# Edenzzzz/Stable-Diffusion-for-book-cover-generation

Hardware: NVIDIA B200
Metric: unet_denoise_it_per_s (higher is better)
Workload: dtype bf16

## Files before the change

### include/b200sd.h

```cpp
#ifndef B200SD_H_
#define B200SD_H_

#include <stddef.h>
#include <stdint.h>

#ifdef __cplusplus
extern "C" {
#endif

#define B200SD_OK 0
#define B200SD_ERR_INVALID 1
#define B200SD_ERR_CUDA 2
#define B200SD_ERR_UNSUPPORTED 3

#define B200SD_F32 0
#define B200SD_BF16 1

typedef void* b200sd_stream_t;

const char* b200sd_last_error(void);
int b200sd_version(void);
int64_t b200sd_launch_count(void);

void b200sd_debug_gemm_trace(void* buf);
void b200sd_debug_set(int key, int value);
int b200sd_timer_reserve(int n);
int b200sd_timer_record(int i, b200sd_stream_t stream);
int b200sd_timer_elapsed_ms(int i, int j, float* ms);


int b200sd_cfg_ddim_step(const void* eps_u, const void* eps_c, const void* x, void* out, void* eps_out,
                         int64_t n, float guidance, float sa_t, float sb_t, float sa_p, float sb_p,
                         int eps_dtype, int x_dtype, b200sd_stream_t stream);

int b200sd_sampler_advance(const float* timesteps, int n_steps, int* cursor, float* in_t, int n_t, b200sd_stream_t stream);
int b200sd_cfg_ddim_step_table(const void* eps_u, const void* eps_c, const void* x, void* out, void* eps_out,
                               int64_t n, float guidance, const float* coef_table, const int* cursor,
                               int eps_dtype, int x_dtype, b200sd_stream_t stream);

int b200sd_cfg_plms_step_table(const float* eps_u, const float* eps_c, float* x, float* saved, float* ring, int64_t n,
                               float guidance, const float* table, const int* cursor, b200sd_stream_t stream);

int b200sd_cfg_plms_step(const void* eps_u, const void* eps_c, const void* x, void* out, void* eps_out,
                         const void* hist0, const void* hist1, const void* hist2, const void* hist3,
                         int nhist, const float* w_host5, int64_t n, float guidance, float cx, float ce,
                         int eps_dtype, int x_dtype, b200sd_stream_t stream);

int b200sd_add_noise(const void* x0, const void* noise, const int64_t* timesteps, const float* sa_table,
                     const float* sb_table, void* out, int batch, int64_t per_sample, int num_train_timesteps,
                     int dtype, b200sd_stream_t stream);

int b200sd_mse_workspace_floats(void);
int b200sd_mse_loss_fwd(const void* pred, const void* target, float* loss_out, float* workspace, int64_t n,
                        int pred_dtype, int target_dtype, b200sd_stream_t stream);
int b200sd_mse_loss_bwd(const void* pred, const void* target, const float* grad_loss, void* grad_pred, int64_t n,
                        int pred_dtype, int target_dtype, b200sd_stream_t stream);


int b200sd_timestep_embedding(const float* timesteps, float* out, int batch, int dim, b200sd_stream_t stream);

int b200sd_small_linear(const float* in, const void* w_bf16, const float* bias, float* out, int batch, int N, int K,
                        int silu_in, int silu_out, b200sd_stream_t stream);

#define B200SD_EPI_LINEAR 0
#define B200SD_EPI_GEGLU 1
#define B200SD_W_ROW_MAJOR 0
#define B200SD_W_KBLOCK_MAJOR 1

typedef struct b200sd_gemm_args {
    const void* a0;
    const void* a1;
    const void* w;
    const float* bias;
    const float* rowbias;
    const void* residual;
    void* out;
    int M, N, K;
    int C0, C1;
    int lda0, lda1;
    int ldc, ldr;
    int ldrb;
    int conv_taps;
    int batch, H, W;
    int rows_per_image;
    int epilogue;
    int out_dtype;
    int residual_dtype;
    int block_n;
    int split_k;
    void* workspace;
    size_t workspace_bytes;
    int pair;
    float* gn_part;
    const void* prefetch;
    size_t prefetch_bytes;
    int w_layout;
} b200sd_gemm_args;

size_t b200sd_gemm_workspace_bytes(void);
int b200sd_geglu_tile(int N);
int b200sd_gemm(const b200sd_gemm_args* args, b200sd_stream_t stream);
int b200sd_gemm_gn_layout(const b200sd_gemm_args* args, int hw, int* parts_per_image, int* total_parts);

typedef struct b200sd_dgrad_args {
    const void* dy;
    const void* w;
    const void* residual;
    void* out;
    int M, Cout, Cin;
    int conv_taps;
    int batch, H, W;
    int ldy, ldc, ldr;
    int out_dtype, residual_dtype;
    int block_n;
    int pair;
} b200sd_dgrad_args;
int b200sd_gemm_dgrad(const b200sd_dgrad_args* args, b200sd_stream_t stream);

typedef struct b200sd_wgrad_args {
    const void* dy;
    const void* x;
    float* dw;
    int rows, Cout, Cin;
    int conv_taps;
    int batch, H, W;
    int ldy, ldx, lddw;
    int block_n, split_k;
} b200sd_wgrad_args;
int b200sd_gemm_wgrad(const b200sd_wgrad_args* args, b200sd_stream_t stream);

int b200sd_conv_in(const float* x_nchw, const float* w, const float* bias, void* out_nhwc, int batch, int Cin,
                   int Cout, int H, int W, int out_dtype, b200sd_stream_t stream);
int b200sd_conv_out(const void* x_nhwc, const float* w, const float* bias, float* out_nchw, int batch, int Cin,
                    int Cout, int H, int W, b200sd_stream_t stream);
int b200sd_nhwc_bias_to_nchw(const float* x, const float* bias, float* out_nchw, int batch, int C, int hw, int ld,
                             b200sd_stream_t stream);

int b200sd_groupnorm_silu(const void* x0, const void* x1, int C0, int C1, const float* gamma, const float* beta,
                          void* out, void* raw_out, float* stats_ws, int batch, int hw, int groups, float eps,
                          int silu, int in_dtype, b200sd_stream_t stream);

int b200sd_groupnorm_silu_stats(const void* x0, const void* x1, int C0, int C1, const float* gamma, const float* beta,
                                void* out, void* raw_out, float* stats_ws, float* stats_out, int batch, int hw, int groups,
                                float eps, int silu, int in_dtype, b200sd_stream_t stream);

int b200sd_groupnorm_silu_parts(const void* x0, const void* x1, int C0, int C1, const float* part0, int ppi0, int ld0,
                                const float* part1, int ppi1, int ld1, const float* gamma, const float* beta, void* out,
                                void* raw_out, float* stats_out, int batch, int hw, int groups, float eps, int silu,
                                int in_dtype, b200sd_stream_t stream);

int b200sd_groupnorm_workspace_floats(int batch);
int b200sd_layernorm(const void* x, const float* gamma, const float* beta, void* out, int rows, int C, float eps,
                     int in_dtype, b200sd_stream_t stream);

size_t b200sd_attention_workspace_bytes(int batch, int heads, int Skv, int d);
int b200sd_attention(const void* q, const void* k, const void* v, void* out, int batch, int heads, int Sq, int Skv,
                     int d, int ldq, int ldk, int ldv, int ldo, float scale, void* workspace, size_t workspace_bytes,
                     b200sd_stream_t stream);

int b200sd_attention_lse(const void* q, const void* k, const void* v, void* out, float* lse, int batch, int heads, int Sq,
                         int Skv, int d, int ldq, int ldk, int ldv, int ldo, float scale, void* workspace,
                         size_t workspace_bytes, b200sd_stream_t stream);

size_t b200sd_attention_bwd_workspace_bytes(int batch, int heads, int Sq);
int b200sd_attention_bwd(const void* q, const void* k, const void* v, const void* out, const void* dout,
                         const float* lse, void* dq, void* dk, void* dv, int batch, int heads, int Sq, int Skv, int d,
                         int ldq, int ldk, int ldv, int ldo, int lddo, int lddq, int lddk, int lddv, float scale,
                         void* workspace, size_t workspace_bytes, b200sd_stream_t stream);


int b200sd_clip_embed(const int64_t* ids, const float* tok, const float* pos, float* out, int batch, int S, int C, int vocab,
                      b200sd_stream_t stream);
int b200sd_clip_embed_bwd(const int64_t* ids, const float* dx, float* dtok, float* dpos, int batch, int S, int C, int vocab,
                          b200sd_stream_t stream);
int b200sd_quick_gelu_fwd(const void* u, void* out, int64_t n, b200sd_stream_t stream);
int b200sd_quick_gelu_bwd(const void* u, const void* dg, void* du, int64_t n, b200sd_stream_t stream);
int b200sd_layernorm_f32out(const float* x, const float* gamma, const float* beta, float* out, int rows, int C, float eps,
                            b200sd_stream_t stream);
int b200sd_causal_attention(const void* qkv, void* out, int batch, int heads, int S, int d, int ld, int ldo, int q_off,
                            int k_off, int v_off, float scale, b200sd_stream_t stream);
int b200sd_causal_attention_bwd(const void* qkv, const void* dout, void* dqkv, int batch, int heads, int S, int d, int ld,
                                int lddo, int ldd, int q_off, int k_off, int v_off, float scale, b200sd_stream_t stream);


int b200sd_im2col_s2_pad(const void* x, void* out, int batch, int H, int W, int C, int in_dtype, int pad,
                         b200sd_stream_t stream);
int b200sd_softmax_rows(const float* x, void* out_bf16, int rows, int L, int ldx, int ldo, float scale, b200sd_stream_t stream);
int b200sd_conv1x1_small(const float* x_nchw, const float* w, const float* bias, float* out_nchw, int batch, int Cin, int Cout,
                         int hw, b200sd_stream_t stream);
int b200sd_gaussian_sample(const float* moments, const float* noise, float* out, int batch, int C, int hw, float out_scale,
                           b200sd_stream_t stream);


int b200sd_grad_prep(const void* in, int in_dtype, void* out_bf16, float* colsum, int rows, int N, int ld,
                     int rows_per_image, int ldcs, b200sd_stream_t stream);

int b200sd_groupnorm_bwd_workspace_floats(int batch);
int b200sd_groupnorm_silu_bwd(const void* x0, const void* x1, int C0, int C1, int in_dtype, const float* gamma,
                              const float* beta, const void* dy, const float* add_src, void* out0, void* out1,
                              int out_dtype, int accumulate0, int accumulate1, float* dgamma, float* dbeta,
                              const float* mean_rstd, float* workspace, int batch, int hw, int groups, float eps, int silu,
                              b200sd_stream_t stream);

int b200sd_layernorm_bwd(const void* x, int in_dtype, const float* gamma, const void* dy, float* dres, float* dgamma,
                         float* dbeta, int rows, int C, float eps, b200sd_stream_t stream);

int b200sd_geglu_fwd(const void* u, void* out, int64_t rows, int C_half, b200sd_stream_t stream);
int b200sd_geglu_bwd(const void* u, const void* dff, void* du, int64_t rows, int C_half, b200sd_stream_t stream);

int b200sd_upsample2x_bwd(const void* dy, float* dx, int batch, int H, int W, int C, int accumulate, b200sd_stream_t stream);
int b200sd_col2im_s2(const void* dcol, float* dx, int batch, int H, int W, int C, int accumulate, b200sd_stream_t stream);

int b200sd_conv_out_bwd(const float* dout_nchw, const void* x_nhwc, const float* w, void* dx_nhwc, float* dw,
                        float* dbias, int batch, int Cin, int Cout, int H, int W, b200sd_stream_t stream);
int b200sd_conv_in_wgrad(const void* dy_nhwc, int dy_dtype, const float* x_nchw, float* dw, int batch, int Cin, int Cout,
                         int H, int W, b200sd_stream_t stream);

int b200sd_cast_act(const float* in, void* out_bf16, int64_t n, int silu, b200sd_stream_t stream);
int b200sd_silu_bwd_mul(const float* pre, float* grad, int64_t n, b200sd_stream_t stream);

int b200sd_split_hi_lo(const float* x, void* hi_bf16, void* lo_bf16, int64_t n, b200sd_stream_t stream);
int b200sd_groupnorm_silu_split(const void* x0, const void* x1, int C0, int C1, const float* gamma, const float* beta,
                                void* out, void* out_lo, void* raw_out, void* raw_lo, float* stats_ws, float* stats_out,
                                int batch, int hw, int groups, float eps, int silu, int in_dtype, b200sd_stream_t stream);
int b200sd_layernorm_split(const void* x, const float* gamma, const float* beta, void* out, void* out_lo, int rows, int C,
                           float eps, int in_dtype, b200sd_stream_t stream);
int b200sd_geglu_f32(const float* u, void* hi_bf16, void* lo_bf16, int64_t rows, int C_half, b200sd_stream_t stream);
int b200sd_attention_f32(const float* q, const float* k, const float* v, float* out, int batch, int heads, int Sq, int Skv,
                         int d, int ldq, int ldk, int ldv, int ldo, float scale, b200sd_stream_t stream);
int b200sd_small_linear_f32(const float* in, const float* w, const float* bias, float* out, int batch, int N, int K,
                            int silu_in, int silu_out, b200sd_stream_t stream);

int b200sd_cast_flat(const float* in, void* out_bf16, int64_t n, b200sd_stream_t stream);
int b200sd_adamw_step(float* param, float* grad, float* exp_avg, float* exp_avg_sq, void* weights_bf16, int64_t n,
                      float lr, float beta1, float beta2, float eps, float weight_decay, int step, float grad_scale,
                      int zero_grad, b200sd_stream_t stream);

int b200sd_adamw8bit_step(float* param, float* grad, uint8_t* state1, uint8_t* state2, float* absmax1, float* absmax2,
                          const float* qmap1, const float* qmap2, const int32_t* chunk_mode, float* small_exp_avg,
                          float* small_exp_avg_sq, void* weights_bf16, int64_t n, float lr, float beta1, float beta2, float eps,
                          float weight_decay, int step, float grad_scale, int zero_grad, b200sd_stream_t stream);

int b200sd_upsample2x(const void* x, void* out, int batch, int H, int W, int C, int in_dtype, b200sd_stream_t stream);
int b200sd_im2col_s2(const void* x, void* out, int batch, int H, int W, int C, int in_dtype, b200sd_stream_t stream);

#ifdef __cplusplus
}
#endif
#endif
```

### stable-diffusion-for-book-cover-generation_b200/_lib.py

```python
from __future__ import annotations

import ctypes as C
import os

_HERE = os.path.dirname(os.path.abspath(__file__))
LIB_PATH = os.path.join(_HERE, "libb200sd.so")

_lib = None


class B200SDError(RuntimeError):
    pass


class GemmArgs(C.Structure):
    _fields_ = [
        ("a0", C.c_void_p), ("a1", C.c_void_p), ("w", C.c_void_p), ("bias", C.c_void_p), ("rowbias", C.c_void_p),
        ("residual", C.c_void_p), ("out", C.c_void_p),
        ("M", C.c_int), ("N", C.c_int), ("K", C.c_int), ("C0", C.c_int), ("C1", C.c_int),
        ("lda0", C.c_int), ("lda1", C.c_int), ("ldc", C.c_int), ("ldr", C.c_int), ("ldrb", C.c_int), ("conv_taps", C.c_int),
        ("batch", C.c_int), ("H", C.c_int), ("W", C.c_int), ("rows_per_image", C.c_int), ("epilogue", C.c_int),
        ("out_dtype", C.c_int), ("residual_dtype", C.c_int), ("block_n", C.c_int), ("split_k", C.c_int),
        ("workspace", C.c_void_p), ("workspace_bytes", C.c_size_t), ("pair", C.c_int), ("gn_part", C.c_void_p), ("prefetch", C.c_void_p), ("prefetch_bytes", C.c_size_t), ("w_layout", C.c_int),
    ]


class DgradArgs(C.Structure):
    _fields_ = [
        ("dy", C.c_void_p), ("w", C.c_void_p), ("residual", C.c_void_p), ("out", C.c_void_p),
        ("M", C.c_int), ("Cout", C.c_int), ("Cin", C.c_int), ("conv_taps", C.c_int),
        ("batch", C.c_int), ("H", C.c_int), ("W", C.c_int), ("ldy", C.c_int), ("ldc", C.c_int), ("ldr", C.c_int),
        ("out_dtype", C.c_int), ("residual_dtype", C.c_int), ("block_n", C.c_int), ("pair", C.c_int),
    ]


class WgradArgs(C.Structure):
    _fields_ = [
        ("dy", C.c_void_p), ("x", C.c_void_p), ("dw", C.c_void_p),
        ("rows", C.c_int), ("Cout", C.c_int), ("Cin", C.c_int), ("conv_taps", C.c_int),
        ("batch", C.c_int), ("H", C.c_int), ("W", C.c_int), ("ldy", C.c_int), ("ldx", C.c_int), ("lddw", C.c_int),
        ("block_n", C.c_int), ("split_k", C.c_int),
    ]


_vp, _i, _i64, _f, _sz = C.c_void_p, C.c_int, C.c_int64, C.c_float, C.c_size_t

SIGNATURES = {
    "b200sd_last_error": (C.c_char_p, []),
    "b200sd_version": (_i, []),
    "b200sd_launch_count": (_i64, []),
    "b200sd_debug_gemm_trace": (None, [_vp]),
    "b200sd_debug_set": (None, [_i, _i]),
    "b200sd_timer_reserve": (_i, [_i]),
    "b200sd_timer_record": (_i, [_i, _vp]),
    "b200sd_timer_elapsed_ms": (_i, [_i, _i, C.POINTER(C.c_float)]),
    "b200sd_cfg_ddim_step": (_i, [_vp, _vp, _vp, _vp, _vp, _i64, _f, _f, _f, _f, _f, _i, _i, _vp]),
    "b200sd_clip_embed": (_i, [_vp, _vp, _vp, _vp, _i, _i, _i, _i, _vp]),
    "b200sd_clip_embed_bwd": (_i, [_vp, _vp, _vp, _vp, _i, _i, _i, _i, _vp]),
    "b200sd_quick_gelu_fwd": (_i, [_vp, _vp, _i64, _vp]),
    "b200sd_quick_gelu_bwd": (_i, [_vp, _vp, _vp, _i64, _vp]),
    "b200sd_layernorm_f32out": (_i, [_vp, _vp, _vp, _vp, _i, _i, _f, _vp]),
    "b200sd_causal_attention": (_i, [_vp, _vp, _i, _i, _i, _i, _i, _i, _i, _i, _i, _f, _vp]),
    "b200sd_causal_attention_bwd": (_i, [_vp, _vp, _vp, _i, _i, _i, _i, _i, _i, _i, _i, _i, _i, _f, _vp]),
    "b200sd_im2col_s2_pad": (_i, [_vp, _vp, _i, _i, _i, _i, _i, _i, _vp]),
    "b200sd_softmax_rows": (_i, [_vp, _vp, _i, _i, _i, _i, _f, _vp]),
    "b200sd_conv1x1_small": (_i, [_vp, _vp, _vp, _vp, _i, _i, _i, _i, _vp]),
    "b200sd_gaussian_sample": (_i, [_vp, _vp, _vp, _i, _i, _i, _f, _vp]),
    "b200sd_sampler_advance": (_i, [_vp, _i, _vp, _vp, _i, _vp]),
    "b200sd_cfg_plms_step_table": (_i, [_vp, _vp, _vp, _vp, _vp, _i64, _f, _vp, _vp, _vp]),
    "b200sd_cfg_ddim_step_table": (_i, [_vp, _vp, _vp, _vp, _vp, _i64, _f, _vp, _vp, _i, _i, _vp]),
    "b200sd_cfg_plms_step": (_i, [_vp, _vp, _vp, _vp, _vp, _vp, _vp, _vp, _vp, _i, C.POINTER(C.c_float), _i64, _f, _f,
                                  _f, _i, _i, _vp]),
    "b200sd_add_noise": (_i, [_vp, _vp, _vp, _vp, _vp, _vp, _i, _i64, _i, _i, _vp]),
    "b200sd_mse_workspace_floats": (_i, []),
    "b200sd_mse_loss_fwd": (_i, [_vp, _vp, _vp, _vp, _i64, _i, _i, _vp]),
    "b200sd_mse_loss_bwd": (_i, [_vp, _vp, _vp, _vp, _i64, _i, _i, _vp]),
    "b200sd_timestep_embedding": (_i, [_vp, _vp, _i, _i, _vp]),
    "b200sd_small_linear": (_i, [_vp, _vp, _vp, _vp, _i, _i, _i, _i, _i, _vp]),
    "b200sd_gemm_workspace_bytes": (_sz, []),
    "b200sd_geglu_tile": (_i, [_i]),
    "b200sd_gemm": (_i, [C.POINTER(GemmArgs), _vp]),
    "b200sd_gemm_gn_layout": (_i, [C.POINTER(GemmArgs), _i, C.POINTER(C.c_int), C.POINTER(C.c_int)]),
    "b200sd_groupnorm_silu_parts": (_i, [_vp, _vp, _i, _i, _vp, _i, _i, _vp, _i, _i, _vp, _vp, _vp, _vp, _vp, _i, _i, _i, _f, _i,
                                         _i, _vp]),
    "b200sd_gemm_dgrad": (_i, [C.POINTER(DgradArgs), _vp]),
    "b200sd_gemm_wgrad": (_i, [C.POINTER(WgradArgs), _vp]),
    "b200sd_conv_in": (_i, [_vp, _vp, _vp, _vp, _i, _i, _i, _i, _i, _i, _vp]),
    "b200sd_conv_out": (_i, [_vp, _vp, _vp, _vp, _i, _i, _i, _i, _i, _vp]),
    "b200sd_nhwc_bias_to_nchw": (_i, [_vp, _vp, _vp, _i, _i, _i, _i, _vp]),
    "b200sd_groupnorm_silu": (_i, [_vp, _vp, _i, _i, _vp, _vp, _vp, _vp, _vp, _i, _i, _i, _f, _i, _i, _vp]),
    "b200sd_groupnorm_silu_stats": (_i, [_vp, _vp, _i, _i, _vp, _vp, _vp, _vp, _vp, _vp, _i, _i, _i, _f, _i, _i, _vp]),
    "b200sd_groupnorm_workspace_floats": (_i, [_i]),
    "b200sd_layernorm": (_i, [_vp, _vp, _vp, _vp, _i, _i, _f, _i, _vp]),
    "b200sd_attention_workspace_bytes": (_sz, [_i, _i, _i, _i]),
    "b200sd_attention": (_i, [_vp, _vp, _vp, _vp, _i, _i, _i, _i, _i, _i, _i, _i, _i, _f, _vp, _sz, _vp]),
    "b200sd_attention_lse": (_i, [_vp, _vp, _vp, _vp, _vp, _i, _i, _i, _i, _i, _i, _i, _i, _i, _f, _vp, _sz, _vp]),
    "b200sd_attention_bwd_workspace_bytes": (_sz, [_i, _i, _i]),
    "b200sd_attention_bwd": (_i, [_vp] * 9 + [_i] * 13 + [_f, _vp, _sz, _vp]),
    "b200sd_grad_prep": (_i, [_vp, _i, _vp, _vp, _i, _i, _i, _i, _i, _vp]),
    "b200sd_groupnorm_bwd_workspace_floats": (_i, [_i]),
    "b200sd_groupnorm_silu_bwd": (_i, [_vp, _vp, _i, _i, _i, _vp, _vp, _vp, _vp, _vp, _vp, _i, _i, _i, _vp, _vp, _vp, _vp, _i,
                                       _i, _i, _f, _i, _vp]),
    "b200sd_layernorm_bwd": (_i, [_vp, _i, _vp, _vp, _vp, _vp, _vp, _i, _i, _f, _vp]),
    "b200sd_geglu_fwd": (_i, [_vp, _vp, _i64, _i, _vp]),
    "b200sd_geglu_bwd": (_i, [_vp, _vp, _vp, _i64, _i, _vp]),
    "b200sd_upsample2x_bwd": (_i, [_vp, _vp, _i, _i, _i, _i, _i, _vp]),
    "b200sd_col2im_s2": (_i, [_vp, _vp, _i, _i, _i, _i, _i, _vp]),
    "b200sd_conv_out_bwd": (_i, [_vp, _vp, _vp, _vp, _vp, _vp, _i, _i, _i, _i, _i, _vp]),
    "b200sd_conv_in_wgrad": (_i, [_vp, _i, _vp, _vp, _i, _i, _i, _i, _i, _vp]),
    "b200sd_cast_act": (_i, [_vp, _vp, _i64, _i, _vp]),
    "b200sd_silu_bwd_mul": (_i, [_vp, _vp, _i64, _vp]),
    "b200sd_split_hi_lo": (_i, [_vp, _vp, _vp, _i64, _vp]),
    "b200sd_groupnorm_silu_split": (_i, [_vp, _vp, _i, _i, _vp, _vp, _vp, _vp, _vp, _vp, _vp, _vp, _i, _i, _i, _f, _i, _i, _vp]),
    "b200sd_layernorm_split": (_i, [_vp, _vp, _vp, _vp, _vp, _i, _i, _f, _i, _vp]),
    "b200sd_geglu_f32": (_i, [_vp, _vp, _vp, _i64, _i, _vp]),
    "b200sd_attention_f32": (_i, [_vp, _vp, _vp, _vp, _i, _i, _i, _i, _i, _i, _i, _i, _i, _f, _vp]),
    "b200sd_small_linear_f32": (_i, [_vp, _vp, _vp, _vp, _i, _i, _i, _i, _i, _vp]),
    "b200sd_cast_flat": (_i, [_vp, _vp, _i64, _vp]),
    "b200sd_adamw_step": (_i, [_vp, _vp, _vp, _vp, _vp, _i64, _f, _f, _f, _f, _f, _i, _f, _i, _vp]),
    "b200sd_adamw8bit_step": (_i, [_vp] * 12 + [_i64, _f, _f, _f, _f, _f, _i, _f, _i, _vp]),
    "b200sd_upsample2x": (_i, [_vp, _vp, _i, _i, _i, _i, _i, _vp]),
    "b200sd_im2col_s2": (_i, [_vp, _vp, _i, _i, _i, _i, _i, _vp]),
}


def lib() -> C.CDLL:
    global _lib
    if _lib is None:
        if not os.path.exists(LIB_PATH):
            raise B200SDError(
                f"{LIB_PATH} is missing: build it with `python -c 'import __graft_entry__ as g; g.build()'` "
                "(b200sd has no CPU / eager fallback)")
        L = C.CDLL(LIB_PATH)
        for name, (res, args) in SIGNATURES.items():
            fn = getattr(L, name)
            fn.restype = res
            fn.argtypes = args
        _lib = L
    return _lib


def check(rc: int, what: str = "") -> None:
    if rc != 0:
        msg = lib().b200sd_last_error().decode("utf-8", "replace")
        raise B200SDError(f"{what or 'b200sd call'} failed (code {rc}): {msg}")
```

### stable-diffusion-for-book-cover-generation_b200/csrc/gemm_tcgen05.cu

```cuda
#include <atomic>
#include <cstring>
#include <mutex>
#include <cstdio>
#include <cstdlib>

#include "common.cuh"

extern std::atomic<long long> g_b200sd_launches;

static unsigned long long* g_gemm_trace = nullptr;
static int g_dbg[4] = {-1, 0, 0, 0};
static const int g_dbg_env = [] {
    const char* e = getenv("B200SD_EPI_DEPTH");
    if (e) g_dbg[3] = atoi(e);
    return 0;
}();
extern "C" void b200sd_debug_set(int key, int value) { if (key >= 0 && key < 4) g_dbg[key] = value; }
extern "C" void b200sd_debug_gemm_trace(void* buf) { g_gemm_trace = static_cast<unsigned long long*>(buf); }

namespace {

__device__ __forceinline__ unsigned long long gtimer() {
    unsigned long long t;
    asm volatile("mov.u64 %0, %globaltimer;" : "=l"(t));
    return t;
}
#define TRACE(slot)                                                                                   \
    do {                                                                                              \
        if (p.trace) p.trace[((size_t)(blockIdx.z * gridDim.y + blockIdx.y) * gridDim.x + blockIdx.x) * 16 + (slot)] = gtimer(); \
    } while (0)

constexpr int BLOCK_M = 128;
constexpr size_t kWsPartialBytes = (size_t)160 * 128 * 256 * sizeof(float);
constexpr size_t kWsCounterBytes = 4096;
constexpr int BLOCK_K = 64;
constexpr int UMMA_K = 16;
constexpr int kNumThreads = 192;
constexpr int kMaxStages = 8;
constexpr int kABytes = BLOCK_M * BLOCK_K * 2;


struct KParams {
    CUtensorMap tmA0, tmA1, tmB;
    const float* bias;
    const float* rowbias;
    const void* residual;
    void* out;
    int M, N;
    int num_k_blocks;
    int kb_per_split;
    int split_k;
    int block_n;
    int stages;
    int conv;
    int cblocks0;
    int cblocks;
    int tile_w, tile_h, tile_n;
    int tiles_y;
    int tiles_x;
    int rows_valid;
    int a_bytes;
    int ldc, ldr, ldrb;
    int rows_per_image;
    int epilogue;
    int out_f32;
    int res_f32;
    uint32_t tmem_cols;
    int a_mn;
    int b_mode;
    int conv_sign;
    int n_valid;
    int tiles_per_tap;
    int atomic_out;
    int pair;
    int persist;
    int psplit;
    int w_kmajor;
    const void* prefetch;
    size_t prefetch_bytes;
    float* gn_part;
    unsigned long long* trace;
};

__device__ __forceinline__ void cluster_sync_all() {
    asm volatile("barrier.cluster.arrive.release.aligned;\n\tbarrier.cluster.wait.acquire.aligned;" ::: "memory");
}
__device__ __forceinline__ uint32_t cluster_ctarank() {
    uint32_t r;
    asm volatile("mov.u32 %0, %%cluster_ctarank;" : "=r"(r));
    return r;
}
__device__ __forceinline__ float4 ld_dsmem_v4(uint32_t local_smem_addr, uint32_t cta_rank) {
    uint32_t raddr;
    asm volatile("mapa.shared::cluster.u32 %0, %1, %2;" : "=r"(raddr) : "r"(local_smem_addr), "r"(cta_rank));
    float4 v;
    asm volatile("ld.shared::cluster.v4.f32 {%0, %1, %2, %3}, [%4];" : "=f"(v.x), "=f"(v.y), "=f"(v.z), "=f"(v.w) : "r"(raddr) : "memory");
    return v;
}

__device__ __forceinline__ void red_add_v4(float* dst, float a, float b, float c, float d) {
    asm volatile("red.global.add.v4.f32 [%0], {%1, %2, %3, %4};" ::"l"(dst), "f"(a), "f"(b), "f"(c), "f"(d) : "memory");
}

struct EpiCtx {
    uint32_t stage_u32;
    int pitch_f, row_end, R, cb, half, m0, col_out, img0, n0cb;
    const float* s_rb;
    bool multi_img, rb_smem;
};
__device__ __forceinline__ void lds8(uint32_t addr, float (&v)[8]) {
    asm volatile("ld.shared.v4.f32 {%0, %1, %2, %3}, [%4];" : "=f"(v[0]), "=f"(v[1]), "=f"(v[2]), "=f"(v[3]) : "r"(addr));
    asm volatile("ld.shared.v4.f32 {%0, %1, %2, %3}, [%4];" : "=f"(v[4]), "=f"(v[5]), "=f"(v[6]), "=f"(v[7]) : "r"(addr + 16));
}
template <int OUT, int RES, bool SPLIT, bool GEGLU, bool STATS = false>
__device__ __forceinline__ void epilogue_rows(const KParams& p, const EpiCtx& e, int row0, const float (&b)[8], const float (&bg)[8],
                                              float* cs = nullptr, float* cq = nullptr) {
    constexpr int U = 4;
    for (int row = row0; row < e.row_end; row += e.R * U) {
        float v[U][8], r[U][8];
#pragma unroll
        for (int u = 0; u < U; ++u) {
            const int rl = min(row + u * e.R, e.row_end - 1);
            const uint32_t addr = e.stage_u32 + (uint32_t)(rl * e.pitch_f + e.cb) * 4u;
            if constexpr (SPLIT) {
#pragma unroll
                for (int i = 0; i < 8; ++i) v[u][i] = 0.f;
                for (int sp = 0; sp < p.split_k; ++sp) {
                    const float4 a0 = ld_dsmem_v4(addr, sp), a1 = ld_dsmem_v4(addr + 16, sp);
                    v[u][0] += a0.x; v[u][1] += a0.y; v[u][2] += a0.z; v[u][3] += a0.w;
                    v[u][4] += a1.x; v[u][5] += a1.y; v[u][6] += a1.z; v[u][7] += a1.w;
                }
            } else {
                lds8(addr, v[u]);
            }
            if constexpr (GEGLU) lds8(addr + (uint32_t)e.half * 4u, r[u]);
            else if constexpr (RES == 2) ld8<B200SD_F32>(p.residual, (size_t)(e.m0 + rl) * p.ldr + e.col_out, r[u]);
            else if constexpr (RES == 1) ld8<B200SD_BF16>(p.residual, (size_t)(e.m0 + rl) * p.ldr + e.col_out, r[u]);
        }
#pragma unroll
        for (int u = 0; u < U; ++u) {
            const int rl = row + u * e.R;
            if (rl >= e.row_end) break;
            const int grow = e.m0 + rl;
            float o[8];
            if constexpr (GEGLU) {
#pragma unroll
                for (int i = 0; i < 8; ++i) o[i] = (v[u][i] + b[i]) * gelu_erf_f(r[u][i] + bg[i]);
                st8<B200SD_BF16>(p.out, (size_t)grow * p.ldc + e.col_out, o);
            } else {
#pragma unroll
                for (int i = 0; i < 8; ++i) o[i] = v[u][i] + b[i];
                if constexpr (RES != 0) {
#pragma unroll
                    for (int i = 0; i < 8; ++i) o[i] += r[u][i];
                }
                if (e.multi_img) {
                    const int img = grow / p.rows_per_image;
                    if (e.rb_smem) {
                        const float* rb = e.s_rb + (img == e.img0 ? 0 : 256) + e.cb;
#pragma unroll
                        for (int i = 0; i < 8; ++i) o[i] += rb[i];
                    } else {
                        float t[8];
                        ld8<B200SD_F32>(p.rowbias, (size_t)img * p.ldrb + e.n0cb, t);
#pragma unroll
                        for (int i = 0; i < 8; ++i) o[i] += t[i];
                    }
                }
                if constexpr (STATS) {
#pragma unroll
                    for (int i = 0; i < 8; ++i) { cs[i] += o[i]; cq[i] = fmaf(o[i], o[i], cq[i]); }
                }
                if constexpr (OUT == 2) {
                    float* dst = static_cast<float*>(p.out) + (size_t)grow * p.ldc + e.col_out;
                    red_add_v4(dst, o[0], o[1], o[2], o[3]);
                    red_add_v4(dst + 4, o[4], o[5], o[6], o[7]);
                } else if constexpr (OUT == 1) st8<B200SD_F32>(p.out, (size_t)grow * p.ldc + e.col_out, o);
                else st8<B200SD_BF16>(p.out, (size_t)grow * p.ldc + e.col_out, o);
            }
        }
    }
}

template <bool PAIR, int OP>
__global__ void __launch_bounds__(kNumThreads, 1) gemm_tcgen05_kernel(const __grid_constant__ KParams p) {
    constexpr bool a_mn = OP >= 2;
    constexpr int b_mode = OP;
    extern __shared__ uint8_t smem_raw[];
    uint8_t* smem = reinterpret_cast<uint8_t*>((reinterpret_cast<uintptr_t>(smem_raw) + 1023) & ~uintptr_t(1023));
    constexpr bool pair = PAIR;
    const uint32_t crank = pair ? cluster_ctarank() : 0;
    const int b_bytes = (p.block_n * BLOCK_K * 2) >> (pair ? 1 : 0);
    uint8_t* smem_a = smem;
    uint8_t* smem_b = smem + (size_t)p.stages * kABytes;
    uint64_t* bars = reinterpret_cast<uint64_t*>(smem_b + (size_t)p.stages * b_bytes);
    uint64_t* full_bar = bars;
    uint64_t* empty_bar = bars + kMaxStages;
    uint64_t* tmem_full_bar = bars + 2 * kMaxStages;
    uint32_t* tmem_slot = reinterpret_cast<uint32_t*>(bars + 2 * kMaxStages + 1);

    const int warp = threadIdx.x >> 5;
    const int lane = threadIdx.x & 31;
    const int m_tile = blockIdx.x;
    const int n_tile = blockIdx.y;
    const int split = blockIdx.z;
    const int kb_begin = split * p.kb_per_split;
    const int kb_end = min(kb_begin + p.kb_per_split, p.num_k_blocks);
    const int w_tap = b_mode == 3 ? n_tile / p.tiles_per_tap : 0;
    const int n0 = (b_mode == 3 ? n_tile - w_tap * p.tiles_per_tap : n_tile) * p.block_n;
    const int col_base = w_tap * p.n_valid + n0;
    const int col_valid = min(p.block_n, p.n_valid - n0);
    const int m0 = m_tile * p.rows_valid;

    ptx::pdl_trigger();
    if (threadIdx.x == 0) TRACE(0);
    if (warp == 0 && lane == 0) {
        ptx::prefetch_tmap(&p.tmA0);
        ptx::prefetch_tmap(&p.tmB);
        if (p.cblocks0 != p.cblocks) ptx::prefetch_tmap(&p.tmA1);
        for (int s = 0; s < p.stages; ++s) {
            ptx::mbar_init(&full_bar[s], 1);
            ptx::mbar_init(&empty_bar[s], 1);
        }
        ptx::mbar_init(tmem_full_bar, 1);
        ptx::fence_barrier_init();
    }
    if (warp == 1) {
        if constexpr (pair) { ptx::tmem_alloc_cg2(tmem_slot, p.tmem_cols); ptx::tmem_relinquish_cg2(); }
        else { ptx::tmem_alloc(tmem_slot, p.tmem_cols); ptx::tmem_relinquish(); }
    }
    ptx::tc_fence_before();
    __syncthreads();
    if constexpr (pair) cluster_sync_all();
    ptx::tc_fence_after();
    const uint32_t tmem_base = *tmem_slot;
    ptx::pdl_wait();
    if (threadIdx.x == 0) TRACE(1);

    const int epi_tid = threadIdx.x - 64;
    const int pitch_f = p.block_n + 4;
    float* stage = reinterpret_cast<float*>(smem);
    float* s_bias = reinterpret_cast<float*>(bars + 32);
    float* s_rb = s_bias + 256;
    int img0 = 0, img1 = 0;
    bool rb_smem = false;
    if (p.rowbias && m0 < p.M) {
        img0 = m0 / p.rows_per_image;
        img1 = (min(m0 + p.rows_valid, p.M) - 1) / p.rows_per_image;
        rb_smem = (img1 - img0) <= 1;
    }

    if (warp == 0) {
        if (ptx::elect_one()) {
            int stage = 0;
            uint32_t phase = 0;
            int img = 0, y0 = 0, x0 = 0;
            if (p.conv) {
                if (p.tile_n > 1) { img = m_tile * p.tile_n; y0 = 0; }
                else {
                    int mt = m_tile;
                    if (p.tiles_x > 1) { x0 = (mt % p.tiles_x) * p.tile_w; mt /= p.tiles_x; }
                    img = mt / p.tiles_y; y0 = (mt % p.tiles_y) * p.tile_h;
                }
            }
            const int nbox_live = (b_mode != 0 && !pair) ? (col_valid + 63) >> 6 : (p.block_n >> 6);
            const int nboxb = nbox_live >> (pair ? 1 : 0);
            const int nb0 = n0 + (pair ? (int)crank * (p.block_n >> 1) : 0);
            const uint32_t stage_tx = (b_mode != 0 && !pair) ? (uint32_t)(p.a_bytes + nbox_live * 8192)
                                                             : ((uint32_t)(p.a_bytes + b_bytes) << (pair ? 1 : 0));
            for (int kb = kb_begin; kb < kb_end; ++kb) {
                ptx::mbar_wait(&empty_bar[stage], phase ^ 1);
                if (!pair || crank == 0) ptx::mbar_expect_tx(&full_bar[stage], stage_tx);
                uint8_t* dst_a = smem_a + (size_t)stage * kABytes;
                uint8_t* dst_b = smem_b + (size_t)stage * b_bytes;
                uint64_t* fb = &full_bar[stage];
                const uint32_t fbc = pair ? ptx::mapa_u32(ptx::smem_u32(fb), 0) : 0;
#define LD2(dst, tm, c0, c1) do { if constexpr (pair) ptx::tma_load_2d_cg2(dst, tm, fbc, c0, c1); else ptx::tma_load_2d(dst, tm, fb, c0, c1); } while (0)
#define LD3(dst, tm, c0, c1, c2) do { if constexpr (pair) ptx::tma_load_3d_cg2(dst, tm, fbc, c0, c1, c2); else ptx::tma_load_3d(dst, tm, fb, c0, c1, c2); } while (0)
#define LD4(dst, tm, c0, c1, c2, c3) do { if constexpr (pair) ptx::tma_load_4d_cg2(dst, tm, fbc, c0, c1, c2, c3); else ptx::tma_load_4d(dst, tm, fb, c0, c1, c2, c3); } while (0)
                if (a_mn) {
                    LD2(dst_a, &p.tmA0, m0, kb * BLOCK_K);
                    LD2(dst_a + kABytes / 2, &p.tmA0, m0 + 64, kb * BLOCK_K);
                } else if (!p.conv) {
                    if (kb < p.cblocks0) LD2(dst_a, &p.tmA0, kb * BLOCK_K, m0);
                    else LD2(dst_a, &p.tmA1, (kb - p.cblocks0) * BLOCK_K, m0);
                } else {
                    const int tap = kb / p.cblocks;
                    const int cb = kb - tap * p.cblocks;
                    const int dy = (tap / 3 - 1) * p.conv_sign, dx = (tap % 3 - 1) * p.conv_sign;
                    if (cb < p.cblocks0) LD4(dst_a, &p.tmA0, cb * BLOCK_K, x0 + dx, y0 + dy, img);
                    else LD4(dst_a, &p.tmA1, (cb - p.cblocks0) * BLOCK_K, x0 + dx, y0 + dy, img);
                }
                if (b_mode == 0) {
                    if (p.w_kmajor) LD3(dst_b, &p.tmB, 0, nb0, kb);
                    else LD2(dst_b, &p.tmB, kb * BLOCK_K, nb0);
                } else if (b_mode == 1) {
                    if (!p.conv) {
                        for (int j = 0; j < nboxb; ++j) LD2(dst_b + j * 8192, &p.tmB, nb0 + j * 64, kb * BLOCK_K);
                    } else {
                        const int tap = kb / p.cblocks;
                        const int cb = kb - tap * p.cblocks;
                        for (int j = 0; j < nboxb; ++j) LD3(dst_b + j * 8192, &p.tmB, nb0 + j * 64, tap, cb * BLOCK_K);
                    }
                } else if (b_mode == 2) {
                    for (int j = 0; j < nboxb; ++j) LD2(dst_b + j * 8192, &p.tmB, nb0 + j * 64, kb * BLOCK_K);
                } else {
                    int bimg, by0;
                    if (p.tile_n > 1) { bimg = kb * p.tile_n; by0 = 0; }
                    else { bimg = kb / p.tiles_y; by0 = (kb - bimg * p.tiles_y) * p.tile_h; }
                    const int dy = w_tap / 3 - 1, dx = w_tap % 3 - 1;
                    for (int j = 0; j < nboxb; ++j) LD4(dst_b + j * 8192, &p.tmB, nb0 + j * 64, dx, by0 + dy, bimg);
                }
#undef LD2
#undef LD3
#undef LD4
                if (++stage == p.stages) { stage = 0; phase ^= 1; }
            }
        }
    } else if (warp == 1) {
        if ((!pair || crank == 0) && ptx::elect_one()) {
            const uint32_t b_mn = b_mode != 0;
            const uint32_t mma_n = (b_mode != 0 && !pair) ? (uint32_t)(((col_valid + 63) >> 6) << 6) : (uint32_t)p.block_n;
            const uint32_t idesc = ptx::umma_idesc_bf16(pair ? 2 * BLOCK_M : BLOCK_M, mma_n) | ((uint32_t)a_mn << 15) | (b_mn << 16);
            const uint32_t a_step = a_mn ? (2048 >> 4) : 2, b_step = b_mn ? (2048 >> 4) : 2;
            int stage = 0;
            uint32_t phase = 0;
            for (int kb = kb_begin; kb < kb_end; ++kb) {
                ptx::mbar_wait(&full_bar[stage], phase);
                ptx::tc_fence_after();
                if (kb == kb_begin) TRACE(2);
                const uint32_t sa = ptx::smem_u32(smem_a + (size_t)stage * kABytes), sb = ptx::smem_u32(smem_b + (size_t)stage * b_bytes);
                const uint64_t da = a_mn ? ptx::umma_desc_mn_sw128(sa, 8192) : ptx::umma_desc_k_sw128(sa);
                const uint64_t db = b_mn ? ptx::umma_desc_mn_sw128(sb, 8192) : ptx::umma_desc_k_sw128(sb);
#pragma unroll
                for (int k = 0; k < BLOCK_K / UMMA_K; ++k) {
                    const uint32_t accum = (kb > kb_begin || k > 0) ? 1u : 0u;
                    if constexpr (pair) ptx::umma_bf16_ss_cg2(tmem_base, da + a_step * k, db + b_step * k, idesc, accum);
                    else ptx::umma_bf16_ss(tmem_base, da + a_step * k, db + b_step * k, idesc, accum);
                }
                if constexpr (pair) ptx::umma_commit_cg2(&empty_bar[stage], 3); else ptx::umma_commit(&empty_bar[stage]);
                if (++stage == p.stages) { stage = 0; phase ^= 1; }
            }
            if constexpr (pair) ptx::umma_commit_cg2(tmem_full_bar, 3); else ptx::umma_commit(tmem_full_bar);
            TRACE(3);
        }
    } else {
        const int q = warp & 3;
        const int r_in_tile = q * 32 + lane;
        const uint32_t taddr = tmem_base + ((uint32_t)(q * 32) << 16);
        for (int c = epi_tid; c < p.block_n; c += 128) {
            s_bias[c] = (p.bias && c < col_valid) ? __ldg(p.bias + n0 + c) : 0.f;
            if (rb_smem) {
                s_rb[c] = __ldg(p.rowbias + (size_t)img0 * p.ldrb + n0 + c);
                s_rb[256 + c] = __ldg(p.rowbias + (size_t)img1 * p.ldrb + n0 + c);
            }
        }
        if (epi_tid == 0 && p.prefetch_bytes)
            ptx::prefetch_share_l2(p.prefetch, p.prefetch_bytes, (blockIdx.z * gridDim.y + blockIdx.y) * gridDim.x + blockIdx.x,
                              gridDim.x * gridDim.y * gridDim.z);
        ptx::mbar_wait(tmem_full_bar, 0);
        ptx::tc_fence_after();
        if (epi_tid == 0) TRACE(4);
        {
            float4* my_row = reinterpret_cast<float4*>(stage + (size_t)r_in_tile * pitch_f);
            for (int c = 0; c < p.block_n; c += 32) {
                uint32_t r0[16], r1[16];
                const bool two = (c + 16 < p.block_n);
                ptx::tmem_ld_32x32b_x16(taddr + c, r0);
                if (two) ptx::tmem_ld_32x32b_x16(taddr + c + 16, r1);
                ptx::tmem_ld_wait();
#pragma unroll
                for (int i = 0; i < 4; ++i)
                    my_row[c / 4 + i] = make_float4(__uint_as_float(r0[4 * i]), __uint_as_float(r0[4 * i + 1]),
                                                    __uint_as_float(r0[4 * i + 2]), __uint_as_float(r0[4 * i + 3]));
                if (two) {
#pragma unroll
                    for (int i = 0; i < 4; ++i)
                        my_row[c / 4 + 4 + i] = make_float4(__uint_as_float(r1[4 * i]), __uint_as_float(r1[4 * i + 1]),
                                                            __uint_as_float(r1[4 * i + 2]), __uint_as_float(r1[4 * i + 3]));
                }
            }
        }
        ptx::tc_fence_before();
        ptx::named_bar_sync(1, 128);
        if (epi_tid == 0) TRACE(5);
    }

    if (p.split_k > 1) cluster_sync_all(); else __syncthreads();

    {
        const int rank = p.split_k > 1 ? (int)cluster_ctarank() : 0;
        const int rows_per_cta = BLOCK_M / p.split_k;
        const int row_begin = rank * rows_per_cta;
        int valid = min(p.rows_valid, p.M - m0) - row_begin;
        valid = max(0, min(valid, rows_per_cta));
        const bool geglu = p.epilogue == B200SD_EPI_GEGLU;
        const int half = p.block_n / 2;
        const int groups = (geglu ? half : p.block_n) / 8;
        const int R = kNumThreads / groups;
        const int tid = threadIdx.x;
        float cs[8], cq[8];
#pragma unroll
        for (int i = 0; i < 8; ++i) { cs[i] = 0.f; cq[i] = 0.f; }
        if (tid < R * groups && valid > 0) {
            const int c8 = tid % groups, r0 = tid / groups;
            const int cb = c8 * 8;
            if (geglu || cb < col_valid) {
                float b[8], bg[8];
#pragma unroll
                for (int i = 0; i < 8; ++i) { b[i] = s_bias[cb + i]; bg[i] = geglu ? s_bias[half + cb + i] : 0.f; }
                const bool multi_img = p.rowbias != nullptr && img1 != img0;
                if (p.rowbias != nullptr && !multi_img) {
#pragma unroll
                    for (int i = 0; i < 8; ++i) b[i] += s_rb[cb + i];
                }
                EpiCtx e;
                e.stage_u32 = ptx::smem_u32(stage);
                e.pitch_f = pitch_f; e.row_end = row_begin + valid; e.R = R; e.cb = cb; e.half = half; e.m0 = m0;
                e.col_out = geglu ? n_tile * half + cb : col_base + cb;
                e.s_rb = s_rb; e.img0 = img0; e.multi_img = multi_img; e.rb_smem = rb_smem; e.n0cb = n0 + cb;
                const int row0 = row_begin + r0;
                const int ok = p.atomic_out ? 2 : (p.out_f32 ? 1 : 0);
                const int rk = p.residual ? (p.res_f32 ? 2 : 1) : 0;
                if (geglu) epilogue_rows<0, 0, false, true>(p, e, row0, b, bg);
                else if (p.split_k > 1) {
                    if (ok == 1 && p.gn_part) { if (rk == 2) epilogue_rows<1, 2, true, false, true>(p, e, row0, b, bg, cs, cq); else epilogue_rows<1, 0, true, false, true>(p, e, row0, b, bg, cs, cq); }
                    else if (ok == 1) { if (rk == 2) epilogue_rows<1, 2, true, false>(p, e, row0, b, bg); else if (rk == 1) epilogue_rows<1, 1, true, false>(p, e, row0, b, bg); else epilogue_rows<1, 0, true, false>(p, e, row0, b, bg); }
                    else { if (rk == 2) epilogue_rows<0, 2, true, false>(p, e, row0, b, bg); else if (rk == 1) epilogue_rows<0, 1, true, false>(p, e, row0, b, bg); else epilogue_rows<0, 0, true, false>(p, e, row0, b, bg); }
                } else if (ok == 2) epilogue_rows<2, 0, false, false>(p, e, row0, b, bg);
                else if (ok == 1 && p.gn_part) { if (rk == 2) epilogue_rows<1, 2, false, false, true>(p, e, row0, b, bg, cs, cq); else epilogue_rows<1, 0, false, false, true>(p, e, row0, b, bg, cs, cq); }
                else if (ok == 1) { if (rk == 2) epilogue_rows<1, 2, false, false>(p, e, row0, b, bg); else if (rk == 1) epilogue_rows<1, 1, false, false>(p, e, row0, b, bg); else epilogue_rows<1, 0, false, false>(p, e, row0, b, bg); }
                else { if (rk == 2) epilogue_rows<0, 2, false, false>(p, e, row0, b, bg); else if (rk == 1) epilogue_rows<0, 1, false, false>(p, e, row0, b, bg); else epilogue_rows<0, 0, false, false>(p, e, row0, b, bg); }
            }
        }
        if (p.gn_part != nullptr) {
            if (p.split_k > 1) cluster_sync_all(); else __syncthreads();
            float* s_gn = reinterpret_cast<float*>(stage);
#pragma unroll
            for (int i = 0; i < 8; ++i) { s_gn[tid * 16 + i] = cs[i]; s_gn[tid * 16 + 8 + i] = cq[i]; }
            __syncthreads();
            float* dst = p.gn_part + (size_t)(m_tile * p.split_k + rank) * 2 * p.N;
            for (int idx = tid; idx < groups * 16; idx += kNumThreads) {
                const int c8 = idx >> 4, k = idx & 15, col = c8 * 8 + (k & 7);
                float a = 0.f;
                for (int r = 0; r < R; ++r) a += s_gn[(r * groups + c8) * 16 + k];
                if (col < col_valid) dst[(size_t)(k >> 3) * p.N + n0 + col] = a;
            }
        }
        if (epi_tid == 0) TRACE(6);
    }
    if (p.split_k > 1 && p.gn_part == nullptr) cluster_sync_all();

    ptx::tc_fence_before();
    __syncthreads();
    if constexpr (pair) cluster_sync_all();
    if (warp == 1) {
        ptx::tc_fence_after();
        if constexpr (pair) ptx::tmem_dealloc_cg2(tmem_base, p.tmem_cols); else ptx::tmem_dealloc(tmem_base, p.tmem_cols);
    }
    if (threadIdx.x == 0) TRACE(7);
}

constexpr int kEpiWarps = 8;
constexpr int kPersistThreads = 64 + 32 * kEpiWarps + 32;
constexpr int kMaxDepth = 3;

struct PParams {
    CUtensorMap tmA0, tmA1, tmB, tmOut, tmRes;
    const float* bias;
    const float* rowbias;
    float* gn_part;
    int M, N;
    int num_k_blocks, block_n, stages;
    int conv, cblocks0, cblocks, tile_h, tile_n, tiles_y, w_kmajor;
    int tile_w, tiles_x;
    int n_tiles, num_tiles;
    int ldrb, rows_per_image;
    int geglu, out_f32, res_kind;
    int pf_share;
    int depth;
    int chunk_bytes;
    uint32_t tmem_cols, acc_stride;
    uint32_t off_b, off_epi, off_bias, off_stat, off_bars;
    int split, kb_per_split;
    CUtensorMap tmWs;
    float* ws;
    int* cnt;
    const void* prefetch;
    size_t prefetch_bytes;
    const void* residual;
    void* out;
    int ldc, ldr;
    unsigned long long* trace;
};
#define PTRACE(slot) do { if (p.trace) p.trace[(size_t)blockIdx.x * 16 + (slot)] = gtimer(); } while (0)
#ifdef B200SD_TRACE_EPILOGUE
#define PACC(i) do { if (p.trace && ew == 0) { const long long t__ = clock64(); pacc[i] += t__ - pt0; pt0 = t__; } } while (0)
#else
#define PACC(i) do { } while (0)
#endif


template <bool OUT_F32, int RES, bool GEGLU, bool STATS>
__device__ __forceinline__ void persist_chunk(const PParams& p, uint32_t taddr, int ch, const float* sbv, const float* sbg, uint8_t* cb,
                                              int lane, bool last_chunk, uint64_t* tempty_bar, uint64_t* rfull_bar, uint32_t rparity,
                                              float* gn_dst, int nrows) {
    uint32_t r0[16], r1[16], g0[16], g1[16];
    ptx::tmem_ld_32x32b_x16(taddr + ch * 32, r0);
    ptx::tmem_ld_32x32b_x16(taddr + ch * 32 + 16, r1);
    const int half = p.block_n >> 1;
    if constexpr (GEGLU) {
        ptx::tmem_ld_32x32b_x16(taddr + half + ch * 32, g0);
        ptx::tmem_ld_32x32b_x16(taddr + half + ch * 32 + 16, g1);
    }
    if constexpr (RES != 0) ptx::mbar_wait(rfull_bar, rparity);
    ptx::tmem_ld_wait();
    if (last_chunk) {
        ptx::tc_fence_before();
        __syncwarp();
        if (lane == 0) ptx::mbar_arrive(tempty_bar);
    }
    float v[32];
    const float4* sb4 = reinterpret_cast<const float4*>(sbv);
#pragma unroll
    for (int j = 0; j < 8; ++j) {
        const float4 b = sb4[j];
        const uint32_t* r = j < 4 ? r0 : r1;
        const int o = (j & 3) * 4;
        v[4 * j + 0] = __uint_as_float(r[o + 0]) + b.x;
        v[4 * j + 1] = __uint_as_float(r[o + 1]) + b.y;
        v[4 * j + 2] = __uint_as_float(r[o + 2]) + b.z;
        v[4 * j + 3] = __uint_as_float(r[o + 3]) + b.w;
    }
    if constexpr (GEGLU) {
        const float4* sg4 = reinterpret_cast<const float4*>(sbg);
#pragma unroll
        for (int j = 0; j < 8; ++j) {
            const float4 b = sg4[j];
            const uint32_t* r = j < 4 ? g0 : g1;
            const int o = (j & 3) * 4;
            v[4 * j + 0] *= gelu_erf_fast(__uint_as_float(r[o + 0]) + b.x);
            v[4 * j + 1] *= gelu_erf_fast(__uint_as_float(r[o + 1]) + b.y);
            v[4 * j + 2] *= gelu_erf_fast(__uint_as_float(r[o + 2]) + b.z);
            v[4 * j + 3] *= gelu_erf_fast(__uint_as_float(r[o + 3]) + b.w);
        }
    }
    uint8_t* row128 = cb + lane * 128;
    uint8_t* row64 = cb + lane * 64;
    const int x128 = lane & 7, x64 = (lane >> 1) & 3;
    if constexpr (RES == 2) {
#pragma unroll
        for (int j = 0; j < 8; ++j) {
            const float4 t = *reinterpret_cast<const float4*>(row128 + ((j ^ x128) << 4));
            v[4 * j + 0] += t.x; v[4 * j + 1] += t.y; v[4 * j + 2] += t.z; v[4 * j + 3] += t.w;
        }
    } else if constexpr (RES == 1) {
#pragma unroll
        for (int j = 0; j < 4; ++j) {
            const uint4 u = *reinterpret_cast<const uint4*>(row64 + ((j ^ x64) << 4));
            float2 f;
            f = unpack_bf16x2(u.x); v[8 * j + 0] += f.x; v[8 * j + 1] += f.y;
            f = unpack_bf16x2(u.y); v[8 * j + 2] += f.x; v[8 * j + 3] += f.y;
            f = unpack_bf16x2(u.z); v[8 * j + 4] += f.x; v[8 * j + 5] += f.y;
            f = unpack_bf16x2(u.w); v[8 * j + 6] += f.x; v[8 * j + 7] += f.y;
        }
    }
    if constexpr (RES != 0 && ((RES == 2) != OUT_F32)) __syncwarp();
    if constexpr (OUT_F32) {
#pragma unroll
        for (int j = 0; j < 8; ++j)
            *reinterpret_cast<float4*>(row128 + ((j ^ x128) << 4)) = make_float4(v[4 * j], v[4 * j + 1], v[4 * j + 2], v[4 * j + 3]);
    } else {
#pragma unroll
        for (int j = 0; j < 4; ++j) {
            uint4 u;
            u.x = pack_bf16x2(v[8 * j + 0], v[8 * j + 1]);
            u.y = pack_bf16x2(v[8 * j + 2], v[8 * j + 3]);
            u.z = pack_bf16x2(v[8 * j + 4], v[8 * j + 5]);
            u.w = pack_bf16x2(v[8 * j + 6], v[8 * j + 7]);
            *reinterpret_cast<uint4*>(row64 + ((j ^ x64) << 4)) = u;
        }
    }
    if constexpr (STATS) {
        __syncwarp();
        float s = 0.f, ss = 0.f;
        const uint8_t* colp = cb + ((lane & 3) << 2);
        const int piece = lane >> 2;
        for (int r = 0; r < nrows; ++r) {
            const float x = *reinterpret_cast<const float*>(colp + r * 128 + ((piece ^ (r & 7)) << 4));
            s += x;
            ss = fmaf(x, x, ss);
        }
        gn_dst[ch * 32 + lane] = s;
        gn_dst[256 + ch * 32 + lane] = ss;
    }
}

template <bool OUT_F32, int RES, bool GEGLU, bool STATS>
__device__ __forceinline__ void persist_epilogue(const PParams& p, uint8_t* smem, uint32_t tmem_base, int warp, int lane) {
    const int ew = warp - 2;
    const int q = warp & 3;
    const int h = ew >> 2;
    const int D = p.depth;
    const int kChunkBytes = p.chunk_bytes;
    uint8_t* my = smem + p.off_epi + (size_t)ew * D * kChunkBytes;
    float* sb = reinterpret_cast<float*>(smem + p.off_bias) + ew * 256;
    uint64_t* bars = reinterpret_cast<uint64_t*>(smem + p.off_bars);
    uint64_t* tfull = bars + 16;
    uint64_t* tempty = bars + 18;
    uint64_t* rfull = bars + 20 + ew * kMaxDepth;
    const int half = p.block_n >> 1;
    const int nch = (GEGLU ? half : p.block_n) >> 5;
    const int nl = nch > h ? (nch - h + 1) >> 1 : 0;
    const int my_tiles = ((int)blockIdx.x < p.num_tiles) ? (p.num_tiles - 1 - (int)blockIdx.x) / (int)gridDim.x + 1 : 0;
    const int total = my_tiles * nl;
    const int out_n = GEGLU ? half : p.block_n;

    auto issue_res = [&](int g) {
        const int itl = g / nl, ch = h + 2 * (g - itl * nl);
        const int tile = (int)blockIdx.x + itl * (int)gridDim.x;
        const int m_tile = tile / p.n_tiles, n_tile = tile - m_tile * p.n_tiles;
        const int buf = g % D;
        ptx::mbar_expect_tx(&rfull[buf], RES == 2 ? 4096u : 2048u);
        ptx::tma_load_2d(my + buf * kChunkBytes, &p.tmRes, &rfull[buf], n_tile * p.block_n + ch * 32, m_tile * BLOCK_M + q * 32);
    };
    if constexpr (RES != 0) {
        if (lane == 0)
            for (int g = 0; g < D && g < total; ++g) issue_res(g);
    }

    int g = 0;
#ifdef B200SD_TRACE_EPILOGUE
    long long pacc[6] = {0, 0, 0, 0, 0, 0}, pt0 = clock64();
#endif
    for (int it = 0; it < my_tiles; ++it) {
        const int tile = (int)blockIdx.x + it * (int)gridDim.x;
        const int m_tile = tile / p.n_tiles, n_tile = tile - m_tile * p.n_tiles;
        const int n0 = n_tile * p.block_n;
        const int row0 = m_tile * BLOCK_M + q * 32;
        PACC(5);
        __syncwarp();
        {
            const int img = p.rowbias ? min(row0, p.M - 1) / p.rows_per_image : 0;
            for (int l = 0; l < nl; ++l) {
                const int c = (h + 2 * l) * 32 + lane;
                float b = p.bias ? __ldg(p.bias + n0 + c) : 0.f;
                if (p.rowbias) b += __ldg(p.rowbias + (size_t)img * p.ldrb + n0 + c);
                sb[l * 32 + lane] = b;
                if constexpr (GEGLU) sb[128 + l * 32 + lane] = p.bias ? __ldg(p.bias + n0 + half + c) : 0.f;
            }
        }
        __syncwarp();
        PACC(0);
        const int acc = it & 1;
        ptx::mbar_wait(&tfull[acc], (uint32_t)(it >> 1) & 1u);
        ptx::tc_fence_after();
        PACC(1);
        if (it == 0 && ew == 0 && lane == 0) PTRACE(4);
        const uint32_t taddr = tmem_base + (uint32_t)acc * p.acc_stride + ((uint32_t)(q * 32) << 16);
        const int nrows = max(0, min(32, p.M - row0));
        float* sstat = reinterpret_cast<float*>(smem + p.off_stat);
        float* gn_dst = STATS ? sstat + q * 512 : nullptr;
        if (nl == 0) {
            ptx::tc_fence_before();
            __syncwarp();
            if (lane == 0) ptx::mbar_arrive(&tempty[acc]);
        }
        for (int l = 0; l < nl; ++l, ++g) {
            const int ch = h + 2 * l;
            const int buf = g % D;
            uint8_t* cb = my + buf * kChunkBytes;
            if constexpr (RES == 0) {
                if (lane == 0) ptx::tma_store_wait_read<1>();
                __syncwarp();
            }
            PACC(2);
            persist_chunk<OUT_F32, RES, GEGLU, STATS>(p, taddr, ch, sb + l * 32, sb + 128 + l * 32, cb, lane, l == nl - 1, &tempty[acc],
                                                     &rfull[buf], (uint32_t)(g / D) & 1u, gn_dst, nrows);
            PACC(3);
            ptx::fence_proxy_async();
            __syncwarp();
            if (lane == 0) {
                ptx::tma_store_2d(&p.tmOut, cb, n_tile * out_n + ch * 32, row0);
                ptx::tma_store_commit();
                if constexpr (RES != 0) {
                    if (g >= 1 && g - 1 + D < total) {
                        ptx::tma_store_wait_read<1>();
                        issue_res(g - 1 + D);
                    }
                }
            }
            PACC(4);
        }
        if constexpr (STATS) {
            ptx::named_bar_sync(1, kEpiWarps * 32);
            const int te = ew * 32 + lane;
            if (te < p.block_n) {
                float s0 = 0.f, s1 = 0.f;
#pragma unroll
                for (int qq = 0; qq < 4; ++qq) { s0 += sstat[qq * 512 + te]; s1 += sstat[qq * 512 + 256 + te]; }
                float* dst = p.gn_part + (size_t)m_tile * 2 * p.N + n0 + te;
                dst[0] = s0;
                dst[p.N] = s1;
            }
            ptx::named_bar_sync(1, kEpiWarps * 32);
        }
    }
    if (ew == 0 && lane == 0) PTRACE(5);
#ifdef B200SD_TRACE_EPILOGUE
    if (p.trace && ew == 0 && lane == 0)
        for (int i = 0; i < 6; ++i) p.trace[(size_t)blockIdx.x * 16 + 8 + i] = (unsigned long long)pacc[i];
#endif
    if (lane == 0) ptx::tma_store_wait<0>();
    __syncwarp();
    if (ew == 0 && lane == 0) PTRACE(6);
}

template <bool OUT_F32, int RES, bool STATS>
__device__ __forceinline__ void persist_epilogue_split(const PParams& p, uint8_t* smem, uint32_t tmem_base, int warp, int lane) {
    const int ew = warp - 2, q = warp & 3, h = ew >> 2;
    const int kChunkBytes = 4096;
    uint8_t* my = smem + p.off_epi + (size_t)ew * 2 * kChunkBytes;
    uint64_t* bars = reinterpret_cast<uint64_t*>(smem + p.off_bars);
    uint64_t* tfull = bars + 16;
    uint64_t* tempty = bars + 18;
    const int unit = blockIdx.x, tile = unit / p.split, s = unit - tile * p.split;
    const int m_tile = tile / p.n_tiles, n_tile = tile - m_tile * p.n_tiles;
    const int n0 = n_tile * p.block_n, m0 = m_tile * BLOCK_M;
    const int nch = p.block_n >> 5;
    const int nl = nch > h ? (nch - h + 1) >> 1 : 0;
    ptx::mbar_wait(&tfull[0], 0);
    ptx::tc_fence_after();
    const uint32_t taddr = tmem_base + ((uint32_t)(q * 32) << 16);
    for (int l = 0; l < nl; ++l) {
        const int ch = h + 2 * l;
        uint8_t* cb = my + (l & 1) * kChunkBytes;
        if (lane == 0) ptx::tma_store_wait_read<1>();
        __syncwarp();
        uint32_t r0[16], r1[16];
        ptx::tmem_ld_32x32b_x16(taddr + ch * 32, r0);
        ptx::tmem_ld_32x32b_x16(taddr + ch * 32 + 16, r1);
        ptx::tmem_ld_wait();
        uint8_t* row128 = cb + lane * 128;
        const int x128 = lane & 7;
#pragma unroll
        for (int j = 0; j < 8; ++j) {
            const uint32_t* r = j < 4 ? r0 : r1;
            const int o = (j & 3) * 4;
            *reinterpret_cast<uint4*>(row128 + ((j ^ x128) << 4)) = make_uint4(r[o], r[o + 1], r[o + 2], r[o + 3]);
        }
        ptx::fence_proxy_async();
        __syncwarp();
        if (lane == 0) {
            ptx::tma_store_2d(&p.tmWs, cb, ch * 32, unit * BLOCK_M + q * 32);
            ptx::tma_store_commit();
        }
    }
    ptx::tc_fence_before();
    __syncwarp();
    if (lane == 0) {
        ptx::mbar_arrive(&tempty[0]);
        ptx::tma_store_wait<0>();
        ptx::fence_proxy_async_global();
        __threadfence();
    }
    ptx::named_bar_sync(1, kEpiWarps * 32);
    const int te = ew * 32 + lane;
    int* cnt_in = p.cnt + tile;
    int* cnt_out = p.cnt + p.num_tiles + tile;
    if (te == 0) {
        atomicAdd(cnt_in, 1);
        int seen;
        long long t0 = clock64();
        do {
            asm volatile("ld.acquire.gpu.global.s32 %0, [%1];" : "=r"(seen) : "l"(cnt_in) : "memory");
            if (clock64() - t0 > 4000000000LL) { printf("b200sd: split-K arrival wait timed out (unit %d)\n", unit); __trap(); }
        } while (seen < p.split);
        __threadfence();
    }
    ptx::named_bar_sync(1, kEpiWarps * 32);
    const int rpc = BLOCK_M / p.split;
    const int groups = p.block_n >> 2;
    const int rslots = (kEpiWarps * 32) / groups < 4 ? (kEpiWarps * 32) / groups : 4;
    const int c4 = te % groups, rslot = te / groups;
    float* sstat = reinterpret_cast<float*>(smem + p.off_stat);
    float cs[4] = {0.f, 0.f, 0.f, 0.f}, cq[4] = {0.f, 0.f, 0.f, 0.f};
    if (rslot < rslots) {
        const int col = n0 + c4 * 4;
        float4 b4 = p.bias ? __ldg(reinterpret_cast<const float4*>(p.bias + col)) : make_float4(0.f, 0.f, 0.f, 0.f);
        for (int r = rslot; r < rpc; r += rslots) {
            const int trow = s * rpc + r;
            const int grow = m0 + trow;
            if (grow >= p.M) break;
            float4 v = make_float4(0.f, 0.f, 0.f, 0.f);
            const float* src = p.ws + ((size_t)(tile * p.split) * BLOCK_M + trow) * p.block_n + c4 * 4;
            for (int j = 0; j < p.split; ++j) {
                const float4 t = __ldcg(reinterpret_cast<const float4*>(src + (size_t)j * BLOCK_M * p.block_n));
                v.x += t.x; v.y += t.y; v.z += t.z; v.w += t.w;
            }
            v.x += b4.x; v.y += b4.y; v.z += b4.z; v.w += b4.w;
            if (p.rowbias) {
                const float4 t = __ldg(reinterpret_cast<const float4*>(p.rowbias + (size_t)(grow / p.rows_per_image) * p.ldrb + col));
                v.x += t.x; v.y += t.y; v.z += t.z; v.w += t.w;
            }
            if constexpr (RES == 2) {
                const float4 t = __ldcg(reinterpret_cast<const float4*>(static_cast<const float*>(p.residual) + (size_t)grow * p.ldr + col));
                v.x += t.x; v.y += t.y; v.z += t.z; v.w += t.w;
            } else if constexpr (RES == 1) {
                const uint2 u = __ldcg(reinterpret_cast<const uint2*>(static_cast<const bf16*>(p.residual) + (size_t)grow * p.ldr + col));
                const float2 f0 = unpack_bf16x2(u.x), f1 = unpack_bf16x2(u.y);
                v.x += f0.x; v.y += f0.y; v.z += f1.x; v.w += f1.y;
            }
            if constexpr (STATS) {
                cs[0] += v.x; cs[1] += v.y; cs[2] += v.z; cs[3] += v.w;
                cq[0] = fmaf(v.x, v.x, cq[0]); cq[1] = fmaf(v.y, v.y, cq[1]); cq[2] = fmaf(v.z, v.z, cq[2]); cq[3] = fmaf(v.w, v.w, cq[3]);
            }
            if constexpr (OUT_F32) {
                *reinterpret_cast<float4*>(static_cast<float*>(p.out) + (size_t)grow * p.ldc + col) = v;
            } else {
                uint2 u;
                u.x = pack_bf16x2(v.x, v.y);
                u.y = pack_bf16x2(v.z, v.w);
                *reinterpret_cast<uint2*>(static_cast<bf16*>(p.out) + (size_t)grow * p.ldc + col) = u;
            }
        }
    }
    if constexpr (STATS) {
        if (rslot < 4) {
#pragma unroll
            for (int i = 0; i < 4; ++i) { sstat[rslot * 512 + c4 * 4 + i] = cs[i]; sstat[rslot * 512 + 256 + c4 * 4 + i] = cq[i]; }
        }
        ptx::named_bar_sync(1, kEpiWarps * 32);
        if (te < p.block_n) {
            float s0 = 0.f, s1 = 0.f;
            for (int rs = 0; rs < rslots; ++rs) { s0 += sstat[rs * 512 + te]; s1 += sstat[rs * 512 + 256 + te]; }
            float* dst = p.gn_part + (size_t)(m_tile * p.split + s) * 2 * p.N + n0 + te;
            dst[0] = s0;
            dst[p.N] = s1;
        }
    }
    ptx::named_bar_sync(1, kEpiWarps * 32);
    if (te == 0) {
        __threadfence();
        if (atomicAdd(cnt_out, 1) == p.split - 1) {
            *cnt_out = 0;
            *cnt_in = 0;
            __threadfence();
        }
    }
}

__global__ void __launch_bounds__(kPersistThreads, 1) gemm_persist_kernel(const __grid_constant__ PParams p) {
    extern __shared__ uint8_t smem_raw[];
    uint8_t* smem = reinterpret_cast<uint8_t*>((reinterpret_cast<uintptr_t>(smem_raw) + 1023) & ~uintptr_t(1023));
    uint8_t* smem_a = smem;
    uint8_t* smem_b = smem + p.off_b;
    uint64_t* bars = reinterpret_cast<uint64_t*>(smem + p.off_bars);
    uint64_t* full_bar = bars;
    uint64_t* empty_bar = bars + 8;
    uint64_t* tfull = bars + 16;
    uint64_t* tempty = bars + 18;
    uint64_t* rfull = bars + 20;
    uint32_t* tmem_slot = reinterpret_cast<uint32_t*>(bars + 20 + kEpiWarps * kMaxDepth);
    const int warp = threadIdx.x >> 5;
    const int lane = threadIdx.x & 31;
    const int b_bytes = p.block_n * BLOCK_K * 2;

    const bool splitk = p.split > 1;
    const int sk_tile = splitk ? (int)blockIdx.x / p.split : 0, sk_s = splitk ? (int)blockIdx.x - sk_tile * p.split : 0;
    const int sk_kb0 = splitk ? (sk_s * p.num_k_blocks) / p.split : 0;
    const int sk_kb1 = splitk ? ((sk_s + 1) * p.num_k_blocks) / p.split : p.num_k_blocks;
    int pr_stage = 0, pr_tile = splitk ? sk_tile : (int)blockIdx.x, pr_kb = sk_kb0, pr_m0 = 0, pr_n0 = 0, pr_img = 0, pr_y0 = 0, pr_x0 = 0, pr_tap = 0,
        pr_cb = 0, pr_me = 0;
    bool pr_new = true;
    uint32_t pr_phase = 0;
    constexpr int kPrefetch = 0;
    auto prefetch_b = [&](int k) {
        if (k < p.num_k_blocks && k % p.pf_share == pr_me) {
            if (p.w_kmajor) ptx::tma_prefetch_3d(&p.tmB, 0, pr_n0, k);
            else ptx::tma_prefetch_2d(&p.tmB, k * BLOCK_K, pr_n0);
        }
    };
    auto produce = [&](int limit, const int what) {
        const bool load_a = what & 1, load_b = what & 2;
        while (limit > 0 && pr_tile < p.num_tiles) {
            if (pr_new) {
                pr_new = false;
                const int m_tile = pr_tile / p.n_tiles, n_tile = pr_tile - m_tile * p.n_tiles;
                pr_m0 = m_tile * BLOCK_M;
                pr_n0 = n_tile * p.block_n;
                if (p.conv) {
                    if (p.tile_n > 1) { pr_img = m_tile * p.tile_n; pr_y0 = 0; }
                    else {
                        int mt = m_tile;
                        if (p.tiles_x > 1) { pr_x0 = (mt % p.tiles_x) * p.tile_w; mt /= p.tiles_x; }
                        pr_img = mt / p.tiles_y; pr_y0 = (mt - pr_img * p.tiles_y) * p.tile_h;
                    }
                }
                pr_tap = pr_kb / p.cblocks;
                pr_cb = pr_kb - pr_tap * p.cblocks;
                pr_me = m_tile % p.pf_share;
                if (load_b)
                    for (int k = p.stages; k < kPrefetch; ++k) prefetch_b(k);
            }
            uint64_t* fb = &full_bar[pr_stage];
            if (what) ptx::mbar_wait(&empty_bar[pr_stage], pr_phase ^ 1);
            if (load_a) {
                ptx::mbar_expect_tx(fb, (uint32_t)kABytes);

                uint8_t* dst_a = smem_a + (size_t)pr_stage * kABytes;
                if (!p.conv) {
                    if (pr_kb < p.cblocks0) ptx::tma_load_2d(dst_a, &p.tmA0, fb, pr_kb * BLOCK_K, pr_m0);
                    else ptx::tma_load_2d(dst_a, &p.tmA1, fb, (pr_kb - p.cblocks0) * BLOCK_K, pr_m0);
                } else {
                    const int dy = pr_tap / 3 - 1, dx = pr_tap - (pr_tap / 3) * 3 - 1;
                    if (pr_cb < p.cblocks0) ptx::tma_load_4d(dst_a, &p.tmA0, fb, pr_cb * BLOCK_K, pr_x0 + dx, pr_y0 + dy, pr_img);
                    else ptx::tma_load_4d(dst_a, &p.tmA1, fb, (pr_cb - p.cblocks0) * BLOCK_K, pr_x0 + dx, pr_y0 + dy, pr_img);
                }
            }
            if (load_b) {
                ptx::mbar_expect_tx(fb, (uint32_t)b_bytes);
                uint8_t* dst_b = smem_b + (size_t)pr_stage * b_bytes;
                if (p.w_kmajor) ptx::tma_load_3d(dst_b, &p.tmB, fb, 0, pr_n0, pr_kb);
                else ptx::tma_load_2d(dst_b, &p.tmB, fb, pr_kb * BLOCK_K, pr_n0);
                if (kPrefetch > 0) prefetch_b(pr_kb + kPrefetch);
            }
            if (++pr_stage == p.stages) { pr_stage = 0; pr_phase ^= 1; }
            if (++pr_cb == p.cblocks) { pr_cb = 0; ++pr_tap; }
            if (++pr_kb == sk_kb1) { pr_kb = 0; pr_new = true; pr_tile = splitk ? p.num_tiles : pr_tile + (int)gridDim.x; }
            --limit;
        }
    };
    const bool is_prod_a = threadIdx.x == 0, is_prod_b = threadIdx.x == kPersistThreads - 32;

    ptx::pdl_trigger();
    if (threadIdx.x == 0) PTRACE(0);
    if (warp == 0 && lane == 0) {
        ptx::prefetch_tmap(&p.tmA0);
        ptx::prefetch_tmap(&p.tmB);
        ptx::prefetch_tmap(&p.tmOut);
        if (p.cblocks0 != p.cblocks) ptx::prefetch_tmap(&p.tmA1);
        if (p.res_kind) ptx::prefetch_tmap(&p.tmRes);
        for (int s = 0; s < p.stages; ++s) {
            ptx::mbar_init(&full_bar[s], 2);
            ptx::mbar_init(&empty_bar[s], 1);
        }
        for (int s = 0; s < 2; ++s) {
            ptx::mbar_init(&tfull[s], 1);
            ptx::mbar_init(&tempty[s], kEpiWarps);
        }
        for (int s = 0; s < kEpiWarps * kMaxDepth; ++s) ptx::mbar_init(&rfull[s], 1);
        ptx::fence_barrier_init();
        ptx::pdl_wait();
        produce(p.stages, 3);
    }
    if (warp == 1) {
        ptx::tmem_alloc(tmem_slot, p.tmem_cols);
        ptx::tmem_relinquish();
    }
    ptx::tc_fence_before();
    __syncthreads();
    ptx::tc_fence_after();
    const uint32_t tmem_base = *tmem_slot;
    ptx::pdl_wait();
    if (threadIdx.x == 0) PTRACE(1);

    if (warp == 0) {
        if (is_prod_a) produce(0x7fffffff, 1);
    } else if (warp == kPersistThreads / 32 - 1) {
        if (is_prod_b) {
            produce(p.stages, 0);
            produce(0x7fffffff, 2);
        }
    } else if (warp == 1) {
        if (ptx::elect_one()) {
            const uint32_t idesc = ptx::umma_idesc_bf16(BLOCK_M, (uint32_t)p.block_n);
            int stage = 0;
            uint32_t phase = 0;
            int it = 0;
            const int nkb = sk_kb1 - sk_kb0;
            for (int tile = splitk ? sk_tile : (int)blockIdx.x; tile < p.num_tiles; tile = splitk ? p.num_tiles : tile + (int)gridDim.x, ++it) {
                const int acc = it & 1;
                ptx::mbar_wait(&tempty[acc], ((uint32_t)(it >> 1) & 1u) ^ 1u);
                ptx::tc_fence_after();
                const uint32_t d_tmem = tmem_base + (uint32_t)acc * p.acc_stride;
                for (int kb = 0; kb < nkb; ++kb) {
                    ptx::mbar_wait(&full_bar[stage], phase);
                    ptx::tc_fence_after();
                    if (it == 0 && kb == 0) PTRACE(2);
                    const uint64_t da = ptx::umma_desc_k_sw128(ptx::smem_u32(smem_a + (size_t)stage * kABytes));
                    const uint64_t db = ptx::umma_desc_k_sw128(ptx::smem_u32(smem_b + (size_t)stage * b_bytes));
#pragma unroll
                    for (int k = 0; k < BLOCK_K / UMMA_K; ++k)
                        ptx::umma_bf16_ss(d_tmem, da + 2 * k, db + 2 * k, idesc, (kb > 0 || k > 0) ? 1u : 0u);
                    ptx::umma_commit(&empty_bar[stage]);
                    if (++stage == p.stages) { stage = 0; phase ^= 1; }
                }
                ptx::umma_commit(&tfull[acc]);
                if (it == 0) PTRACE(3);
            }
        }
    } else {
        if (warp == 2 && lane == 0 && p.prefetch_bytes)
            ptx::prefetch_share_l2(p.prefetch, p.prefetch_bytes, blockIdx.x, gridDim.x);
        const int variant = (p.geglu ? 100 : 0) + (p.out_f32 ? 10 : 0) + p.res_kind + (p.gn_part ? 1000 : 0);
        if (splitk) {
            switch (variant) {
                case 0: persist_epilogue_split<false, 0, false>(p, smem, tmem_base, warp, lane); break;
                case 1: persist_epilogue_split<false, 1, false>(p, smem, tmem_base, warp, lane); break;
                case 2: persist_epilogue_split<false, 2, false>(p, smem, tmem_base, warp, lane); break;
                case 10: persist_epilogue_split<true, 0, false>(p, smem, tmem_base, warp, lane); break;
                case 11: persist_epilogue_split<true, 1, false>(p, smem, tmem_base, warp, lane); break;
                case 12: persist_epilogue_split<true, 2, false>(p, smem, tmem_base, warp, lane); break;
                case 1010: persist_epilogue_split<true, 0, true>(p, smem, tmem_base, warp, lane); break;
                case 1012: persist_epilogue_split<true, 2, true>(p, smem, tmem_base, warp, lane); break;
                default: break;
            }
        } else
        switch (variant) {
            case 100: persist_epilogue<false, 0, true, false>(p, smem, tmem_base, warp, lane); break;
            case 0: persist_epilogue<false, 0, false, false>(p, smem, tmem_base, warp, lane); break;
            case 1: persist_epilogue<false, 1, false, false>(p, smem, tmem_base, warp, lane); break;
            case 2: persist_epilogue<false, 2, false, false>(p, smem, tmem_base, warp, lane); break;
            case 10: persist_epilogue<true, 0, false, false>(p, smem, tmem_base, warp, lane); break;
            case 11: persist_epilogue<true, 1, false, false>(p, smem, tmem_base, warp, lane); break;
            case 12: persist_epilogue<true, 2, false, false>(p, smem, tmem_base, warp, lane); break;
            case 1010: persist_epilogue<true, 0, false, true>(p, smem, tmem_base, warp, lane); break;
            case 1012: persist_epilogue<true, 2, false, true>(p, smem, tmem_base, warp, lane); break;
            default: break;
        }
    }
    ptx::tc_fence_before();
    __syncthreads();
    if (warp == 1) {
        ptx::tc_fence_after();
        ptx::tmem_dealloc(tmem_base, p.tmem_cols);
    }
    if (threadIdx.x == 0) PTRACE(7);
}

uint32_t pow2_cols(int n) {
    uint32_t c = 32;
    while ((int)c < n) c <<= 1;
    return c;
}

int pick_block_n(int N, int m_tiles, int epilogue, bool can_split = false) {
    const int step = (epilogue == B200SD_EPI_GEGLU) ? 32 : 16;
    const int sms = b200sd_num_sms();
    int best = 0;
    for (int bn = 160; bn >= 64; bn -= step)
        if (N % bn == 0) { best = bn; break; }
    if (best == 0) {
        for (int bn = 256; bn >= step; bn -= step)
            if (N % bn == 0) { best = bn; break; }
        return best;
    }
    if (epilogue == B200SD_EPI_LINEAR && !can_split && (long)m_tiles * (N / best) * 2 <= sms) {
        for (int bn = 80; bn < best; bn += step)
            if (N % bn == 0 && (long)m_tiles * (N / bn) <= sms) { best = bn; break; }
    }
    return best;
}


typedef void (*gemm_kernel_t)(const KParams);
gemm_kernel_t gemm_entry(int pair, int op) {
    switch ((op << 1) | (pair ? 1 : 0)) {
        case 0: return gemm_tcgen05_kernel<false, 0>;
        case 1: return gemm_tcgen05_kernel<true, 0>;
        case 2: return gemm_tcgen05_kernel<false, 1>;
        case 3: return gemm_tcgen05_kernel<true, 1>;
        case 4: return gemm_tcgen05_kernel<false, 2>;
        case 5: return gemm_tcgen05_kernel<true, 2>;
        case 6: return gemm_tcgen05_kernel<false, 3>;
        default: return gemm_tcgen05_kernel<true, 3>;
    }
}

int configure_gemm_kernels() {
    static std::mutex mu;
    static bool configured[64] = {};
    int dev = 0;
    B200SD_CUDA(cudaGetDevice(&dev));
    std::lock_guard<std::mutex> lock(mu);
    if (dev < 0 || dev >= 64 || configured[dev]) return B200SD_OK;
    for (int i = 0; i < 8; ++i) {
        B200SD_CUDA(cudaFuncSetAttribute(gemm_entry(i & 1, i >> 1), cudaFuncAttributeMaxDynamicSharedMemorySize, (int)(227 * 1024)));
        B200SD_CUDA(cudaFuncSetAttribute(gemm_entry(i & 1, i >> 1), cudaFuncAttributePreferredSharedMemoryCarveout, 100));
    }
    B200SD_CUDA(cudaFuncSetAttribute(gemm_persist_kernel, cudaFuncAttributeMaxDynamicSharedMemorySize, (int)(227 * 1024)));
    B200SD_CUDA(cudaFuncSetAttribute(gemm_persist_kernel, cudaFuncAttributePreferredSharedMemoryCarveout, 100));
    configured[dev] = true;
    return B200SD_OK;
}

bool persist_enabled() {
    static const bool off = getenv("B200SD_PERSIST") && getenv("B200SD_PERSIST")[0] == '0';
    if (g_dbg[0] >= 0) return g_dbg[0] != 0;
    return !off;
}
int pick_block_n_persist(int N, int m_tiles, bool geglu) {
    const int sms = b200sd_num_sms();
    const int step = geglu ? 64 : 32;
    long best_cost = 0;
    int best = 0;
    for (int bn = step; bn <= 256; bn += step) {
        if (N % bn) continue;
        const long tiles = (long)m_tiles * (N / bn);
        const long cost = ((tiles + sms - 1) / sms) * (BLOCK_M + bn);
        if (best == 0 || cost < best_cost || (cost == best_cost && bn > best)) { best = bn; best_cost = cost; }
    }
    return best;
}

int launch_persist(const b200sd_gemm_args* a, const KParams& k, int m_tiles, b200sd_stream_t stream) {
    PParams p;
    memset(&p, 0, sizeof(p));
    p.tmA0 = k.tmA0; p.tmA1 = k.tmA1; p.tmB = k.tmB;
    p.bias = k.bias; p.rowbias = k.rowbias; p.gn_part = k.gn_part;
    p.M = k.M; p.N = k.N;
    p.num_k_blocks = k.num_k_blocks; p.block_n = k.block_n;
    p.conv = k.conv; p.cblocks0 = k.cblocks0; p.cblocks = k.cblocks;
    p.tile_h = k.tile_h; p.tile_n = k.tile_n; p.tiles_y = k.tiles_y; p.w_kmajor = k.w_kmajor;
    p.tile_w = k.tile_w; p.tiles_x = k.tiles_x;
    p.n_tiles = k.N / k.block_n;
    p.num_tiles = m_tiles * p.n_tiles;
    p.ldrb = k.ldrb; p.rows_per_image = k.rows_per_image;
    p.geglu = k.epilogue == B200SD_EPI_GEGLU;
    p.out_f32 = k.out_f32;
    p.res_kind = k.residual ? (k.res_f32 ? 2 : 1) : 0;
    {
        const int sms_ = b200sd_num_sms();
        const int grid_ = p.num_tiles < sms_ ? p.num_tiles : sms_;
        int share = grid_ / p.n_tiles;
        if (share > m_tiles) share = m_tiles;
        p.pf_share = share < 1 ? 1 : share;
    }
    p.depth = p.res_kind ? kMaxDepth : 2;
    if (p.res_kind && g_dbg[3] >= 2 && g_dbg[3] <= kMaxDepth) p.depth = g_dbg[3];
    p.split = k.psplit > 1 ? k.psplit : 1;
    p.kb_per_split = ceil_div(k.num_k_blocks, p.split);
    p.residual = k.residual; p.out = k.out; p.ldc = k.ldc; p.ldr = k.ldr;
    p.prefetch = k.prefetch; p.prefetch_bytes = k.prefetch_bytes;
    const int units = p.num_tiles * p.split;
    if (p.split > 1) {
        B200SD_REQUIRE(k.num_k_blocks >= p.split, "gemm(split-K): fewer K blocks (%d) than slices (%d)", k.num_k_blocks, p.split);
        B200SD_REQUIRE(units <= b200sd_num_sms() && (size_t)units * BLOCK_M * k.block_n * sizeof(float) <= kWsPartialBytes &&
                           (size_t)2 * p.num_tiles * sizeof(int) <= kWsCounterBytes,
                       "gemm(split-K): %d units do not fit the workspace / the machine", units);
        p.depth = 2;
        p.ws = static_cast<float*>(a->workspace);
        p.cnt = reinterpret_cast<int*>(static_cast<char*>(a->workspace) + kWsPartialBytes);
        const uint64_t dims[2] = {(uint64_t)k.block_n, (uint64_t)units * BLOCK_M};
        const uint64_t str[2] = {0, (uint64_t)k.block_n * 4};
        const uint32_t box[2] = {32, 32};
        const int rc = b200sd_make_tmap(&p.tmWs, a->workspace, 2, dims, str, box, CU_TENSOR_MAP_SWIZZLE_128B, CU_TENSOR_MAP_DATA_TYPE_FLOAT32);
        if (rc) return rc;
    }
    const int bn = k.block_n;
    p.acc_stride = bn <= 128 ? 128 : 256;
    p.tmem_cols = 2 * p.acc_stride;
    const int out_cols = p.geglu ? k.N / 2 : k.N;
    {
        const uint64_t dims[2] = {(uint64_t)out_cols, (uint64_t)k.M};
        const uint64_t str[2] = {0, (uint64_t)k.ldc * (k.out_f32 ? 4 : 2)};
        const uint32_t box[2] = {32, 32};
        const int rc = b200sd_make_tmap(&p.tmOut, k.out, 2, dims, str, box, k.out_f32 ? CU_TENSOR_MAP_SWIZZLE_128B : CU_TENSOR_MAP_SWIZZLE_64B,
                                        k.out_f32 ? CU_TENSOR_MAP_DATA_TYPE_FLOAT32 : CU_TENSOR_MAP_DATA_TYPE_BFLOAT16);
        if (rc) return rc;
    }
    if (p.res_kind) {
        const uint64_t dims[2] = {(uint64_t)k.N, (uint64_t)k.M};
        const uint64_t str[2] = {0, (uint64_t)k.ldr * (k.res_f32 ? 4 : 2)};
        const uint32_t box[2] = {32, 32};
        const int rc = b200sd_make_tmap(&p.tmRes, k.residual, 2, dims, str, box, k.res_f32 ? CU_TENSOR_MAP_SWIZZLE_128B : CU_TENSOR_MAP_SWIZZLE_64B,
                                        k.res_f32 ? CU_TENSOR_MAP_DATA_TYPE_FLOAT32 : CU_TENSOR_MAP_DATA_TYPE_BFLOAT16);
        if (rc) return rc;
    }
    const int stage_bytes = kABytes + bn * BLOCK_K * 2;
    p.chunk_bytes = (p.out_f32 || p.res_kind == 2 || k.psplit > 1) ? 4096 : 2048;
    const int epi_bytes = kEpiWarps * p.depth * p.chunk_bytes;
    const int bias_bytes = kEpiWarps * 256 * (int)sizeof(float);
    const int stat_bytes = k.gn_part ? 4 * 2 * 256 * (int)sizeof(float) : 0;
    const int bars_bytes = 512;
    const int budget = 227 * 1024 - 1024;
    int stages = (budget - epi_bytes - bias_bytes - stat_bytes - bars_bytes) / stage_bytes;
    if (stages > kMaxStages) stages = kMaxStages;
    if (g_dbg[1] > 0 && g_dbg[1] < stages) stages = g_dbg[1];
    B200SD_REQUIRE(stages >= 2, "gemm(persistent): smem budget leaves %d stages for block_n %d", stages, bn);
    p.stages = stages;
    p.off_b = (uint32_t)stages * kABytes;
    p.off_epi = (uint32_t)stages * stage_bytes;
    p.off_bias = p.off_epi + epi_bytes;
    p.off_stat = p.off_bias + bias_bytes;
    p.off_bars = p.off_stat + stat_bytes;
    const size_t smem_bytes = (size_t)p.off_bars + bars_bytes + 1024;
    p.trace = g_gemm_trace;
    {
        const int rc = configure_gemm_kernels();
        if (rc) return rc;
    }
    const int sms = b200sd_num_sms();
    cudaLaunchConfig_t cfg = {};
    int grid = p.num_tiles < sms ? p.num_tiles : sms;
    if (g_dbg[2] > 0 && g_dbg[2] < grid) grid = g_dbg[2];
    if (p.split > 1) grid = units;
    cfg.gridDim = dim3(grid);
    cfg.blockDim = dim3(kPersistThreads);
    cfg.dynamicSmemBytes = smem_bytes;
    cfg.stream = static_cast<cudaStream_t>(stream);
    cudaLaunchAttribute attr[2];
    int na = 0;
    if (p.split > 1) {
        attr[na].id = cudaLaunchAttributeCooperative;
        attr[na].val.cooperative = 1;
        ++na;
    }
    if (b200sd_pdl_enabled()) {
        attr[na].id = cudaLaunchAttributeProgrammaticStreamSerialization;
        attr[na].val.programmaticStreamSerializationAllowed = 1;
        ++na;
    }
    cfg.attrs = attr;
    cfg.numAttrs = na;
    B200SD_CUDA(cudaLaunchKernelEx(&cfg, gemm_persist_kernel, p));
    g_b200sd_launches.fetch_add(1, std::memory_order_relaxed);
    B200SD_LAUNCH_CHECK();
    return B200SD_OK;
}

int launch_gemm(KParams& p, int m_tiles, int n_tiles, int grid_z, bool cluster, b200sd_stream_t stream) {
    const int sms = b200sd_num_sms();
    const int bn = p.block_n;
    if (p.pair) m_tiles = (m_tiles + 1) & ~1;
    const int stage_bytes = kABytes + ((bn * BLOCK_K * 2) >> (p.pair ? 1 : 0));
    const long total_ctas = (long)m_tiles * n_tiles * grid_z;
    int stages;
    if (total_ctas <= sms || bn > 160) stages = (200 * 1024) / stage_bytes;
    else stages = (108 * 1024) / stage_bytes;
    if (stages > kMaxStages) stages = kMaxStages;
    if (stages > p.kb_per_split && total_ctas <= sms) stages = p.kb_per_split;
    const int min_stages = ceil_div(BLOCK_M * (bn + 4) * (int)sizeof(float), stage_bytes);
    if (g_dbg[1] > 0 && g_dbg[1] < stages) stages = g_dbg[1];
    if (stages < min_stages) stages = min_stages;
    if (stages < 2) stages = 2;
    p.stages = stages;
    B200SD_REQUIRE((size_t)stages * stage_bytes >= (size_t)BLOCK_M * (bn + 4) * sizeof(float), "gemm: smem ring smaller than the epilogue staging tile");
    const size_t smem_bytes = (size_t)stages * stage_bytes + 1024  + 256  + 3072 ;
    B200SD_REQUIRE(smem_bytes <= 227 * 1024, "gemm: smem budget exceeded (%zu B)", smem_bytes);

    {
        const int rc = configure_gemm_kernels();
        if (rc) return rc;
    }
    p.trace = g_gemm_trace;
    cudaLaunchConfig_t cfg = {};
    cfg.gridDim = dim3(m_tiles, n_tiles, grid_z);
    cfg.blockDim = dim3(kNumThreads);
    cfg.dynamicSmemBytes = smem_bytes;
    cfg.stream = static_cast<cudaStream_t>(stream);
    cudaLaunchAttribute attr[2];
    int na = 0;
    if ((cluster && grid_z > 1) || p.pair) {
        attr[na].id = cudaLaunchAttributeClusterDimension;
        attr[na].val.clusterDim.x = p.pair ? 2 : 1;
        attr[na].val.clusterDim.y = 1;
        attr[na].val.clusterDim.z = p.pair ? 1 : grid_z;
        ++na;
    }
    if (b200sd_pdl_enabled()) {
        attr[na].id = cudaLaunchAttributeProgrammaticStreamSerialization;
        attr[na].val.programmaticStreamSerializationAllowed = 1;
        ++na;
    }
    cfg.attrs = attr;
    cfg.numAttrs = na;
    B200SD_CUDA(cudaLaunchKernelEx(&cfg, gemm_entry(p.pair, p.b_mode), p));
    g_b200sd_launches.fetch_add(1, std::memory_order_relaxed);
    B200SD_LAUNCH_CHECK();
    return B200SD_OK;
}

bool want_pair(int request, int split, int m_tiles, int n_tiles, int k_blocks) {
    static const bool env_off = getenv("B200SD_PAIR") && getenv("B200SD_PAIR")[0] == '0';
    if (request < 0 || split != 1) return false;
    if (request > 0) return true;
    return !env_off && m_tiles >= 2 && k_blocks >= 32 && (long)m_tiles * n_tiles >= b200sd_num_sms();
}

int pick_block_n_mn(int N, int m_tiles, int kind) {
    int best;
    if (N <= 64) best = 64;
    else if (N <= 128) best = 128;
    else if (kind == 1) best = N <= 192 ? 192 : ((N % 192 == 0 || N % 128 != 0) ? 192 : (N % 256 == 0 ? 256 : 128));
    else best = (N % 192 == 0 && N % 128 != 0) ? 192 : 128;
    while (best > 64 && (long)m_tiles * ceil_div(N, best) * 2 <= b200sd_num_sms()) best -= 64;
    return best;
}

int conv_m_tiling(KParams& p, int NB, int H, int W, int M, int* m_tiles) {
    B200SD_REQUIRE(NB > 0 && H > 0 && W > 0 && M == NB * H * W, "gemm(conv): M=%d != batch*H*W", M);
    p.tiles_x = 1;
    if (W > BLOCK_M) {
        B200SD_REQUIRE(W % BLOCK_M == 0, "gemm(conv): W=%d > 128 must be a multiple of 128", W);
        p.tile_w = BLOCK_M; p.tile_h = 1; p.tile_n = 1;
        p.tiles_x = W / BLOCK_M; p.tiles_y = H;
        p.rows_valid = BLOCK_M;
        p.a_bytes = p.rows_valid * BLOCK_K * 2;
        *m_tiles = NB * H * p.tiles_x;
        return B200SD_OK;
    }
    const int max_h = BLOCK_M / W;
    if (H <= max_h) {
        p.tile_h = H;
        p.tile_n = max_h / H;
        if (p.tile_n < 1) p.tile_n = 1;
        if (p.tile_n > NB) p.tile_n = NB;
    } else {
        p.tile_n = 1;
        p.tile_h = 1;
        for (int h = max_h; h >= 1; --h)
            if (H % h == 0) { p.tile_h = h; break; }
    }
    p.tile_w = W;
    p.tiles_y = H / p.tile_h;
    p.rows_valid = p.tile_w * p.tile_h * p.tile_n;
    p.a_bytes = p.rows_valid * BLOCK_K * 2;
    *m_tiles = (p.tile_n > 1) ? ceil_div(NB, p.tile_n) : NB * p.tiles_y;
    return B200SD_OK;
}

}

extern "C" size_t b200sd_gemm_workspace_bytes(void) { return kWsPartialBytes + kWsCounterBytes; }

extern "C" int b200sd_geglu_tile(int N) {
    if (persist_enabled() && N < 10240) {
        if (N % 256 == 0) return 256;
        if (N % 128 == 0) return 128;
        if (N % 64 == 0) return 64;
    }
    return pick_block_n(N, 1, B200SD_EPI_GEGLU);
}

static int gemm_tiling(const b200sd_gemm_args* a, KParams& p, int* m_tiles_out, int* n_tiles_out) {
    const int C0 = a->C0, C1 = a->a1 ? a->C1 : 0, C = C0 + C1;
    (void)C;
    if (!p.conv) {
        p.rows_valid = BLOCK_M;
        p.a_bytes = kABytes;
        p.tile_w = p.tile_h = p.tile_n = 1;
        p.tiles_x = 1;
        p.tiles_y = 1;
        *m_tiles_out = ceil_div(a->M, BLOCK_M);
    } else {
        const int rc = conv_m_tiling(p, a->batch, a->H, a->W, a->M, m_tiles_out);
        if (rc) return rc;
    }

    const int m_tiles = *m_tiles_out;

    static const bool no_split = getenv("B200SD_SPLITK") && getenv("B200SD_SPLITK")[0] == '0';
    const bool can_split = !no_split && a->split_k <= 0 && a->epilogue == B200SD_EPI_LINEAR && p.num_k_blocks >= 16;
    int bn = a->block_n > 0 ? a->block_n : pick_block_n(a->N, m_tiles, a->epilogue, can_split);
    B200SD_REQUIRE(bn >= 16 && bn <= 256 && bn % 16 == 0 && a->N % bn == 0, "gemm: bad block_n %d for N=%d", bn, a->N);
    B200SD_REQUIRE(a->epilogue != B200SD_EPI_GEGLU || bn % 32 == 0, "gemm: GEGLU needs block_n %% 32 == 0");
    p.block_n = bn;
    int n_tiles = a->N / bn;
    p.tmem_cols = pow2_cols(bn);

    const int sms = b200sd_num_sms();
    int split = a->split_k;
    if (split <= 0) {
        split = 1;
        const int tiles = m_tiles * n_tiles;
        if (!no_split && a->epilogue == B200SD_EPI_LINEAR && tiles * 2 <= sms && p.num_k_blocks >= 16) {
            while (split < 8 && tiles * split * 2 <= sms && p.num_k_blocks / (split * 2) >= 8) split *= 2;
        }
    }
    int n_tiles_f = n_tiles;
    if (a->split_k <= 0 && a->block_n <= 0 && can_split) {
        const int tiles = m_tiles * n_tiles;
        if (split == 8 && tiles > 8) split = 4;
        if (split <= 4 && tiles * split * 2 <= sms && bn % 32 == 0 && bn / 2 >= 80) {
            bn /= 2;
            p.block_n = bn;
            n_tiles_f = a->N / bn;
            p.tmem_cols = pow2_cols(bn);
        }
    }
    B200SD_REQUIRE(split == 1 || a->epilogue == B200SD_EPI_LINEAR, "gemm: split-K only with the linear epilogue");
    B200SD_REQUIRE(split == 1 || split == 2 || split == 4 || split == 8, "gemm: split_k must be 1, 2, 4 or 8 (cluster size)");
    p.kb_per_split = ceil_div(p.num_k_blocks, split);
    B200SD_REQUIRE((split - 1) * p.kb_per_split < p.num_k_blocks, "gemm: split_k=%d leaves an empty split for K=%d", split, a->K);
    *n_tiles_out = n_tiles_f;
    p.split_k = split;
    p.pair = want_pair(a->pair, split, m_tiles, n_tiles_f, p.num_k_blocks) && bn % 32 == 0;
    p.persist = 0;
    p.psplit = 0;
    const bool geglu = a->epilogue == B200SD_EPI_GEGLU;
    static const bool no_psplit = getenv("B200SD_PSPLIT") && getenv("B200SD_PSPLIT")[0] == '0';
    if (persist_enabled() && !no_psplit && a->split_k <= 0 && a->block_n <= 0 && split > 1 && !geglu && p.rows_valid == BLOCK_M &&
        a->N % 32 == 0 && a->workspace != nullptr && a->workspace_bytes >= kWsPartialBytes + kWsCounterBytes &&
        (reinterpret_cast<uintptr_t>(a->workspace) & 127) == 0 && a->ldc % 4 == 0 && (!a->residual || a->ldr % 4 == 0)) {
        int bnp = 0;
        for (int cand : {160, 128, 256, 192, 96, 64, 32})
            if (a->N % cand == 0) { bnp = cand; break; }
        const int sms_s = b200sd_num_sms();
        const long tiles = bnp ? (long)m_tiles * (a->N / bnp) : sms_s + 1;
        int S = 1;
        while (S < 16 && tiles * (S * 2) <= sms_s && p.num_k_blocks / (S * 2) >= 4) S *= 2;
        if (S == 16 && p.num_k_blocks >= 128) {
            p.persist = 1;
            p.psplit = S;
            p.block_n = bnp;
            p.split_k = 1;
            p.pair = 0;
            *n_tiles_out = a->N / bnp;
            return B200SD_OK;
        }
    }
    if (persist_enabled() && split == 1 && !p.pair && p.rows_valid == BLOCK_M && a->N % 32 == 0 &&
        (!a->rowbias || (a->rows_per_image > 0 && a->rows_per_image % 32 == 0)) &&
        !(a->residual && a->residual == a->out && a->residual_dtype != a->out_dtype)) {
        const int bnp = a->block_n > 0 ? a->block_n : pick_block_n_persist(a->N, m_tiles, geglu);
        const long ptiles = bnp > 0 ? (long)m_tiles * (a->N / bnp) : 0;
        const int sms_p = b200sd_num_sms();
        static const int mask = [] { const char* e = getenv("B200SD_PERSIST_MASK"); return e ? atoi(e) : 3; }();
        const bool multi = ptiles >= 2L * sms_p;
        const int cls = !multi ? 4 : (geglu ? 1 : 2);
        if (bnp > 0 && bnp <= 256 && bnp % (geglu ? 64 : 32) == 0 && a->N % bnp == 0 && ((mask & cls) || g_dbg[0] > 0)) {
            p.persist = 1;
            p.block_n = bnp;
            *n_tiles_out = a->N / bnp;
        }
    }
    return B200SD_OK;
}

extern "C" int b200sd_gemm(const b200sd_gemm_args* a, b200sd_stream_t stream) {
    B200SD_REQUIRE(a != nullptr, "gemm: null args");
    B200SD_REQUIRE(a->a0 && a->w && a->out, "gemm: null operand pointer");
    B200SD_REQUIRE(a->M > 0 && a->N > 0 && a->K > 0, "gemm: non-positive dims M=%d N=%d K=%d", a->M, a->N, a->K);
    B200SD_REQUIRE(a->conv_taps == 1 || a->conv_taps == 9, "gemm: conv_taps must be 1 or 9");
    const int C0 = a->C0, C1 = a->a1 ? a->C1 : 0, C = C0 + C1;
    B200SD_REQUIRE(C0 > 0 && C0 % BLOCK_K == 0 && C1 % BLOCK_K == 0, "gemm: channel counts must be multiples of 64 (C0=%d C1=%d)", C0, C1);
    B200SD_REQUIRE(a->K == a->conv_taps * C, "gemm: K=%d != taps*C=%d", a->K, a->conv_taps * C);
    B200SD_REQUIRE(a->N % 16 == 0, "gemm: N=%d must be a multiple of 16", a->N);
    B200SD_REQUIRE(a->epilogue == B200SD_EPI_LINEAR || a->epilogue == B200SD_EPI_GEGLU, "gemm: bad epilogue");
    B200SD_REQUIRE(a->epilogue != B200SD_EPI_GEGLU || (a->bias && !a->residual && !a->rowbias && a->out_dtype == B200SD_BF16),
                   "gemm: GEGLU epilogue needs bias, bf16 out and no residual/rowbias");
    B200SD_REQUIRE(a->out_dtype == B200SD_BF16 || a->out_dtype == B200SD_F32, "gemm: bad out dtype");
    B200SD_REQUIRE(a->residual_dtype == B200SD_BF16 || a->residual_dtype == B200SD_F32, "gemm: bad residual dtype");
    B200SD_REQUIRE(a->ldc % 8 == 0 && (!a->residual || a->ldr % 8 == 0), "gemm: ldc/ldr must be multiples of 8");
    B200SD_REQUIRE((reinterpret_cast<uintptr_t>(a->out) & 15) == 0 && (reinterpret_cast<uintptr_t>(a->a0) & 15) == 0 &&
                       (reinterpret_cast<uintptr_t>(a->w) & 15) == 0 && (reinterpret_cast<uintptr_t>(a->a1) & 15) == 0 &&
                       (reinterpret_cast<uintptr_t>(a->residual) & 15) == 0 && (reinterpret_cast<uintptr_t>(a->bias) & 15) == 0 &&
                       (reinterpret_cast<uintptr_t>(a->rowbias) & 15) == 0,
                   "gemm: pointers must be 16-byte aligned");
    B200SD_REQUIRE(!a->rowbias || (a->rows_per_image > 0 && a->ldrb % 4 == 0), "gemm: rowbias needs rows_per_image and ldrb %% 4 == 0");

    KParams p;
    memset(&p, 0, sizeof(p));
    p.M = a->M;
    p.N = a->N;
    p.num_k_blocks = a->K / BLOCK_K;
    p.conv = a->conv_taps == 9;
    p.cblocks0 = C0 / BLOCK_K;
    p.cblocks = C / BLOCK_K;
    p.bias = a->bias;
    p.rowbias = a->rowbias;
    p.residual = a->residual;
    p.res_f32 = a->residual_dtype == B200SD_F32;
    p.out = a->out;
    p.ldc = a->ldc;
    p.ldr = a->ldr;
    p.ldrb = a->ldrb > 0 ? a->ldrb : a->N;
    p.rows_per_image = a->rows_per_image > 0 ? a->rows_per_image : 1;
    p.epilogue = a->epilogue;
    p.out_f32 = a->out_dtype == B200SD_F32;
    p.conv_sign = 1;
    p.n_valid = a->N;
    p.tiles_per_tap = 1;

    int m_tiles = 0, n_tiles = 0;
    {
        const int rc = gemm_tiling(a, p, &m_tiles, &n_tiles);
        if (rc) return rc;
    }
    const int bn = p.block_n, split = p.split_k;
    p.gn_part = a->gn_part;
    p.prefetch = a->prefetch;
    p.prefetch_bytes = a->prefetch ? a->prefetch_bytes : 0;
    B200SD_REQUIRE(!a->prefetch || (reinterpret_cast<uintptr_t>(a->prefetch) & 15) == 0, "gemm: prefetch pointer must be 16-byte aligned");
    B200SD_REQUIRE(!a->gn_part || (a->out_dtype == B200SD_F32 && a->epilogue == B200SD_EPI_LINEAR &&
                                   (!a->residual || a->residual_dtype == B200SD_F32)),
                   "gemm: gn_part needs fp32 output, the linear epilogue and no bf16 residual");

    if (!p.conv) {
        const uint64_t dimsA[2] = {(uint64_t)C0, (uint64_t)a->M};
        const uint64_t strA[2] = {0, (uint64_t)(a->lda0 > 0 ? a->lda0 : C0) * 2};
        const uint32_t boxA[2] = {BLOCK_K, BLOCK_M};
        int rc = b200sd_make_tmap(&p.tmA0, a->a0, 2, dimsA, strA, boxA, CU_TENSOR_MAP_SWIZZLE_128B);
        if (rc) return rc;
        if (C1 > 0) {
            const uint64_t dimsA1[2] = {(uint64_t)C1, (uint64_t)a->M};
            const uint64_t strA1[2] = {0, (uint64_t)(a->lda1 > 0 ? a->lda1 : C1) * 2};
            rc = b200sd_make_tmap(&p.tmA1, a->a1, 2, dimsA1, strA1, boxA, CU_TENSOR_MAP_SWIZZLE_128B);
            if (rc) return rc;
        }
    } else {
        const uint32_t boxA[4] = {BLOCK_K, (uint32_t)p.tile_w, (uint32_t)p.tile_h, (uint32_t)p.tile_n};
        const uint64_t dims0[4] = {(uint64_t)C0, (uint64_t)a->W, (uint64_t)a->H, (uint64_t)a->batch};
        const uint64_t str0[4] = {0, (uint64_t)C0 * 2, (uint64_t)a->W * C0 * 2, (uint64_t)a->H * a->W * C0 * 2};
        int rc = b200sd_make_tmap(&p.tmA0, a->a0, 4, dims0, str0, boxA, CU_TENSOR_MAP_SWIZZLE_128B);
        if (rc) return rc;
        if (C1 > 0) {
            const uint64_t dims1[4] = {(uint64_t)C1, (uint64_t)a->W, (uint64_t)a->H, (uint64_t)a->batch};
            const uint64_t str1[4] = {0, (uint64_t)C1 * 2, (uint64_t)a->W * C1 * 2, (uint64_t)a->H * a->W * C1 * 2};
            rc = b200sd_make_tmap(&p.tmA1, a->a1, 4, dims1, str1, boxA, CU_TENSOR_MAP_SWIZZLE_128B);
            if (rc) return rc;
        }
    }
    p.w_kmajor = a->w_layout == B200SD_W_KBLOCK_MAJOR;
    B200SD_REQUIRE(a->w_layout == B200SD_W_ROW_MAJOR || a->w_layout == B200SD_W_KBLOCK_MAJOR, "gemm: bad w_layout %d", a->w_layout);
    if (p.w_kmajor) {
        const uint64_t dimsB[3] = {(uint64_t)BLOCK_K, (uint64_t)a->N, (uint64_t)(a->K / BLOCK_K)};
        const uint64_t strB[3] = {0, (uint64_t)BLOCK_K * 2, (uint64_t)a->N * BLOCK_K * 2};
        const uint32_t boxB[3] = {BLOCK_K, (uint32_t)(p.pair ? bn / 2 : bn), 1};
        int rc = b200sd_make_tmap(&p.tmB, a->w, 3, dimsB, strB, boxB, CU_TENSOR_MAP_SWIZZLE_128B);
        if (rc) return rc;
    } else {
        const uint64_t dimsB[2] = {(uint64_t)a->K, (uint64_t)a->N};
        const uint64_t strB[2] = {0, (uint64_t)a->K * 2};
        const uint32_t boxB[2] = {BLOCK_K, (uint32_t)(p.pair ? bn / 2 : bn)};
        int rc = b200sd_make_tmap(&p.tmB, a->w, 2, dimsB, strB, boxB, CU_TENSOR_MAP_SWIZZLE_128B);
        if (rc) return rc;
    }

    if (p.persist) return launch_persist(a, p, m_tiles, stream);
    return launch_gemm(p, m_tiles, n_tiles, split, true, stream);
}

extern "C" int b200sd_gemm_gn_layout(const b200sd_gemm_args* a, int hw, int* parts_per_image, int* total_parts) {
    B200SD_REQUIRE(a && parts_per_image && total_parts && hw > 0, "gemm_gn_layout: bad arguments");
    KParams p;
    memset(&p, 0, sizeof(p));
    p.M = a->M;
    p.N = a->N;
    p.num_k_blocks = a->K / BLOCK_K;
    p.conv = a->conv_taps == 9;
    int m_tiles = 0, n_tiles = 0;
    const int rc = gemm_tiling(a, p, &m_tiles, &n_tiles);
    if (rc) return rc;
    *parts_per_image = 0;
    *total_parts = 0;
    if (a->out_dtype != B200SD_F32 || a->epilogue != B200SD_EPI_LINEAR || (a->residual && a->residual_dtype != B200SD_F32)) return B200SD_OK;
    if (p.persist && p.psplit > 1) {
        const int rpc = BLOCK_M / p.psplit;
        if (a->M % hw != 0 || hw % rpc != 0 || (p.conv && a->H * a->W != hw)) return B200SD_OK;
        *parts_per_image = hw / rpc;
        *total_parts = m_tiles * p.psplit;
        return B200SD_OK;
    }
    if (p.persist) {
        if (a->M % hw != 0 || hw % BLOCK_M != 0 || (p.conv && a->H * a->W != hw)) return B200SD_OK;
        *parts_per_image = hw / BLOCK_M;
        *total_parts = m_tiles;
        return B200SD_OK;
    }
    const int rpp = BLOCK_M / p.split_k;
    int ppi;
    if (p.conv) {
        if (a->H * a->W != hw) return B200SD_OK;
        if (p.tile_n == 1) ppi = p.tiles_y * p.tiles_x * p.split_k;
        else if (p.rows_valid == BLOCK_M && hw % rpp == 0) ppi = hw / rpp;
        else return B200SD_OK;
    } else {
        if (a->M % hw != 0 || hw % rpp != 0) return B200SD_OK;
        ppi = hw / rpp;
    }
    if (p.pair) m_tiles = (m_tiles + 1) & ~1;
    *parts_per_image = ppi;
    *total_parts = m_tiles * p.split_k;
    return B200SD_OK;
}

extern "C" int b200sd_gemm_dgrad(const b200sd_dgrad_args* a, b200sd_stream_t stream) {
    B200SD_REQUIRE(a != nullptr && a->dy && a->w && a->out, "dgrad: null pointer");
    B200SD_REQUIRE(a->conv_taps == 1 || a->conv_taps == 9, "dgrad: conv_taps must be 1 or 9");
    B200SD_REQUIRE(a->M > 0 && a->Cout > 0 && a->Cout % BLOCK_K == 0, "dgrad: Cout=%d must be a positive multiple of 64", a->Cout);
    B200SD_REQUIRE(a->Cin > 0 && a->Cin % 8 == 0, "dgrad: Cin=%d must be a multiple of 8", a->Cin);
    B200SD_REQUIRE(a->out_dtype == B200SD_BF16 || a->out_dtype == B200SD_F32, "dgrad: bad out dtype");
    const int ldy = a->ldy > 0 ? a->ldy : a->Cout;
    const int ldc = a->ldc > 0 ? a->ldc : a->Cin;
    const int ldr = a->ldr > 0 ? a->ldr : a->Cin;
    B200SD_REQUIRE(ldc % 8 == 0 && ldr % 8 == 0 && ldy % 8 == 0, "dgrad: pitches must be multiples of 8");
    B200SD_REQUIRE(((reinterpret_cast<uintptr_t>(a->dy) | reinterpret_cast<uintptr_t>(a->w) | reinterpret_cast<uintptr_t>(a->out) |
                     reinterpret_cast<uintptr_t>(a->residual)) & 15) == 0, "dgrad: pointers must be 16-byte aligned");
    KParams p;
    memset(&p, 0, sizeof(p));
    p.M = a->M;
    p.N = a->Cin;
    p.n_valid = a->Cin;
    p.tiles_per_tap = 1;
    p.conv = a->conv_taps == 9;
    p.conv_sign = -1;
    p.b_mode = 1;
    p.cblocks0 = p.cblocks = a->Cout / BLOCK_K;
    p.num_k_blocks = a->conv_taps * p.cblocks;
    p.residual = a->residual;
    p.res_f32 = a->residual_dtype == B200SD_F32;
    p.out = a->out;
    p.ldc = ldc;
    p.ldr = ldr;
    p.ldrb = a->Cin;
    p.rows_per_image = 1;
    p.epilogue = B200SD_EPI_LINEAR;
    p.out_f32 = a->out_dtype == B200SD_F32;
    int m_tiles;
    if (!p.conv) {
        p.rows_valid = BLOCK_M;
        p.a_bytes = kABytes;
        p.tile_w = p.tile_h = p.tile_n = p.tiles_y = 1;
        p.tiles_x = 1;
        m_tiles = ceil_div(a->M, BLOCK_M);
    } else {
        B200SD_REQUIRE(ldy == a->Cout, "dgrad(conv): dy must be dense NHWC");
        const int rc = conv_m_tiling(p, a->batch, a->H, a->W, a->M, &m_tiles);
        if (rc) return rc;
    }
    int bn = a->block_n > 0 ? a->block_n : pick_block_n_mn(a->Cin, m_tiles, 0);
    B200SD_REQUIRE(bn % 64 == 0 && bn >= 64 && bn <= 256, "dgrad: block_n %d must be 64, 128, 192 or 256", bn);
    p.pair = want_pair(a->pair, 1, m_tiles, ceil_div(a->Cin, bn), p.num_k_blocks);
    if (p.pair && bn % 128 != 0) {
        if (a->block_n > 0) p.pair = 0;
        else bn = (ceil_div(a->Cin, 256) * 256 <= ceil_div(a->Cin, 128) * 128) ? 256 : 128;
    }
    p.block_n = bn;
    const int n_tiles = ceil_div(a->Cin, bn);
    p.tmem_cols = pow2_cols(bn);
    int split = 1;
    {
        static const bool no_split = getenv("B200SD_SPLITK") && getenv("B200SD_SPLITK")[0] == '0';
// ... 120 lines not shown
```

### stable-diffusion-for-book-cover-generation_b200/engine.py

```python
from __future__ import annotations

import ctypes as C

import os

import weakref

import torch

from . import ops
from ._lib import check, lib


class _Pool:

    def __init__(self, device):
        self.device = device
        self.free = {}
        self.total = 0

    def get(self, rows, cols, dtype=torch.bfloat16):
        key = (rows * cols, dtype)
        lst = self.free.get(key)
        if lst:
            return lst.pop().view(rows, cols)
        self.total += rows * cols * (2 if dtype == torch.bfloat16 else 4)
        return torch.empty(rows, cols, dtype=dtype, device=self.device)

    def put(self, t):
        self.free.setdefault((t.numel(), t.dtype), []).append(t)


class _Plan(list):

    def __init__(self):
        super().__init__()
        self.meta = []

    def append(self, fn, kind="other", flops=0.0, name=""):
        super().append(fn)
        self.meta.append((kind, float(flops), name))


class Engine:
    def __init__(self, model, N, H, W, S_ctx, device, io=None):
        self.model, self.N, self.H, self.W, self.S = model, N, H, W, S_ctx
        self.device = device
        self._io = io
        cfg = model.config
        self.heads = cfg.attention_head_dim
        self.ctx_dim = cfg.cross_attention_dim
        self.plan = _Plan()
        self.ctx_plan = _Plan()
        self.pool = _Pool(device)
        self.graph = None
        self._ctx_key = None
        self._keep = []
        self.debug = False
        self.debug_out = {}
        self.gn_from_gemm = os.environ.get("B200SD_GN_FROM_GEMM", "1") != "0"
        self._gn_parts = {}
        self.prefetch_kblocks = int(os.environ.get("B200SD_PREFETCH", "0"))
        self.prefetch_weights = self.prefetch_kblocks > 0
        self._prev_gemm, self._first_w = None, None
        with torch.cuda.device(device):
            self._build()

    def _gemm(self, plan, a0, w, out, **kw):
        rb = kw.pop("rowbias_ptr", None)
        gn_hw = kw.pop("gn_hw", 0)
        args = ops.gemm(a0, w, out, launch=False, **kw)
        if rb is not None:
            args.rowbias, args.ldrb, args.rows_per_image = rb[0], rb[1], rb[2]
        self._gn_parts.pop(id(out), None)
        if gn_hw > 0 and self.gn_from_gemm:
            parts = ops.gemm_attach_gn_parts(args, gn_hw, self.device)
            if parts is not None:
                self._gn_parts[id(out)] = parts
                self._keep.append(parts)
        self._keep.append((a0, w, out, kw))
        if plan is self.plan and self.prefetch_weights:
            if self._prev_gemm is not None:
                self._prev_gemm.prefetch, self._prev_gemm.prefetch_bytes = w.data_ptr(), self._prefetch_bytes(w)
            else:
                self._first_w = w
            self._prev_gemm = args
        kind = "conv3x3" if args.conv_taps == 9 else "gemm"
        plan.append(lambda a=args: ops.gemm_run(a), kind, 2.0 * args.M * args.N * args.K,
                    f"{kind} M{args.M} N{args.N} K{args.K}")

    def _prefetch_bytes(self, w):
        total = w.numel() * w.element_size()
        if w.dim() == 3:
            return min(total, self.prefetch_kblocks * w.shape[1] * w.shape[2] * w.element_size())
        return total if self.prefetch_kblocks >= 1000 else 0

    def _groupnorm(self, x, skip, g, b, out, hw, eps, silu, raw_out=None):
        N = self.N
        p0 = self._gn_parts.get(id(x))
        p1 = self._gn_parts.get(id(skip)) if skip is not None else None
        C = x.shape[-1] + (skip.shape[-1] if skip is not None else 0)
        if p0 is not None and (skip is None or p1 is not None) and ops.gn_parts_supported(C, 32):
            self._keep.append((p0, p1))
            self.plan.append(lambda: ops.groupnorm_silu_parts(x, skip, p0, p1, g, b, out, N, hw, 32, eps, silu, raw_out=raw_out),
                             "groupnorm", 0, "groupnorm (stats from GEMM)")
        else:
            self.plan.append(lambda: ops.groupnorm_silu(x, skip, g, b, out, N, hw, 32, eps, silu, raw_out=raw_out), "groupnorm")

    def _tap(self, name, t, h, w):
        def op():
            if self.debug:
                self.debug_out[name] = t.float().reshape(self.N, h, w, -1).permute(0, 3, 1, 2).clone()
        self.plan.append(op, "tap")

    def _build(self):
        m, Wp, N, dev = self.model, self.model._packed, self.N, self.device
        cfg = m.config
        boc = cfg.block_out_channels
        P, pool = self.plan, self.pool
        f32 = dict(dtype=torch.float32, device=dev)

        if self._io is not None:
            self.in_sample, self.in_t, self.out = self._io
        else:
            self.in_sample = torch.zeros(N, cfg.in_channels, self.H, self.W, **f32)
            self.in_t = torch.zeros(N, **f32)
            self.out = torch.zeros(N, cfg.out_channels, self.H, self.W, **f32)
        self.in_ctx = torch.zeros(N * self.S, self.ctx_dim, dtype=torch.bfloat16, device=dev)

        temb_dim = boc[0] * 4
        t_sin = torch.empty(N, boc[0], **f32)
        t_h = torch.empty(N, temb_dim, **f32)
        t_emb = torch.empty(N, temb_dim, **f32)
        n_tp = Wp["tproj"]["n"]
        self.tproj = torch.empty(N, n_tp, **f32)
        te = Wp["temb"]
        P.append(lambda: ops.timestep_embedding(self.in_t, boc[0], out=t_sin), "time_embed")
        P.append(lambda: ops.small_linear(t_sin, te["w1"], te["b1"], silu_out=True, out=t_h), "time_embed")
        P.append(lambda: ops.small_linear(t_h, te["w2"], te["b2"], out=t_emb), "time_embed")
        self.large_batch = N >= int(os.environ.get("B200SD_LARGE_BATCH", "8"))
        if self.large_batch:
            a16 = torch.empty(N, temb_dim, dtype=torch.bfloat16, device=dev)
            P.append(lambda: ops.cast_act(t_emb, a16, silu=True), "time_embed")
            self._gemm(P, a16, Wp["tproj"]["w"], self.tproj, bias=Wp["tproj"]["b"])
            self.plan.meta[-1] = ("time_embed", self.plan.meta[-1][1], "time_emb_proj x22 (tensor cores)")
        else:
            P.append(lambda: ops.small_linear(t_emb, Wp["tproj"]["w"], Wp["tproj"]["b"], silu_in=True, out=self.tproj), "time_embed", 0, "time_emb_proj x22")

        self.attn_ws = torch.empty(ops.attention_workspace_bytes(N, self.heads, self.H * self.W, boc[0] // self.heads) + 256,
                                   dtype=torch.uint8, device=dev)

        h, w = self.H, self.W
        F32 = torch.float32
        x = pool.get(N * h * w, boc[0], F32)
        P.append(lambda x=x: ops.conv_in(self.in_sample, Wp["conv_in"]["w"], Wp["conv_in"]["b"], x), "conv_io", 0, "conv_in")

        self._tap("conv_in", x, h, w)
        skips = [(x, boc[0])]
        skip_refs = {id(x): 1}

        def release(t):
            if skip_refs.get(id(t), 0) > 0:
                return
            pool.put(t)

        def resnet(prefix, r, x, skip, h, w):
            wr = Wp[prefix]
            M = N * h * w
            cin, cout = r.cin, r.cout
            t1 = pool.get(M, cin)
            raw = pool.get(M, cin) if "wsc" in wr else None
            self._groupnorm(x, skip, wr["g1"], wr["b1"], t1, h * w, cfg.norm_eps, True, raw_out=raw)
            hbuf = pool.get(M, cout, F32)
            rb = (self.tproj.data_ptr() + m._tproj_off[prefix] * 4, n_tp, h * w)
            self._gemm(P, t1, wr["w1"], hbuf, bias=wr["cb1"], conv=(N, h, w), rowbias_ptr=rb, gn_hw=h * w)
            pool.put(t1)
            t2 = pool.get(M, cout)
            self._groupnorm(hbuf, None, wr["g2"], wr["b2"], t2, h * w, cfg.norm_eps, True)
            pool.put(hbuf)
            if "wsc" in wr:
                sc = pool.get(M, cout, F32)
                self._gemm(P, raw, wr["wsc"], sc, bias=wr["bsc"])
                pool.put(raw)
            else:
                sc = x
            y = pool.get(M, cout, F32)
            self._gemm(P, t2, wr["w2"], y, bias=wr["cb2"], residual=sc, conv=(N, h, w), gn_hw=h * w)
            pool.put(t2)
            if sc is not x:
                pool.put(sc)
            self._tap(prefix, y, h, w)
            return y

        def xformer(prefix, a, x, h, w):
            wa = Wp[prefix]
            Cc = a.ch
            M = N * h * w
            d = Cc // self.heads
            scale = d ** -0.5
            kv = torch.empty(N * self.S, 2 * Cc, dtype=torch.bfloat16, device=dev)
            self._gemm(self.ctx_plan, self.in_ctx, wa["w_kv2"], kv)
            t = pool.get(M, Cc)
            self._groupnorm(x, None, wa["gn_g"], wa["gn_b"], t, h * w, 1e-6, False)
            hs = pool.get(M, Cc, F32)
            self._gemm(P, t, wa["w_in"], hs, bias=wa["b_in"])
            P.append(lambda: ops.layernorm(hs, wa["ln1_g"], wa["ln1_b"], t), "layernorm")
            qkv = pool.get(M, 3 * Cc)
            self._gemm(P, t, wa["w_qkv"], qkv)
            P.append(lambda: ops.attention(qkv, qkv, qkv, t, N, self.heads, h * w, h * w, d, scale, ldq=3 * Cc,
                                           ldk=3 * Cc, ldv=3 * Cc, ldo=Cc, q_off=0, k_off=Cc, v_off=2 * Cc, ws=self.attn_ws),
                     "attention", 4.0 * N * self.heads * (h * w) * (h * w) * d, f"self-attn S{h * w} d{d}")
            pool.put(qkv)
            self._gemm(P, t, wa["w_o1"], hs, bias=wa["b_o1"], residual=hs)
            P.append(lambda: ops.layernorm(hs, wa["ln2_g"], wa["ln2_b"], t), "layernorm")
            q = pool.get(M, Cc)
            self._gemm(P, t, wa["w_q2"], q)
            P.append(lambda: ops.attention(q, kv, kv, t, N, self.heads, h * w, self.S, d, scale, ldq=Cc, ldk=2 * Cc,
                                           ldv=2 * Cc, ldo=Cc, k_off=0, v_off=Cc, ws=self.attn_ws),
                     "attention", 4.0 * N * self.heads * (h * w) * self.S * d, f"cross-attn S{h * w} d{d}")
            pool.put(q)
            self._gemm(P, t, wa["w_o2"], hs, bias=wa["b_o2"], residual=hs)
            P.append(lambda: ops.layernorm(hs, wa["ln3_g"], wa["ln3_b"], t), "layernorm")
            ff = pool.get(M, 4 * Cc)
            self._gemm(P, t, wa["w_ff1"], ff, bias=wa["b_ff1"], epilogue=ops.EPI_GEGLU, block_n=wa["ff_tile"])
            self._gemm(P, ff, wa["w_ff2"], t, bias=wa["b_ff2"], residual=hs)
            pool.put(ff)
            y = pool.get(M, Cc, F32)
            self._gemm(P, t, wa["w_out"], y, bias=wa["b_out"], residual=x, gn_hw=h * w)
            pool.put(t)
            pool.put(hs)
            self._tap(prefix, y, h, w)
            return y

        def push_skip(t, c):
            skips.append((t, c))
            skip_refs[id(t)] = skip_refs.get(id(t), 0) + 1

        for i, b in enumerate(m.down_blocks):
            for j, r in enumerate(b.resnets):
                y = resnet(f"down{i}.res{j}", r, x, None, h, w)
                release(x)
                x = y
                if hasattr(b, "attentions"):
                    y = xformer(f"down{i}.attn{j}", b.attentions[j], x, h, w)
                    release(x)
                    x = y
                push_skip(x, r.cout)
            if hasattr(b, "downsamplers"):
                wd = Wp[f"down{i}.ds"]
                Cc = boc[i]
                col = pool.get(N * (h // 2) * (w // 2), 9 * Cc)
                P.append(lambda x=x, col=col, h=h, w=w: ops.im2col_s2(x, col, N, h, w), "resample", 0, "im2col_s2")
                h, w = h // 2, w // 2
                y = pool.get(N * h * w, Cc, F32)
                self._gemm(P, col, wd["w"], y, bias=wd["b"], gn_hw=h * w)
                pool.put(col)
                release(x)
                x = y
                self._tap(f"down{i}.ds", x, h, w)
                push_skip(x, Cc)

        y = resnet("mid.res0", m.mid_block.resnets[0], x, None, h, w)
        release(x)
        x = y
        y = xformer("mid.attn0", m.mid_block.attentions[0], x, h, w)
        release(x)
        x = y
        y = resnet("mid.res1", m.mid_block.resnets[1], x, None, h, w)
        release(x)
        x = y

        for i, b in enumerate(m.up_blocks):
            for j, r in enumerate(b.resnets):
                skip, _c = skips.pop()
                y = resnet(f"up{i}.res{j}", r, x, skip, h, w)
                skip_refs[id(skip)] -= 1
                release(skip)
                release(x)
                x = y
                if hasattr(b, "attentions"):
                    y = xformer(f"up{i}.attn{j}", b.attentions[j], x, h, w)
                    release(x)
                    x = y
            if hasattr(b, "upsamplers"):
                wu = Wp[f"up{i}.us"]
                Cc = x.shape[1]
                up = pool.get(N * 4 * h * w, Cc)
                P.append(lambda x=x, up=up, h=h, w=w: ops.upsample2x(x, up, N, h, w), "resample", 0, "upsample2x")
                release(x)
                h, w = 2 * h, 2 * w
                y = pool.get(N * h * w, Cc, F32)
                self._gemm(P, up, wu["w"], y, bias=wu["b"], conv=(N, h, w), gn_hw=h * w)
                pool.put(up)
                x = y
                self._tap(f"up{i}.us", x, h, w)

        wo = Wp["conv_out"]
        t = pool.get(N * h * w, boc[0])
        self._groupnorm(x, None, wo["g"], wo["beta"], t, h * w, cfg.norm_eps, True)
        if self.large_batch and boc[0] % 64 == 0 and cfg.out_channels <= 4:
            tmp = pool.get(N * h * w, 32, F32)
            self._gemm(P, t, wo["w_tc"], tmp, a1=t, conv=(N, h, w))
            self.plan.meta[-1] = ("conv_io", self.plan.meta[-1][1], "conv_out (tensor cores)")
            P.append(lambda tmp=tmp: ops.nhwc_bias_to_nchw(tmp, wo["b"], self.out), "conv_io", 0, "conv_out: bias + NCHW")
        else:
            P.append(lambda t=t: ops.conv_out(t, wo["w"], wo["b"], self.out), "conv_io", 0, "conv_out")
        if self._prev_gemm is not None and self._first_w is not None:
            self._prev_gemm.prefetch, self._prev_gemm.prefetch_bytes = self._first_w.data_ptr(), self._prefetch_bytes(self._first_w)
        self.activation_bytes = pool.total

    def set_context(self, ctx):
        ref = self._ctx_key[0]() if self._ctx_key is not None else None
        if ref is ctx and self._ctx_key[1] == ctx._version:
            return
        self.in_ctx.copy_(ctx.reshape(self.N * self.S, self.ctx_dim))
        for op in self.ctx_plan:
            op()
        self._ctx_key = (weakref.ref(ctx), ctx._version)

    def _run_plan(self):
        for op in self.plan:
            op()

    def run(self, sample, timestep, ctx, use_graph=True):
        with torch.cuda.device(self.device):
            self.set_context(ctx)
            self.in_sample.copy_(sample)
            if torch.is_tensor(timestep):
                self.in_t.copy_(timestep.to(device=self.device, dtype=torch.float32).reshape(-1).expand(self.N))
            else:
                self.in_t.fill_(float(timestep))
            if not use_graph:
                self._run_plan()
            else:
                if self.graph is None:
                    self._run_plan()
                    torch.cuda.current_stream().synchronize()
                    g = torch.cuda.CUDAGraph()
                    before = ops.launch_count()
                    with torch.cuda.graph(g):
                        self._run_plan()
                    self.kernels_per_graph = ops.launch_count() - before
                    self.graph = g
                self.graph.replay()
            return self.out.clone()

    def profile(self, iters=5):
        return profile_plan(self.plan, self.device, iters)


def profile_plan(plan, device, iters=5):
    with torch.cuda.device(device):
        entries = [(op, meta) for op, meta in zip(plan, plan.meta) if meta[0] != "tap"]
        n = len(entries)
        check(lib().b200sd_timer_reserve(n + 1), "timer_reserve")

        def run_all():
            for op, _m in entries:
                op()
        run_all()
        torch.cuda.synchronize()
        side = torch.cuda.Stream()
        g = torch.cuda.CUDAGraph()
        with torch.cuda.graph(g, stream=side):
            sh = torch.cuda.current_stream().cuda_stream
            for i, (op, _meta) in enumerate(entries):
                check(lib().b200sd_timer_record(i, sh), "timer_record")
                op()
            check(lib().b200sd_timer_record(n, sh), "timer_record")
        torch.cuda.synchronize()
        times = [0.0] * n
        total = 0.0
        ms = C.c_float(0.0)
        g.replay()
        torch.cuda.synchronize()
        for _ in range(iters):
            g.replay()
            torch.cuda.synchronize()
            for i in range(n):
# ... 15 lines not shown
```

### stable-diffusion-for-book-cover-generation_b200/ops.py

```python
from __future__ import annotations

import ctypes as C

import torch

from ._lib import DgradArgs, GemmArgs, WgradArgs, B200SDError, check, lib

F32, BF16 = 0, 1
EPI_LINEAR, EPI_GEGLU = 0, 1
_GN_RECOMPUTE = __import__("os").environ.get("B200SD_GN_FAST", "1") == "0"


def _up16(*ts):
    had = any(t is not None and t.dtype == torch.float16 for t in ts)
    return tuple(t.float() if (t is not None and t.dtype == torch.float16) else t for t in ts) + (had,)


def _dt(t: torch.Tensor) -> int:
    if t.dtype == torch.float32:
        return F32
    if t.dtype == torch.bfloat16:
        return BF16
    raise B200SDError(f"unsupported dtype {t.dtype} (float32 / bfloat16 only)")

# ... 71 lines not shown
        out = torch.empty_like(x)
    if eps_u.numel() != x.numel():
        raise ValueError(f"model_output {tuple(eps_u.shape)} and sample {tuple(x.shape)} sizes differ")
    w = (C.c_float * 5)(*([float(v) for v in weights] + [0.0] * (5 - len(weights))))
    hp = [_p(h) for h in hist] + [None] * (4 - len(hist))
    check(lib().b200sd_cfg_plms_step(_p(eps_u), _p(eps_c), _p(x), _p(out), _p(eps_out), hp[0], hp[1], hp[2], hp[3],
                                     len(hist), w, x.numel(), float(guidance), float(cx), float(ce), _dt(eps_u), _dt(x),
                                     _stream()), "cfg_plms_step")
    return out


def add_noise(x0, noise, timesteps, sa_table, sb_table, out=None):
    x0, noise, half = _up16(x0, noise)
    if half:
        r = add_noise(x0.contiguous(), noise.contiguous(), timesteps, sa_table, sb_table).half()
        return r if out is None else out.copy_(r)
    _chk(x0, noise, timesteps, sa_table, sb_table, out)
    if x0.shape != noise.shape:
        raise ValueError("original_samples / noise shape mismatch")
    if timesteps.dtype != torch.int64 or timesteps.numel() != x0.shape[0]:
        raise ValueError("timesteps must be int64 of shape (batch,)")
    if noise.dtype != x0.dtype:
        noise = noise.to(x0.dtype)
    if out is None:
        out = torch.empty_like(x0)
    B = x0.shape[0]
    check(lib().b200sd_add_noise(_p(x0), _p(noise), _p(timesteps), _p(sa_table), _p(sb_table), _p(out), B,
                                 x0.numel() // max(B, 1), sa_table.numel(), _dt(x0), _stream()), "add_noise")
    return out


def mse_loss_fwd(pred, target):
    _chk(pred, target)
    if pred.shape != target.shape:
        raise ValueError("pred / target shape mismatch")
    ws = _workspace("mse", lib().b200sd_mse_workspace_floats() * 4, pred.device)
    out = torch.empty(1, dtype=torch.float32, device=pred.device)
    check(lib().b200sd_mse_loss_fwd(_p(pred), _p(target), _p(out), _p(ws), pred.numel(), _dt(pred), _dt(target),
                                    _stream()), "mse_loss_fwd")
    return out


def mse_loss_bwd(pred, target, grad_loss):
    _chk(pred, target, grad_loss)
    g = torch.empty_like(pred)
    gl = grad_loss.reshape(1).to(torch.float32)
    check(lib().b200sd_mse_loss_bwd(_p(pred), _p(target), _p(gl), _p(g), pred.numel(), _dt(pred), _dt(target),
                                    _stream()), "mse_loss_bwd")
    return g


class _MSELoss(torch.autograd.Function):
    @staticmethod
    def forward(ctx, pred, target):
        ctx.pred_dtype = pred.dtype
        pred, target, _ = _up16(pred, target)
        ctx.save_for_backward(pred, target)
        return mse_loss_fwd(pred.contiguous(), target.contiguous()).reshape(())

    @staticmethod
    def backward(ctx, grad):
        pred, target = ctx.saved_tensors
        return mse_loss_bwd(pred.contiguous(), target.contiguous(), grad.contiguous().float()).to(ctx.pred_dtype), None


def mse_loss(pred, target):
    return _MSELoss.apply(pred, target)


def timestep_embedding(t_f32, dim, out=None):
    _chk(t_f32, out)
    B = t_f32.numel()
    if out is None:
        out = torch.empty(B, dim, dtype=torch.float32, device=t_f32.device)
    check(lib().b200sd_timestep_embedding(_p(t_f32), _p(out), B, dim, _stream()), "timestep_embedding")
    return out


def small_linear(x, w_bf16, bias, silu_in=False, silu_out=False, out=None):
    _chk(x, w_bf16, bias, out)
    B, K = x.shape
    N = w_bf16.shape[0]
    if out is None:
        out = torch.empty(B, N, dtype=torch.float32, device=x.device)
    check(lib().b200sd_small_linear(_p(x), _p(w_bf16), _p(bias), _p(out), B, N, K, int(silu_in), int(silu_out),
                                    _stream()), "small_linear")
    return out


def gemm_workspace(device):
    return _workspace(("gemm", _stream()), max(16, lib().b200sd_gemm_workspace_bytes()), device)


def gemm(a0, w, out, *, a1=None, bias=None, rowbias=None, residual=None, conv=None, rows_per_image=0,
         epilogue=EPI_LINEAR, block_n=0, split_k=0, M=None, ldrb=0, launch=True, pair=0):
    _chk(a0, a1, w, bias, rowbias, residual, out)
    if w.dim() == 3:
        N, K = w.shape[1], w.shape[0] * w.shape[2]
    else:
        N, K = w.shape
    C0 = a0.shape[-1]
    C1 = a1.shape[-1] if a1 is not None else 0
    if M is None:
        M = a0.numel() // C0
    ws = gemm_workspace(a0.device)
    args = GemmArgs()
    args.a0, args.a1, args.w = _p(a0), _p(a1), _p(w)
    args.bias, args.rowbias, args.residual, args.out = _p(bias), _p(rowbias), _p(residual), _p(out)
    args.M, args.N, args.K, args.C0, args.C1 = M, N, K, C0, C1
    args.lda0, args.lda1 = C0, C1
    args.ldc = out.shape[-1]
    args.ldr = residual.shape[-1] if residual is not None else 0
    args.ldrb = ldrb
    if conv is not None:
        args.conv_taps = 9
        args.batch, args.H, args.W = conv
    else:
        args.conv_taps = 1
    args.rows_per_image = rows_per_image
    args.epilogue = epilogue
    args.out_dtype = _dt(out)
    args.residual_dtype = _dt(residual) if residual is not None else BF16
    args.block_n, args.split_k = block_n, split_k
    args.pair = pair
    args.w_layout = 1 if w.dim() == 3 else 0
    args.workspace, args.workspace_bytes = _p(ws), ws.numel()
    if not launch:
        return args
    check(lib().b200sd_gemm(C.byref(args), _stream()), "gemm")
    return out


def gemm_run(args):
    check(lib().b200sd_gemm(C.byref(args), _stream()), "gemm")


class GnParts:
    __slots__ = ("buf", "ppi", "ld")

    def __init__(self, buf, ppi, ld):
        self.buf, self.ppi, self.ld = buf, ppi, ld


def gemm_attach_gn_parts(args, hw, device):
    ppi, total = C.c_int(0), C.c_int(0)
    check(lib().b200sd_gemm_gn_layout(C.byref(args), int(hw), C.byref(ppi), C.byref(total)), "gemm_gn_layout")
    if ppi.value <= 0:
        return None
    buf = torch.zeros(total.value * 2 * args.N, dtype=torch.float32, device=device)
    args.gn_part = buf.data_ptr()
    return GnParts(buf, ppi.value, args.N)


def groupnorm_silu_parts(x0, x1, parts0, parts1, gamma, beta, out, batch, hw, groups=32, eps=1e-5, silu=True, raw_out=None,
                         stats_out=None):
    _chk(x0, x1, gamma, beta, out, raw_out, stats_out)
    C0 = x0.shape[-1]
    C1 = x1.shape[-1] if x1 is not None else 0
    rc = lib().b200sd_groupnorm_silu_parts(_p(x0), _p(x1), C0, C1, _p(parts0.buf), parts0.ppi, parts0.ld,
                                           _p(parts1.buf) if parts1 is not None else None, parts1.ppi if parts1 is not None else 0,
                                           parts1.ld if parts1 is not None else 0, _p(gamma), _p(beta), _p(out), _p(raw_out),
                                           _p(stats_out), batch, hw, groups, float(eps), int(silu), _dt(x0), _stream())
    check(rc, "groupnorm_silu_parts")
    return out


def gn_parts_supported(C, groups=32):
    if C % groups:
        return False
    cpg = C // groups
    G = 1
    while (G * cpg) % 8 != 0 and G < groups:
        G *= 2
    while G * 2 <= groups and groups % (G * 2) == 0 and G * cpg < 32:
        G *= 2
    Cg = G * cpg
    return Cg % 8 == 0 and groups % G == 0 and Cg // 8 <= 512


def gemm_dgrad(dy, w, out, *, residual=None, conv=None, Cin=None, block_n=0, launch=True, pair=0):
    _chk(dy, w, residual, out)
    Cout = w.shape[0]
    taps = 9 if conv is not None else 1
    if Cin is None:
        Cin = w.shape[1] // taps
    a = DgradArgs()
    a.dy, a.w, a.residual, a.out = _p(dy), _p(w), _p(residual), _p(out)
    a.M, a.Cout, a.Cin, a.conv_taps = dy.numel() // dy.shape[-1], Cout, Cin, taps
    if conv is not None:
        a.batch, a.H, a.W = conv
    a.ldy, a.ldc = dy.shape[-1], out.shape[-1]
    a.ldr = residual.shape[-1] if residual is not None else 0
    a.out_dtype = _dt(out)
    a.residual_dtype = _dt(residual) if residual is not None else BF16
    a.block_n = block_n
    a.pair = pair
    if not launch:
        return a
    check(lib().b200sd_gemm_dgrad(C.byref(a), _stream()), "gemm_dgrad")
    return out


def gemm_wgrad(dy, x, dw, *, conv=None, lddw=0, block_n=0, split_k=0, launch=True):
    _chk(dy, x, dw)
    if dw.dtype != torch.float32:
        raise B200SDError("gemm_wgrad: dw must be float32")
    a = WgradArgs()
    a.dy, a.x, a.dw = _p(dy), _p(x), _p(dw)
    a.rows, a.Cout, a.Cin = dy.numel() // dy.shape[-1], dy.shape[-1], x.shape[-1]
    a.conv_taps = 9 if conv is not None else 1
    if conv is not None:
        a.batch, a.H, a.W = conv
    a.ldy, a.ldx, a.lddw = dy.shape[-1], x.shape[-1], lddw
    a.block_n, a.split_k = block_n, split_k
    if not launch:
        return a
    check(lib().b200sd_gemm_wgrad(C.byref(a), _stream()), "gemm_wgrad")
    return dw


def geglu_tile(N):
    return int(lib().b200sd_geglu_tile(N))


def conv_in(x_nchw, w_packed, bias, out):
    _chk(x_nchw, w_packed, bias, out)
    B, Cin, H, W = x_nchw.shape
    check(lib().b200sd_conv_in(_p(x_nchw), _p(w_packed), _p(bias), _p(out), B, Cin, w_packed.shape[0], H, W, _dt(out), _stream()),
          "conv_in")
    return out


def conv_out(x_nhwc, w_packed, bias, out_nchw):
    _chk(x_nhwc, w_packed, bias, out_nchw)
    B, Cout, H, W = out_nchw.shape
    check(lib().b200sd_conv_out(_p(x_nhwc), _p(w_packed), _p(bias), _p(out_nchw), B, x_nhwc.shape[-1], Cout, H, W,
                                _stream()), "conv_out")
    return out_nchw


def nhwc_bias_to_nchw(x_f32, bias, out_nchw):
    _chk(x_f32, bias, out_nchw)
    B, C, H, W = out_nchw.shape
    check(lib().b200sd_nhwc_bias_to_nchw(_p(x_f32), _p(bias), _p(out_nchw), B, C, H * W, x_f32.shape[-1], _stream()), "nhwc_bias_to_nchw")
    return out_nchw


def groupnorm_silu(x0, x1, gamma, beta, out, batch, hw, groups=32, eps=1e-5, silu=True, raw_out=None, stats_out=None):
    _chk(x0, x1, gamma, beta, out, raw_out, stats_out)
    if x1 is not None and x1.dtype != x0.dtype:
        raise B200SDError("groupnorm: both sources must have the same dtype")
    ws = _workspace(("gn", _stream()), lib().b200sd_groupnorm_workspace_floats(batch) * 4, x0.device)
    C0 = x0.shape[-1]
    C1 = x1.shape[-1] if x1 is not None else 0
    check(lib().b200sd_groupnorm_silu_stats(_p(x0), _p(x1), C0, C1, _p(gamma), _p(beta), _p(out), _p(raw_out), _p(ws),
                                            _p(stats_out), batch, hw, groups, float(eps), int(silu), _dt(x0), _stream()),
          "groupnorm_silu")
    return out


def layernorm(x, gamma, beta, out, eps=1e-5):
    _chk(x, gamma, beta, out)
    Cc = x.shape[-1]
    check(lib().b200sd_layernorm(_p(x), _p(gamma), _p(beta), _p(out), x.numel() // Cc, Cc, float(eps), _dt(x), _stream()),
          "layernorm")
    return out


def attention(q, k, v, out, batch, heads, Sq, Skv, d, scale, ldq=None, ldk=None, ldv=None, ldo=None,
              q_off=0, k_off=0, v_off=0, ws=None):
    _chk(q, k, v, out)
    es = 2
    if ws is None:
        ws = _workspace("attn", lib().b200sd_attention_workspace_bytes(batch, heads, Skv, d) + 128, q.device, zero=False)
    check(lib().b200sd_attention(q.data_ptr() + q_off * es, k.data_ptr() + k_off * es, v.data_ptr() + v_off * es,
                                 _p(out), batch, heads, Sq, Skv, d, ldq or q.shape[-1], ldk or k.shape[-1],
                                 ldv or v.shape[-1], ldo or out.shape[-1], float(scale), _p(ws), ws.numel(), _stream()),
          "attention")
    return out


def upsample2x(x, out, batch, H, W):
    _chk(x, out)
    check(lib().b200sd_upsample2x(_p(x), _p(out), batch, H, W, x.shape[-1], _dt(x), _stream()), "upsample2x")
    return out


def im2col_s2(x, out, batch, H, W, pad=1):
    _chk(x, out)
    check(lib().b200sd_im2col_s2_pad(_p(x), _p(out), batch, H, W, x.shape[-1], _dt(x), int(pad), _stream()), "im2col_s2")
    return out


def attention_lse(q, k, v, out, lse, batch, heads, Sq, Skv, d, scale, ldq=None, ldk=None, ldv=None, ldo=None,
                  q_off=0, k_off=0, v_off=0, ws=None):
    _chk(q, k, v, out, lse)
    if ws is None:
        ws = _workspace("attn", lib().b200sd_attention_workspace_bytes(batch, heads, Skv, d) + 128, q.device, zero=False)
    check(lib().b200sd_attention_lse(q.data_ptr() + q_off * 2, k.data_ptr() + k_off * 2, v.data_ptr() + v_off * 2,
                                     _p(out), _p(lse), batch, heads, Sq, Skv, d, ldq or q.shape[-1], ldk or k.shape[-1],
                                     ldv or v.shape[-1], ldo or out.shape[-1], float(scale), _p(ws), ws.numel(),
                                     _stream()), "attention_lse")
    return out


def attention_bwd(q, k, v, out, dout, lse, dq, dk, dv, batch, heads, Sq, Skv, d, scale, *, ldq=None, ldk=None,
# ... 236 lines not shown
```

### stable-diffusion-for-book-cover-generation_b200/packing.py

```python
from __future__ import annotations

import torch


def pack_conv3x3(w: torch.Tensor) -> torch.Tensor:
    co, ci, kh, kw = w.shape
    return w.permute(0, 2, 3, 1).reshape(co, kh * kw * ci).contiguous().to(torch.bfloat16)


def pack_conv3x3_f32(w: torch.Tensor) -> torch.Tensor:
    co, ci, kh, kw = w.shape
    return w.permute(0, 2, 3, 1).reshape(co, kh * kw * ci).contiguous().float()


def pack_linear(w: torch.Tensor) -> torch.Tensor:
    return w.reshape(w.shape[0], -1).contiguous().to(torch.bfloat16)


def pack_geglu(w: torch.Tensor, b: torch.Tensor, tile: int):
    n2 = w.shape[0]
    half = n2 // 2
    h = tile // 2
    assert half % h == 0
    wv, wg = w[:half].reshape(half // h, h, -1), w[half:].reshape(half // h, h, -1)
    bv, bg = b[:half].reshape(half // h, h), b[half:].reshape(half // h, h)
    wp = torch.cat([wv, wg], dim=1).reshape(n2, -1).contiguous().to(torch.bfloat16)
    bp = torch.cat([bv, bg], dim=1).reshape(n2).contiguous().float()
    return wp, bp


def kblock_major(w: torch.Tensor) -> torch.Tensor:
    n, k = w.shape
    assert k % 64 == 0
    return w.reshape(n, k // 64, 64).permute(1, 0, 2).contiguous()


def pack_conv_out_tc(w: torch.Tensor, pad_to: int = 32) -> torch.Tensor:
    co, ci, kh, kw = w.shape
    wt = w.permute(0, 2, 3, 1).reshape(co, kh * kw, ci).float()
    hi = wt.to(torch.bfloat16)
    lo = (wt - hi.float()).to(torch.bfloat16)
    out = torch.zeros(pad_to, kh * kw, 2 * ci, dtype=torch.bfloat16, device=w.device)
    out[:co, :, :ci] = hi
    out[:co, :, ci:] = lo
    return out.reshape(pad_to, kh * kw * 2 * ci).contiguous()
```

### stable-diffusion-for-book-cover-generation_b200/unet.py

```python
from __future__ import annotations

import json
import os
from types import SimpleNamespace

import torch
import torch.nn as nn

from . import ops, packing
from ._lib import B200SDError

SD15_CONFIG = dict(
    sample_size=64, in_channels=4, out_channels=4, center_input_sample=False, flip_sin_to_cos=True, freq_shift=0,
    down_block_types=("CrossAttnDownBlock2D", "CrossAttnDownBlock2D", "CrossAttnDownBlock2D", "DownBlock2D"),
    up_block_types=("UpBlock2D", "CrossAttnUpBlock2D", "CrossAttnUpBlock2D", "CrossAttnUpBlock2D"),
    block_out_channels=(320, 640, 1280, 1280), layers_per_block=2, downsample_padding=1, mid_block_scale_factor=1,
    act_fn="silu", norm_num_groups=32, norm_eps=1e-5, cross_attention_dim=768, attention_head_dim=8,
)


class UNet2DConditionOutput(SimpleNamespace):
    pass


# ... 123 lines not shown
                b.attentions = nn.ModuleList([_xformer(out_ch, ctx) for _ in range(L + 1)])
            if i != len(boc) - 1:
                b.upsamplers = nn.ModuleList([_sampler(out_ch)])
            self.up_blocks.append(b)

        self.conv_norm_out = _norm(boc[0])
        self.conv_out = _conv(cfg["out_channels"], boc[0], 3)

        self.reset_parameters()
        self._engines = {}
        self._packed = None
        self._dirty = True
        self.use_cuda_graph = True
        self._gradient_checkpointing = False
        self._flat = None
        self._train_engines = {}
        self._direct_grads = False
        self._precision = "bf16"
        self._grad_ready_hook = None

    @torch.no_grad()
    def reset_parameters(self):
        params = dict(self.named_parameters())
        for name, p in params.items():
            leaf = name.rsplit(".", 2)
            is_norm = "norm" in leaf[-2]
            if name.endswith("weight"):
                if is_norm:
                    p.fill_(1.0)
                else:
                    fan_in = p[0].numel()
                    bound = (1.0 / fan_in) ** 0.5
                    p.uniform_(-bound, bound)
            else:
                if is_norm:
                    p.zero_()
                else:
                    w = params[name[:-4] + "weight"]
                    bound = (1.0 / w[0].numel()) ** 0.5
                    p.uniform_(-bound, bound)

    @classmethod
    def from_config(cls, cfg):
        return cls(**{k: v for k, v in dict(cfg).items() if not k.startswith("_")})

    @classmethod
    def from_pretrained(cls, path, subfolder=None, torch_dtype=None, **kw):
        d = path if subfolder is None else os.path.join(path, subfolder)
        with open(os.path.join(d, cls.config_name)) as f:
            cfg = json.load(f)
        model = cls(**{k: v for k, v in cfg.items() if not k.startswith("_")})
        st_path = os.path.join(d, "diffusion_pytorch_model.safetensors")
        bin_path = os.path.join(d, "diffusion_pytorch_model.bin")
        if os.path.exists(st_path):
            from safetensors.torch import load_file
            sd = load_file(st_path)
        elif os.path.exists(bin_path):
            sd = torch.load(bin_path, map_location="cpu")
        else:
            raise FileNotFoundError(f"no diffusion_pytorch_model.(safetensors|bin) under {d}")
        model.load_state_dict(sd, strict=True)
        if torch_dtype is not None:
            model.to(dtype=torch_dtype)
        return model.eval()

    def save_pretrained(self, path, safe_serialization=False):
        os.makedirs(path, exist_ok=True)
        cfg = dict(self.config, _class_name="UNet2DConditionModel", _diffusers_version="0.7.2")
        with open(os.path.join(path, self.config_name), "w") as f:
            json.dump(cfg, f, indent=2)
        sd = {k: v.detach().cpu().contiguous() for k, v in self.state_dict().items()}
        if safe_serialization:
            from safetensors.torch import save_file
            save_file(sd, os.path.join(path, "diffusion_pytorch_model.safetensors"))
        else:
            torch.save(sd, os.path.join(path, "diffusion_pytorch_model.bin"))

    def load_state_dict(self, *a, **kw):
        r = super().load_state_dict(*a, **kw)
        self._dirty = True
        return r

    def _apply(self, fn, *a, **kw):
        r = super()._apply(fn, *a, **kw)
        self._dirty = True
        self._engines = {}
        self._flat = None
        self._train_engines = {}
        self._rehome()
        return r

    def _rehome(self):
        ps = list(self.parameters())
        if not ps or any((not p.is_cuda) or p.dtype != torch.float32 or p.device != ps[0].device for p in ps):
            return
        from .train import FlatParams
        with torch.cuda.device(ps[0].device):
            self._flat = FlatParams(self, ps[0].device, lazy=True)

    def set_precision(self, precision: str):
        if precision not in ("bf16", "fp32"):
            raise ValueError("precision must be 'bf16' or 'fp32'")
        if precision != self._precision:
            self._precision = precision
            self._engines = {}
        return self

    def enable_direct_gradients(self, enabled: bool = True):
        self._direct_grads = bool(enabled)
        return self

    def flat_gradients(self):
        return None if self._flat is None else self._flat.grad

    def zero_grad(self, set_to_none: bool = True):
        if self._direct_grads and self._flat is not None and self._flat.grad is not None:
            self._flat.zero_grad()
            self._flat.attach_grads()
            return
        super().zero_grad(set_to_none=set_to_none)

    def mark_weights_changed(self):
        self._dirty = True

    @property
    def device(self):
        return self.conv_in.weight.device

    @property
    def dtype(self):
        return self.conv_in.weight.dtype

    def enable_gradient_checkpointing(self):
        self._gradient_checkpointing = True

    @torch.no_grad()
    def _pack_weights(self):
        W = {}
        f32 = lambda t: t.detach().float().clone()

        def res(prefix, r):
            W[prefix] = dict(
                g1=f32(r.norm1.weight), b1=f32(r.norm1.bias), w1=packing.pack_conv3x3(r.conv1.weight.detach()),
                cb1=f32(r.conv1.bias), g2=f32(r.norm2.weight), b2=f32(r.norm2.bias),
                w2=packing.pack_conv3x3(r.conv2.weight.detach()), cb2=f32(r.conv2.bias))
            if hasattr(r, "conv_shortcut"):
                W[prefix]["wsc"] = packing.pack_linear(r.conv_shortcut.weight.detach())
                W[prefix]["bsc"] = f32(r.conv_shortcut.bias)

        def xf(prefix, a):
            blk = a.transformer_blocks[0]
            C = a.ch
            tile = ops.geglu_tile(8 * C)
            wg, bg = packing.pack_geglu(blk.ff.net[0].proj.weight.detach().float(), blk.ff.net[0].proj.bias.detach().float(), tile)
            W[prefix] = dict(
                gn_g=f32(a.norm.weight), gn_b=f32(a.norm.bias),
                w_in=packing.pack_linear(a.proj_in.weight.detach()), b_in=f32(a.proj_in.bias),
                w_out=packing.pack_linear(a.proj_out.weight.detach()), b_out=f32(a.proj_out.bias),
                ln1_g=f32(blk.norm1.weight), ln1_b=f32(blk.norm1.bias),
                ln2_g=f32(blk.norm2.weight), ln2_b=f32(blk.norm2.bias),
                ln3_g=f32(blk.norm3.weight), ln3_b=f32(blk.norm3.bias),
                w_qkv=packing.pack_linear(torch.cat([blk.attn1.to_q.weight, blk.attn1.to_k.weight, blk.attn1.to_v.weight], 0).detach()),
                w_o1=packing.pack_linear(blk.attn1.to_out[0].weight.detach()), b_o1=f32(blk.attn1.to_out[0].bias),
                w_q2=packing.pack_linear(blk.attn2.to_q.weight.detach()),
                w_kv2=packing.pack_linear(torch.cat([blk.attn2.to_k.weight, blk.attn2.to_v.weight], 0).detach()),
                w_o2=packing.pack_linear(blk.attn2.to_out[0].weight.detach()), b_o2=f32(blk.attn2.to_out[0].bias),
                w_ff1=wg, b_ff1=bg, ff_tile=tile,
                w_ff2=packing.pack_linear(blk.ff.net[2].weight.detach()), b_ff2=f32(blk.ff.net[2].bias))

        W["conv_in"] = dict(w=packing.pack_conv3x3_f32(self.conv_in.weight.detach()), b=f32(self.conv_in.bias))
        W["conv_out"] = dict(w=packing.pack_conv3x3_f32(self.conv_out.weight.detach()), b=f32(self.conv_out.bias),
                             g=f32(self.conv_norm_out.weight), beta=f32(self.conv_norm_out.bias),
                             w_tc=packing.pack_conv_out_tc(self.conv_out.weight.detach()))
        te = self.time_embedding
        W["temb"] = dict(w1=packing.pack_linear(te.linear_1.weight.detach()), b1=f32(te.linear_1.bias),
                         w2=packing.pack_linear(te.linear_2.weight.detach()), b2=f32(te.linear_2.bias))
        tp_w, tp_b, off = [], [], 0
        self._tproj_off = {}
        for prefix, r in self._iter_resnets():
            res(prefix, r)
            tp_w.append(r.time_emb_proj.weight.detach())
            tp_b.append(r.time_emb_proj.bias.detach())
            self._tproj_off[prefix] = off
            off += r.cout
        W["tproj"] = dict(w=packing.pack_linear(torch.cat(tp_w, 0)), b=f32(torch.cat(tp_b, 0)), n=off)
        for prefix, a in self._iter_xformers():
            xf(prefix, a)
        for i, b in enumerate(self.down_blocks):
            if hasattr(b, "downsamplers"):
                W[f"down{i}.ds"] = dict(w=packing.pack_conv3x3(b.downsamplers[0].conv.weight.detach()),
                                        b=f32(b.downsamplers[0].conv.bias))
        for i, b in enumerate(self.up_blocks):
            if hasattr(b, "upsamplers"):
                W[f"up{i}.us"] = dict(w=packing.pack_conv3x3(b.upsamplers[0].conv.weight.detach()),
                                      b=f32(b.upsamplers[0].conv.bias))
        if os.environ.get("B200SD_W_KMAJOR", "0") == "1":
            gemm_keys = ("w1", "w2", "wsc", "w_in", "w_out", "w_qkv", "w_o1", "w_q2", "w_kv2", "w_o2", "w_ff1", "w_ff2")
            for prefix, d in W.items():
                if prefix in ("conv_in", "conv_out", "temb", "tproj"):
                    continue
                for k in list(d.keys()):
                    if k in gemm_keys or (k == "w" and (prefix.endswith(".ds") or prefix.endswith(".us"))):
                        d[k] = packing.kblock_major(d[k])
        self._packed = W
        self._dirty = False
        self._param_versions = self._versions()

    def _ensure_packed(self):
        if self._dirty or self._packed is None or self._versions() != self._param_versions:
            self._pack_weights()
            self._engines = {}
            self.__dict__["_pack_gen"] = self.__dict__.get("_pack_gen", 0) + 1
        return self.__dict__.setdefault("_pack_gen", 0)

    def _stale(self, pack_gen):
        return self._ensure_packed() != pack_gen

    def _versions(self):
        ps = self.__dict__.get("_param_list")
        if ps is None:
            ps = self.__dict__["_param_list"] = list(self.parameters())
        return sum([p._version for p in ps])

    def _iter_resnets(self):
        for i, b in enumerate(self.down_blocks):
            for j, r in enumerate(b.resnets):
                yield f"down{i}.res{j}", r
        for j, r in enumerate(self.mid_block.resnets):
            yield f"mid.res{j}", r
        for i, b in enumerate(self.up_blocks):
            for j, r in enumerate(b.resnets):
                yield f"up{i}.res{j}", r

    def _iter_xformers(self):
        for i, b in enumerate(self.down_blocks):
            if hasattr(b, "attentions"):
                for j, a in enumerate(b.attentions):
                    yield f"down{i}.attn{j}", a
        yield "mid.attn0", self.mid_block.attentions[0]
        for i, b in enumerate(self.up_blocks):
            if hasattr(b, "attentions"):
                for j, a in enumerate(b.attentions):
                    yield f"up{i}.attn{j}", a

    def forward(self, sample, timestep, encoder_hidden_states, return_dict: bool = True):
        if sample.dim() != 4 or sample.shape[1] != self.in_channels:
            raise ValueError(f"sample must be (N, {self.in_channels}, H, W), got {tuple(sample.shape)}")
        if not sample.is_cuda:
            raise B200SDError("b200sd.UNet2DConditionModel runs on CUDA only (no CPU fallback)")
        N, _, H, Wd = sample.shape
        n_down = len(self.config.block_out_channels) - 1
        if H % (1 << n_down) or Wd % (1 << n_down):
            raise ValueError(f"H and W must be multiples of {1 << n_down}")
        ctx = encoder_hidden_states
        if ctx.dim() != 3 or ctx.shape[0] != N or ctx.shape[2] != self.config.cross_attention_dim:
            raise ValueError(f"encoder_hidden_states must be ({N}, S, {self.config.cross_attention_dim}), got {tuple(ctx.shape)}")
        needs_grad = torch.is_grad_enabled() and (
            sample.requires_grad or ctx.requires_grad or any(p.requires_grad for p in self.parameters()) and self.training)
        if needs_grad:
            from .autograd import unet_forward_train
            out = unet_forward_train(self, sample, timestep, ctx)
            return UNet2DConditionOutput(sample=out) if return_dict else (out,)

        self._ensure_packed()
        key = (N, H, Wd, ctx.shape[1], sample.device.index, self._precision)
        eng = self._engines.get(key)
        if eng is None:
            if self._precision == "fp32":
                from .engine_fp32 import EngineF32
                eng = EngineF32(self, N, H, Wd, ctx.shape[1], sample.device)
            else:
                from .engine import Engine
                eng = Engine(self, N, H, Wd, ctx.shape[1], sample.device)
            self._engines[key] = eng
        out = eng.run(sample, timestep, ctx, use_graph=self.use_cuda_graph)
        out = out.to(sample.dtype) if out.dtype != sample.dtype else out
        return UNet2DConditionOutput(sample=out) if return_dict else (out,)
```

Baseline: 198.0.

## Fuse transformer LayerNorms into producer and consumer GEMM epilogues

```diff
diff --git a/include/b200sd.h b/include/b200sd.h
--- a/include/b200sd.h
+++ b/include/b200sd.h
@@ -95,12 +95,19 @@
     const void* prefetch;
     size_t prefetch_bytes;
     int w_layout;
+    void* ln_out;
+    int ld_ln;
+    float* ln_part;
+    int ln_parts;
+    const float* ln_s;
+    float ln_eps;
 } b200sd_gemm_args;
 
 size_t b200sd_gemm_workspace_bytes(void);
 int b200sd_geglu_tile(int N);
 int b200sd_gemm(const b200sd_gemm_args* args, b200sd_stream_t stream);
 int b200sd_gemm_gn_layout(const b200sd_gemm_args* args, int hw, int* parts_per_image, int* total_parts);
+int b200sd_gemm_ln_layout(const b200sd_gemm_args* args, int* parts);
 
 typedef struct b200sd_dgrad_args {
     const void* dy;
diff --git a/stable-diffusion-for-book-cover-generation_b200/_lib.py b/stable-diffusion-for-book-cover-generation_b200/_lib.py
--- a/stable-diffusion-for-book-cover-generation_b200/_lib.py
+++ b/stable-diffusion-for-book-cover-generation_b200/_lib.py
@@ -22,6 +22,8 @@
         ("batch", C.c_int), ("H", C.c_int), ("W", C.c_int), ("rows_per_image", C.c_int), ("epilogue", C.c_int),
         ("out_dtype", C.c_int), ("residual_dtype", C.c_int), ("block_n", C.c_int), ("split_k", C.c_int),
         ("workspace", C.c_void_p), ("workspace_bytes", C.c_size_t), ("pair", C.c_int), ("gn_part", C.c_void_p), ("prefetch", C.c_void_p), ("prefetch_bytes", C.c_size_t), ("w_layout", C.c_int),
+        ("ln_out", C.c_void_p), ("ld_ln", C.c_int), ("ln_part", C.c_void_p), ("ln_parts", C.c_int), ("ln_s", C.c_void_p),
+        ("ln_eps", C.c_float),
     ]
 
 
@@ -81,6 +83,7 @@
     "b200sd_geglu_tile": (_i, [_i]),
     "b200sd_gemm": (_i, [C.POINTER(GemmArgs), _vp]),
     "b200sd_gemm_gn_layout": (_i, [C.POINTER(GemmArgs), _i, C.POINTER(C.c_int), C.POINTER(C.c_int)]),
+    "b200sd_gemm_ln_layout": (_i, [C.POINTER(GemmArgs), C.POINTER(C.c_int)]),
     "b200sd_groupnorm_silu_parts": (_i, [_vp, _vp, _i, _i, _vp, _i, _i, _vp, _i, _i, _vp, _vp, _vp, _vp, _vp, _i, _i, _i, _f, _i,
                                          _i, _vp]),
     "b200sd_gemm_dgrad": (_i, [C.POINTER(DgradArgs), _vp]),
diff --git a/stable-diffusion-for-book-cover-generation_b200/csrc/gemm_tcgen05.cu b/stable-diffusion-for-book-cover-generation_b200/csrc/gemm_tcgen05.cu
--- a/stable-diffusion-for-book-cover-generation_b200/csrc/gemm_tcgen05.cu
+++ b/stable-diffusion-for-book-cover-generation_b200/csrc/gemm_tcgen05.cu
@@ -75,12 +75,33 @@
     int pair;
     int persist;
     int psplit;
+    int ln;
     int w_kmajor;
     const void* prefetch;
     size_t prefetch_bytes;
     float* gn_part;
+    void* ln_out;
+    int ld_ln;
+    float* ln_part;
+    int ln_parts;
+    const float* ln_s;
+    float ln_eps;
     unsigned long long* trace;
 };
+
+__device__ __forceinline__ void ln_row_stats(const float4* rec, int parts, float inv_c, float eps, float& mu, float& rs) {
+    float sb = 0.f, sf = 0.f;
+    for (int j = 0; j < parts; ++j) { const float4 r = __ldg(rec + j); sb += r.x; sf += r.y; }
+    const float mean = sf * inv_c;
+    float m2 = 0.f;
+    for (int j = 0; j < parts; ++j) {
+        const float4 r = __ldg(rec + j);
+        if (r.w > 0.f) { const float d = r.y / r.w - mean; m2 += fmaf(r.w * d, d, r.z); }
+    }
+    mu = sb * inv_c;
+    rs = rsqrtf(m2 * inv_c + eps);
+}
+__device__ __forceinline__ float bf16_round(float x) { return __bfloat162float(__float2bfloat16(x)); }
 
 __device__ __forceinline__ void cluster_sync_all() {
     asm volatile("barrier.cluster.arrive.release.aligned;\n\tbarrier.cluster.wait.acquire.aligned;" ::: "memory");
@@ -106,16 +127,26 @@
     uint32_t stage_u32;
     int pitch_f, row_end, R, cb, half, m0, col_out, img0, n0cb;
     const float* s_rb;
+    const float* s_ln;
     bool multi_img, rb_smem;
 };
+__device__ __forceinline__ void sts8(uint32_t addr, const float (&v)[8]) {
+    asm volatile("st.shared.v4.f32 [%0], {%1, %2, %3, %4};" ::"r"(addr), "f"(v[0]), "f"(v[1]), "f"(v[2]), "f"(v[3]) : "memory");
+    asm volatile("st.shared.v4.f32 [%0], {%1, %2, %3, %4};" ::"r"(addr + 16), "f"(v[4]), "f"(v[5]), "f"(v[6]), "f"(v[7]) : "memory");
+}
 __device__ __forceinline__ void lds8(uint32_t addr, float (&v)[8]) {
     asm volatile("ld.shared.v4.f32 {%0, %1, %2, %3}, [%4];" : "=f"(v[0]), "=f"(v[1]), "=f"(v[2]), "=f"(v[3]) : "r"(addr));
     asm volatile("ld.shared.v4.f32 {%0, %1, %2, %3}, [%4];" : "=f"(v[4]), "=f"(v[5]), "=f"(v[6]), "=f"(v[7]) : "r"(addr + 16));
 }
-template <int OUT, int RES, bool SPLIT, bool GEGLU, bool STATS = false>
+template <int OUT, int RES, bool SPLIT, bool GEGLU, bool STATS = false, int LN = 0>
 __device__ __forceinline__ void epilogue_rows(const KParams& p, const EpiCtx& e, int row0, const float (&b)[8], const float (&bg)[8],
                                               float* cs = nullptr, float* cq = nullptr) {
     constexpr int U = 4;
+    float sn[8], sg[8];
+    if constexpr (LN == 2) {
+#pragma unroll
+        for (int i = 0; i < 8; ++i) { sn[i] = e.s_ln[e.cb + i]; sg[i] = GEGLU ? e.s_ln[e.half + e.cb + i] : 0.f; }
+    }
     for (int row = row0; row < e.row_end; row += e.R * U) {
         float v[U][8], r[U][8];
 #pragma unroll
@@ -143,6 +174,14 @@
             if (rl >= e.row_end) break;
             const int grow = e.m0 + rl;
             float o[8];
+            if constexpr (LN == 2) {
+                const float mu = e.s_ln[256 + rl], rs = e.s_ln[384 + rl];
+#pragma unroll
+                for (int i = 0; i < 8; ++i) {
+                    v[u][i] = rs * fmaf(-mu, sn[i], v[u][i]);
+                    if constexpr (GEGLU) r[u][i] = rs * fmaf(-mu, sg[i], r[u][i]);
+                }
+            }
             if constexpr (GEGLU) {
 #pragma unroll
                 for (int i = 0; i < 8; ++i) o[i] = (v[u][i] + b[i]) * gelu_erf_f(r[u][i] + bg[i]);
@@ -177,12 +216,16 @@
                     red_add_v4(dst + 4, o[4], o[5], o[6], o[7]);
                 } else if constexpr (OUT == 1) st8<B200SD_F32>(p.out, (size_t)grow * p.ldc + e.col_out, o);
                 else st8<B200SD_BF16>(p.out, (size_t)grow * p.ldc + e.col_out, o);
-            }
-        }
-    }
-}
-
-template <bool PAIR, int OP>
+                if constexpr (LN == 1) {
+                    st8<B200SD_BF16>(p.ln_out, (size_t)grow * p.ld_ln + e.col_out, o);
+                    sts8(e.stage_u32 + (uint32_t)(rl * e.pitch_f + e.cb) * 4u, o);
+                }
+            }
+        }
+    }
+}
+
+template <bool PAIR, int OP, int LN = 0>
 __global__ void __launch_bounds__(kNumThreads, 1) gemm_tcgen05_kernel(const __grid_constant__ KParams p) {
     constexpr bool a_mn = OP >= 2;
     constexpr int b_mode = OP;
@@ -355,6 +398,15 @@
                 s_rb[256 + c] = __ldg(p.rowbias + (size_t)img1 * p.ldrb + n0 + c);
             }
         }
+        if constexpr (LN == 2) {
+            for (int c = epi_tid; c < p.block_n; c += 128) s_rb[c] = __ldg(p.ln_s + n0 + c);
+            float mu = 0.f, rs = 0.f;
+            if (m0 + epi_tid < p.M)
+                ln_row_stats(reinterpret_cast<const float4*>(p.ln_part) + (size_t)(m0 + epi_tid) * p.ln_parts, p.ln_parts,
+                             1.f / (float)(p.num_k_blocks * BLOCK_K), p.ln_eps, mu, rs);
+            s_rb[256 + epi_tid] = mu;
+            s_rb[384 + epi_tid] = rs;
+        }
         if (epi_tid == 0 && p.prefetch_bytes)
             ptx::prefetch_share_l2(p.prefetch, p.prefetch_bytes, (blockIdx.z * gridDim.y + blockIdx.y) * gridDim.x + blockIdx.x,
                               gridDim.x * gridDim.y * gridDim.z);
@@ -419,10 +471,19 @@
                 e.pitch_f = pitch_f; e.row_end = row_begin + valid; e.R = R; e.cb = cb; e.half = half; e.m0 = m0;
                 e.col_out = geglu ? n_tile * half + cb : col_base + cb;
                 e.s_rb = s_rb; e.img0 = img0; e.multi_img = multi_img; e.rb_smem = rb_smem; e.n0cb = n0 + cb;
+                e.s_ln = s_rb;
                 const int row0 = row_begin + r0;
                 const int ok = p.atomic_out ? 2 : (p.out_f32 ? 1 : 0);
                 const int rk = p.residual ? (p.res_f32 ? 2 : 1) : 0;
-                if (geglu) epilogue_rows<0, 0, false, true>(p, e, row0, b, bg);
+                if constexpr (LN == 1) {
+                    if (p.split_k > 1) { if (rk == 2) epilogue_rows<1, 2, true, false, false, 1>(p, e, row0, b, bg); else epilogue_rows<1, 0, true, false, false, 1>(p, e, row0, b, bg); }
+                    else if (rk == 2) epilogue_rows<1, 2, false, false, false, 1>(p, e, row0, b, bg);
+                    else epilogue_rows<1, 0, false, false, false, 1>(p, e, row0, b, bg);
+                } else if constexpr (LN == 2) {
+                    if (geglu) epilogue_rows<0, 0, false, true, false, 2>(p, e, row0, b, bg);
+                    else if (p.split_k > 1) epilogue_rows<0, 0, true, false, false, 2>(p, e, row0, b, bg);
+                    else epilogue_rows<0, 0, false, false, false, 2>(p, e, row0, b, bg);
+                } else if (geglu) epilogue_rows<0, 0, false, true>(p, e, row0, b, bg);
                 else if (p.split_k > 1) {
                     if (ok == 1 && p.gn_part) { if (rk == 2) epilogue_rows<1, 2, true, false, true>(p, e, row0, b, bg, cs, cq); else epilogue_rows<1, 0, true, false, true>(p, e, row0, b, bg, cs, cq); }
                     else if (ok == 1) { if (rk == 2) epilogue_rows<1, 2, true, false>(p, e, row0, b, bg); else if (rk == 1) epilogue_rows<1, 1, true, false>(p, e, row0, b, bg); else epilogue_rows<1, 0, true, false>(p, e, row0, b, bg); }
@@ -431,6 +492,28 @@
                 else if (ok == 1 && p.gn_part) { if (rk == 2) epilogue_rows<1, 2, false, false, true>(p, e, row0, b, bg, cs, cq); else epilogue_rows<1, 0, false, false, true>(p, e, row0, b, bg, cs, cq); }
                 else if (ok == 1) { if (rk == 2) epilogue_rows<1, 2, false, false>(p, e, row0, b, bg); else if (rk == 1) epilogue_rows<1, 1, false, false>(p, e, row0, b, bg); else epilogue_rows<1, 0, false, false>(p, e, row0, b, bg); }
                 else { if (rk == 2) epilogue_rows<0, 2, false, false>(p, e, row0, b, bg); else if (rk == 1) epilogue_rows<0, 1, false, false>(p, e, row0, b, bg); else epilogue_rows<0, 0, false, false>(p, e, row0, b, bg); }
+            }
+        }
+        if constexpr (LN == 1) {
+            __syncthreads();
+            for (int rr = tid; rr < valid; rr += kNumThreads) {
+                const int rl = row_begin + rr;
+                const float4* rowp = reinterpret_cast<const float4*>(stage + (size_t)rl * pitch_f);
+                const int n4 = col_valid >> 2;
+                float sf = 0.f, sb = 0.f;
+                for (int c = 0; c < n4; ++c) {
+                    const float4 x = rowp[c];
+                    sf += (x.x + x.y) + (x.z + x.w);
+                    sb += (bf16_round(x.x) + bf16_round(x.y)) + (bf16_round(x.z) + bf16_round(x.w));
+                }
+                const float mean = sf / (float)col_valid;
+                float m2 = 0.f;
+                for (int c = 0; c < n4; ++c) {
+                    const float4 x = rowp[c];
+                    const float d0 = x.x - mean, d1 = x.y - mean, d2 = x.z - mean, d3 = x.w - mean;
+                    m2 += fmaf(d0, d0, d1 * d1) + fmaf(d2, d2, d3 * d3);
+                }
+                reinterpret_cast<float4*>(p.ln_part)[(size_t)(m0 + rl) * p.ln_parts + n_tile] = make_float4(sb, sf, m2, (float)col_valid);
             }
         }
         if (p.gn_part != nullptr) {
@@ -491,6 +574,12 @@
     const void* residual;
     void* out;
     int ldc, ldr;
+    void* ln_out;
+    int ld_ln;
+    float* ln_part;
+    int ln_parts;
+    const float* ln_s;
+    float ln_eps;
     unsigned long long* trace;
 };
 #define PTRACE(slot) do { if (p.trace) p.trace[(size_t)blockIdx.x * 16 + (slot)] = gtimer(); } while (0)
@@ -501,10 +590,11 @@
 #endif
 
 
-template <bool OUT_F32, int RES, bool GEGLU, bool STATS>
+constexpr int kLnSOff = 64;
+template <bool OUT_F32, int RES, bool GEGLU, bool STATS, int LN>
 __device__ __forceinline__ void persist_chunk(const PParams& p, uint32_t taddr, int ch, const float* sbv, const float* sbg, uint8_t* cb,
                                               int lane, bool last_chunk, uint64_t* tempty_bar, uint64_t* rfull_bar, uint32_t rparity,
-                                              float* gn_dst, int nrows) {
+                                              float* gn_dst, int nrows, float ln_mu, float ln_rs, float4& ln_rec, size_t ln_off) {
     uint32_t r0[16], r1[16], g0[16], g1[16];
     ptx::tmem_ld_32x32b_x16(taddr + ch * 32, r0);
     ptx::tmem_ld_32x32b_x16(taddr + ch * 32 + 16, r1);
@@ -519,6 +609,33 @@
         ptx::tc_fence_before();
         __syncwarp();
         if (lane == 0) ptx::mbar_arrive(tempty_bar);
+    }
+    if constexpr (LN == 2) {
+        constexpr int soff = GEGLU ? kLnSOff : 128;
+        const float4* sn4 = reinterpret_cast<const float4*>(sbv + soff);
+#pragma unroll
+        for (int j = 0; j < 8; ++j) {
+            const float4 sn = sn4[j];
+            uint32_t* r = j < 4 ? r0 : r1;
+            const int o = (j & 3) * 4;
+            r[o + 0] = __float_as_uint(ln_rs * fmaf(-ln_mu, sn.x, __uint_as_float(r[o + 0])));
+            r[o + 1] = __float_as_uint(ln_rs * fmaf(-ln_mu, sn.y, __uint_as_float(r[o + 1])));
+            r[o + 2] = __float_as_uint(ln_rs * fmaf(-ln_mu, sn.z, __uint_as_float(r[o + 2])));
+            r[o + 3] = __float_as_uint(ln_rs * fmaf(-ln_mu, sn.w, __uint_as_float(r[o + 3])));
+        }
+        if constexpr (GEGLU) {
+            const float4* sg4 = reinterpret_cast<const float4*>(sbg + kLnSOff);
+#pragma unroll
+            for (int j = 0; j < 8; ++j) {
+                const float4 sn = sg4[j];
+                uint32_t* r = j < 4 ? g0 : g1;
+                const int o = (j & 3) * 4;
+                r[o + 0] = __float_as_uint(ln_rs * fmaf(-ln_mu, sn.x, __uint_as_float(r[o + 0])));
+                r[o + 1] = __float_as_uint(ln_rs * fmaf(-ln_mu, sn.y, __uint_as_float(r[o + 1])));
+                r[o + 2] = __float_as_uint(ln_rs * fmaf(-ln_mu, sn.z, __uint_as_float(r[o + 2])));
+                r[o + 3] = __float_as_uint(ln_rs * fmaf(-ln_mu, sn.w, __uint_as_float(r[o + 3])));
+            }
+        }
     }
     float v[32];
     const float4* sb4 = reinterpret_cast<const float4*>(sbv);
@@ -566,6 +683,30 @@
         }
     }
     if constexpr (RES != 0 && ((RES == 2) != OUT_F32)) __syncwarp();
+    if constexpr (LN == 1) {
+        if (lane < nrows) {
+            uint4* dst = reinterpret_cast<uint4*>(static_cast<bf16*>(p.ln_out) + ln_off + ch * 32);
+            float sf = 0.f, sb = 0.f;
+#pragma unroll
+            for (int j = 0; j < 4; ++j) {
+                uint4 u;
+                u.x = pack_bf16x2(v[8 * j + 0], v[8 * j + 1]);
+                u.y = pack_bf16x2(v[8 * j + 2], v[8 * j + 3]);
+                u.z = pack_bf16x2(v[8 * j + 4], v[8 * j + 5]);
+                u.w = pack_bf16x2(v[8 * j + 6], v[8 * j + 7]);
+                dst[j] = u;
+#pragma unroll
+                for (int i = 0; i < 8; ++i) { sf += v[8 * j + i]; sb += bf16_round(v[8 * j + i]); }
+            }
+            const float cm = sf * (1.f / 32.f);
+            float m2 = 0.f;
+#pragma unroll
+            for (int i = 0; i < 32; ++i) { const float d = v[i] - cm; m2 = fmaf(d, d, m2); }
+            const float na = ln_rec.w, nn = na + 32.f;
+            const float d = na > 0.f ? cm - ln_rec.y / na : 0.f;
+            ln_rec = make_float4(ln_rec.x + sb, ln_rec.y + sf, ln_rec.z + m2 + d * d * (na * 32.f / nn), nn);
+        }
+    }
     if constexpr (OUT_F32) {
 #pragma unroll
         for (int j = 0; j < 8; ++j)
@@ -596,7 +737,7 @@
     }
 }
 
-template <bool OUT_F32, int RES, bool GEGLU, bool STATS>
+template <bool OUT_F32, int RES, bool GEGLU, bool STATS, int LN = 0>
 __device__ __forceinline__ void persist_epilogue(const PParams& p, uint8_t* smem, uint32_t tmem_base, int warp, int lane) {
     const int ew = warp - 2;
     const int q = warp & 3;
@@ -648,8 +789,19 @@
                 if (p.rowbias) b += __ldg(p.rowbias + (size_t)img * p.ldrb + n0 + c);
                 sb[l * 32 + lane] = b;
                 if constexpr (GEGLU) sb[128 + l * 32 + lane] = p.bias ? __ldg(p.bias + n0 + half + c) : 0.f;
-            }
-        }
+                if constexpr (LN == 2) {
+                    sb[(GEGLU ? kLnSOff : 128) + l * 32 + lane] = __ldg(p.ln_s + n0 + c);
+                    if constexpr (GEGLU) sb[128 + kLnSOff + l * 32 + lane] = __ldg(p.ln_s + n0 + half + c);
+                }
+            }
+        }
+        float ln_mu = 0.f, ln_rs = 0.f;
+        if constexpr (LN == 2) {
+            if (row0 + lane < p.M)
+                ln_row_stats(reinterpret_cast<const float4*>(p.ln_part) + (size_t)(row0 + lane) * p.ln_parts, p.ln_parts,
+                             1.f / (float)(p.num_k_blocks * BLOCK_K), p.ln_eps, ln_mu, ln_rs);
+        }
+        float4 ln_rec = make_float4(0.f, 0.f, 0.f, 0.f);
         __syncwarp();
         PACC(0);
         const int acc = it & 1;
@@ -675,8 +827,9 @@
                 __syncwarp();
             }
             PACC(2);
-            persist_chunk<OUT_F32, RES, GEGLU, STATS>(p, taddr, ch, sb + l * 32, sb + 128 + l * 32, cb, lane, l == nl - 1, &tempty[acc],
-                                                     &rfull[buf], (uint32_t)(g / D) & 1u, gn_dst, nrows);
+            persist_chunk<OUT_F32, RES, GEGLU, STATS, LN>(p, taddr, ch, sb + l * 32, sb + 128 + l * 32, cb, lane, l == nl - 1, &tempty[acc],
+                                                         &rfull[buf], (uint32_t)(g / D) & 1u, gn_dst, nrows, ln_mu, ln_rs, ln_rec,
+                                                         (size_t)(row0 + lane) * p.ld_ln + n0);
             PACC(3);
             ptx::fence_proxy_async();
             __syncwarp();
@@ -691,6 +844,9 @@
                 }
             }
             PACC(4);
+        }
+        if constexpr (LN == 1) {
+            if (lane < nrows) reinterpret_cast<float4*>(p.ln_part)[(size_t)(row0 + lane) * p.ln_parts + n_tile * 2 + h] = ln_rec;
         }
         if constexpr (STATS) {
             ptx::named_bar_sync(1, kEpiWarps * 32);
@@ -850,6 +1006,7 @@
     }
 }
 
+template <int LN>
 __global__ void __launch_bounds__(kPersistThreads, 1) gemm_persist_kernel(const __grid_constant__ PParams p) {
     extern __shared__ uint8_t smem_raw[];
     uint8_t* smem = reinterpret_cast<uint8_t*>((reinterpret_cast<uintptr_t>(smem_raw) + 1023) & ~uintptr_t(1023));
@@ -1004,7 +1161,13 @@
         if (warp == 2 && lane == 0 && p.prefetch_bytes)
             ptx::prefetch_share_l2(p.prefetch, p.prefetch_bytes, blockIdx.x, gridDim.x);
         const int variant = (p.geglu ? 100 : 0) + (p.out_f32 ? 10 : 0) + p.res_kind + (p.gn_part ? 1000 : 0);
-        if (splitk) {
+        if constexpr (LN == 1) {
+            if (p.res_kind == 2) persist_epilogue<true, 2, false, false, 1>(p, smem, tmem_base, warp, lane);
+            else persist_epilogue<true, 0, false, false, 1>(p, smem, tmem_base, warp, lane);
+        } else if constexpr (LN == 2) {
+            if (p.geglu) persist_epilogue<false, 0, true, false, 2>(p, smem, tmem_base, warp, lane);
+            else persist_epilogue<false, 0, false, false, 2>(p, smem, tmem_base, warp, lane);
+        } else if (splitk) {
             switch (variant) {
                 case 0: persist_epilogue_split<false, 0, false>(p, smem, tmem_base, warp, lane); break;
                 case 1: persist_epilogue_split<false, 1, false>(p, smem, tmem_base, warp, lane); break;
@@ -1065,7 +1228,9 @@
 
 
 typedef void (*gemm_kernel_t)(const KParams);
-gemm_kernel_t gemm_entry(int pair, int op) {
+gemm_kernel_t gemm_entry(int pair, int op, int ln = 0) {
+    if (ln == 1) return gemm_tcgen05_kernel<false, 0, 1>;
+    if (ln == 2) return gemm_tcgen05_kernel<false, 0, 2>;
     switch ((op << 1) | (pair ? 1 : 0)) {
         case 0: return gemm_tcgen05_kernel<false, 0>;
         case 1: return gemm_tcgen05_kernel<true, 0>;
@@ -1085,12 +1250,15 @@
     B200SD_CUDA(cudaGetDevice(&dev));
     std::lock_guard<std::mutex> lock(mu);
     if (dev < 0 || dev >= 64 || configured[dev]) return B200SD_OK;
-    for (int i = 0; i < 8; ++i) {
-        B200SD_CUDA(cudaFuncSetAttribute(gemm_entry(i & 1, i >> 1), cudaFuncAttributeMaxDynamicSharedMemorySize, (int)(227 * 1024)));
-        B200SD_CUDA(cudaFuncSetAttribute(gemm_entry(i & 1, i >> 1), cudaFuncAttributePreferredSharedMemoryCarveout, 100));
-    }
-    B200SD_CUDA(cudaFuncSetAttribute(gemm_persist_kernel, cudaFuncAttributeMaxDynamicSharedMemorySize, (int)(227 * 1024)));
-    B200SD_CUDA(cudaFuncSetAttribute(gemm_persist_kernel, cudaFuncAttributePreferredSharedMemoryCarveout, 100));
+    for (int i = 0; i < 10; ++i) {
+        const gemm_kernel_t k = i < 8 ? gemm_entry(i & 1, i >> 1) : gemm_entry(0, 0, i - 7);
+        B200SD_CUDA(cudaFuncSetAttribute(k, cudaFuncAttributeMaxDynamicSharedMemorySize, (int)(227 * 1024)));
+        B200SD_CUDA(cudaFuncSetAttribute(k, cudaFuncAttributePreferredSharedMemoryCarveout, 100));
+    }
+    for (auto k : {gemm_persist_kernel<0>, gemm_persist_kernel<1>, gemm_persist_kernel<2>}) {
+        B200SD_CUDA(cudaFuncSetAttribute(k, cudaFuncAttributeMaxDynamicSharedMemorySize, (int)(227 * 1024)));
+        B200SD_CUDA(cudaFuncSetAttribute(k, cudaFuncAttributePreferredSharedMemoryCarveout, 100));
+    }
     configured[dev] = true;
     return B200SD_OK;
 }
@@ -1143,6 +1311,7 @@
     p.kb_per_split = ceil_div(k.num_k_blocks, p.split);
     p.residual = k.residual; p.out = k.out; p.ldc = k.ldc; p.ldr = k.ldr;
     p.prefetch = k.prefetch; p.prefetch_bytes = k.prefetch_bytes;
+    p.ln_out = k.ln_out; p.ld_ln = k.ld_ln; p.ln_part = k.ln_part; p.ln_parts = k.ln_parts; p.ln_s = k.ln_s; p.ln_eps = k.ln_eps;
     const int units = p.num_tiles * p.split;
     if (p.split > 1) {
         B200SD_REQUIRE(k.num_k_blocks >= p.split, "gemm(split-K): fewer K blocks (%d) than slices (%d)", k.num_k_blocks, p.split);
@@ -1224,7 +1393,8 @@
     }
     cfg.attrs = attr;
     cfg.numAttrs = na;
-    B200SD_CUDA(cudaLaunchKernelEx(&cfg, gemm_persist_kernel, p));
+    const auto kern = k.ln == 1 ? gemm_persist_kernel<1> : (k.ln == 2 ? gemm_persist_kernel<2> : gemm_persist_kernel<0>);
+    B200SD_CUDA(cudaLaunchKernelEx(&cfg, kern, p));
     g_b200sd_launches.fetch_add(1, std::memory_order_relaxed);
     B200SD_LAUNCH_CHECK();
     return B200SD_OK;
@@ -1276,7 +1446,7 @@
     }
     cfg.attrs = attr;
     cfg.numAttrs = na;
-    B200SD_CUDA(cudaLaunchKernelEx(&cfg, gemm_entry(p.pair, p.b_mode), p));
+    B200SD_CUDA(cudaLaunchKernelEx(&cfg, gemm_entry(p.pair, p.b_mode, p.ln), p));
     g_b200sd_launches.fetch_add(1, std::memory_order_relaxed);
     B200SD_LAUNCH_CHECK();
     return B200SD_OK;
@@ -1439,6 +1609,32 @@
     return B200SD_OK;
 }
 
+static int ln_parts_for(const b200sd_gemm_args* a, const KParams& p, int n_tiles) {
+    const bool prod = a->ln_out != nullptr, cons = a->ln_s != nullptr;
+    if (prod == cons || p.pair || p.conv || p.psplit > 1 || a->gn_part || a->a1) return 0;
+    if (prod) {
+        if (a->out_dtype != B200SD_F32 || a->epilogue != B200SD_EPI_LINEAR || (a->residual && a->residual_dtype != B200SD_F32)) return 0;
+        return p.persist ? 2 * n_tiles : n_tiles;
+    }
+    if (a->out_dtype != B200SD_BF16 || a->residual || a->rowbias) return 0;
+    return 1;
+}
+
+extern "C" int b200sd_gemm_ln_layout(const b200sd_gemm_args* a, int* parts) {
+    B200SD_REQUIRE(a && parts, "gemm_ln_layout: bad arguments");
+    KParams p;
+    memset(&p, 0, sizeof(p));
+    p.M = a->M;
+    p.N = a->N;
+    p.num_k_blocks = a->K / BLOCK_K;
+    p.conv = a->conv_taps == 9;
+    int m_tiles = 0, n_tiles = 0;
+    const int rc = gemm_tiling(a, p, &m_tiles, &n_tiles);
+    if (rc) return rc;
+    *parts = ln_parts_for(a, p, n_tiles);
+    return B200SD_OK;
+}
+
 extern "C" int b200sd_gemm(const b200sd_gemm_args* a, b200sd_stream_t stream) {
     B200SD_REQUIRE(a != nullptr, "gemm: null args");
     B200SD_REQUIRE(a->a0 && a->w && a->out, "gemm: null operand pointer");
@@ -1491,6 +1687,20 @@
     }
     const int bn = p.block_n, split = p.split_k;
     p.gn_part = a->gn_part;
+    if (a->ln_out || a->ln_s) {
+        const int parts = ln_parts_for(a, p, n_tiles);
+        B200SD_REQUIRE(parts > 0, "gemm: LayerNorm folding is not available for this GEMM (see b200sd_gemm_ln_layout)");
+        B200SD_REQUIRE(a->ln_part && (reinterpret_cast<uintptr_t>(a->ln_part) & 15) == 0 && a->ln_parts > 0,
+                       "gemm: LayerNorm folding needs a 16-byte aligned ln_part and ln_parts > 0");
+        B200SD_REQUIRE(!a->ln_out || a->ln_parts == parts, "gemm: ln_parts=%d, this GEMM writes %d row records", a->ln_parts, parts);
+        B200SD_REQUIRE(!a->ln_out || ((reinterpret_cast<uintptr_t>(a->ln_out) & 15) == 0 && a->ld_ln % 8 == 0 && a->ld_ln >= a->N),
+                       "gemm: ln_out must be 16-byte aligned with ld_ln a multiple of 8 and >= N");
+        B200SD_REQUIRE(!a->ln_s || ((reinterpret_cast<uintptr_t>(a->ln_s) & 15) == 0 && a->ln_eps > 0.f),
+                       "gemm: ln_s must be 16-byte aligned and ln_eps > 0");
+        p.ln = a->ln_out ? 1 : 2;
+        p.ln_out = a->ln_out; p.ld_ln = a->ld_ln; p.ln_part = a->ln_part; p.ln_parts = a->ln_parts;
+        p.ln_s = a->ln_s; p.ln_eps = a->ln_eps;
+    }
     p.prefetch = a->prefetch;
     p.prefetch_bytes = a->prefetch ? a->prefetch_bytes : 0;
     B200SD_REQUIRE(!a->prefetch || (reinterpret_cast<uintptr_t>(a->prefetch) & 15) == 0, "gemm: prefetch pointer must be 16-byte aligned");
diff --git a/stable-diffusion-for-book-cover-generation_b200/engine.py b/stable-diffusion-for-book-cover-generation_b200/engine.py
--- a/stable-diffusion-for-book-cover-generation_b200/engine.py
+++ b/stable-diffusion-for-book-cover-generation_b200/engine.py
@@ -69,9 +69,12 @@
     def _gemm(self, plan, a0, w, out, **kw):
         rb = kw.pop("rowbias_ptr", None)
         gn_hw = kw.pop("gn_hw", 0)
+        ln = kw.pop("ln", None)
         args = ops.gemm(a0, w, out, launch=False, **kw)
         if rb is not None:
             args.rowbias, args.ldrb, args.rows_per_image = rb[0], rb[1], rb[2]
+        if ln is not None:
+            ln(args)
         self._gn_parts.pop(id(out), None)
         if gn_hw > 0 and self.gn_from_gemm:
             parts = ops.gemm_attach_gn_parts(args, gn_hw, self.device)
@@ -203,28 +206,53 @@
             t = pool.get(M, Cc)
             self._groupnorm(x, None, wa["gn_g"], wa["gn_b"], t, h * w, 1e-6, False)
             hs = pool.get(M, Cc, F32)
-            self._gemm(P, t, wa["w_in"], hs, bias=wa["b_in"])
-            P.append(lambda: ops.layernorm(hs, wa["ln1_g"], wa["ln1_b"], t), "layernorm")
+            hb = pool.get(M, Cc)
+            rec = {}
+
+            def produce(args):
+                args.ln_out, args.ld_ln = hb.data_ptr(), Cc
+                parts = ops.gemm_ln_layout(args)
+                if parts <= 0 or rec.get("parts", parts) != parts:
+                    args.ln_out, args.ld_ln = None, 0
+                    rec["off"] = True
+                    return
+                if "buf" not in rec:
+                    rec["buf"], rec["parts"] = torch.empty(M * parts * 4, **f32), parts
+                    self._keep.append(rec["buf"])
+                args.ln_part, args.ln_parts = rec["buf"].data_ptr(), parts
+
+            def consume(w_, s, out, **kw):
+                if "off" in rec:
+                    P.append(lambda: ops.layernorm(hs, wa["ln_one"], wa["ln_zero"], t, wa["ln_eps"]), "layernorm")
+                    self._gemm(P, t, w_, out, **kw)
+                    return
+
+                def setup(args):
+                    args.ln_s, args.ln_part, args.ln_parts, args.ln_eps = s.data_ptr(), rec["buf"].data_ptr(), rec["parts"], wa["ln_eps"]
+                    if ops.gemm_ln_layout(args) != 1:
+                        raise ops.B200SDError(f"gemm M{args.M} N{args.N} K{args.K}: not covered as a LayerNorm consumer")
+                self._gemm(P, hb, w_, out, ln=setup, **kw)
+
+            self._gemm(P, t, wa["w_in"], hs, bias=wa["b_in"], ln=produce)
             qkv = pool.get(M, 3 * Cc)
-            self._gemm(P, t, wa["w_qkv"], qkv)
+            consume(wa["w_qkv"], wa["s_qkv"], qkv, bias=wa["c_qkv"])
             P.append(lambda: ops.attention(qkv, qkv, qkv, t, N, self.heads, h * w, h * w, d, scale, ldq=3 * Cc,
                                            ldk=3 * Cc, ldv=3 * Cc, ldo=Cc, q_off=0, k_off=Cc, v_off=2 * Cc, ws=self.attn_ws),
                      "attention", 4.0 * N * self.heads * (h * w) * (h * w) * d, f"self-attn S{h * w} d{d}")
             pool.put(qkv)
-            self._gemm(P, t, wa["w_o1"], hs, bias=wa["b_o1"], residual=hs)
-            P.append(lambda: ops.layernorm(hs, wa["ln2_g"], wa["ln2_b"], t), "layernorm")
+            self._gemm(P, t, wa["w_o1"], hs, bias=wa["b_o1"], residual=hs, ln=produce)
             q = pool.get(M, Cc)
-            self._gemm(P, t, wa["w_q2"], q)
+            consume(wa["w_q2"], wa["s_q2"], q, bias=wa["c_q2"])
             P.append(lambda: ops.attention(q, kv, kv, t, N, self.heads, h * w, self.S, d, scale, ldq=Cc, ldk=2 * Cc,
                                            ldv=2 * Cc, ldo=Cc, k_off=0, v_off=Cc, ws=self.attn_ws),
                      "attention", 4.0 * N * self.heads * (h * w) * self.S * d, f"cross-attn S{h * w} d{d}")
             pool.put(q)
-            self._gemm(P, t, wa["w_o2"], hs, bias=wa["b_o2"], residual=hs)
-            P.append(lambda: ops.layernorm(hs, wa["ln3_g"], wa["ln3_b"], t), "layernorm")
+            self._gemm(P, t, wa["w_o2"], hs, bias=wa["b_o2"], residual=hs, ln=produce)
             ff = pool.get(M, 4 * Cc)
-            self._gemm(P, t, wa["w_ff1"], ff, bias=wa["b_ff1"], epilogue=ops.EPI_GEGLU, block_n=wa["ff_tile"])
+            consume(wa["w_ff1"], wa["s_ff1"], ff, bias=wa["b_ff1"], epilogue=ops.EPI_GEGLU, block_n=wa["ff_tile"])
             self._gemm(P, ff, wa["w_ff2"], t, bias=wa["b_ff2"], residual=hs)
             pool.put(ff)
+            pool.put(hb)
             y = pool.get(M, Cc, F32)
             self._gemm(P, t, wa["w_out"], y, bias=wa["b_out"], residual=x, gn_hw=h * w)
             pool.put(t)
diff --git a/stable-diffusion-for-book-cover-generation_b200/ops.py b/stable-diffusion-for-book-cover-generation_b200/ops.py
--- a/stable-diffusion-for-book-cover-generation_b200/ops.py
+++ b/stable-diffusion-for-book-cover-generation_b200/ops.py
@@ -247,6 +247,12 @@
     return GnParts(buf, ppi.value, args.N)
 
 
+def gemm_ln_layout(args):
+    parts = C.c_int(0)
+    check(lib().b200sd_gemm_ln_layout(C.byref(args), C.byref(parts)), "gemm_ln_layout")
+    return parts.value
+
+
 def groupnorm_silu_parts(x0, x1, parts0, parts1, gamma, beta, out, batch, hw, groups=32, eps=1e-5, silu=True, raw_out=None,
                          stats_out=None):
     _chk(x0, x1, gamma, beta, out, raw_out, stats_out)
diff --git a/stable-diffusion-for-book-cover-generation_b200/packing.py b/stable-diffusion-for-book-cover-generation_b200/packing.py
--- a/stable-diffusion-for-book-cover-generation_b200/packing.py
+++ b/stable-diffusion-for-book-cover-generation_b200/packing.py
@@ -29,6 +29,19 @@
     return wp, bp
 
 
+def fold_layernorm(w: torch.Tensor, gamma: torch.Tensor, beta: torch.Tensor, bias=None, geglu_tile: int = 0):
+    w64 = w.detach().reshape(w.shape[0], -1).double()
+    wf = w64 * gamma.detach().double()[None, :]
+    c = w64 @ beta.detach().double()
+    if bias is not None:
+        c = c + bias.detach().double()
+    if geglu_tile:
+        wp, cp = pack_geglu(wf, c, geglu_tile)
+    else:
+        wp, cp = pack_linear(wf), c.float().contiguous()
+    return wp, wp.double().sum(1).float().contiguous(), cp
+
+
 def kblock_major(w: torch.Tensor) -> torch.Tensor:
     n, k = w.shape
     assert k % 64 == 0
diff --git a/stable-diffusion-for-book-cover-generation_b200/unet.py b/stable-diffusion-for-book-cover-generation_b200/unet.py
--- a/stable-diffusion-for-book-cover-generation_b200/unet.py
+++ b/stable-diffusion-for-book-cover-generation_b200/unet.py
@@ -299,20 +299,22 @@
             blk = a.transformer_blocks[0]
             C = a.ch
             tile = ops.geglu_tile(8 * C)
-            wg, bg = packing.pack_geglu(blk.ff.net[0].proj.weight.detach().float(), blk.ff.net[0].proj.bias.detach().float(), tile)
+            w_qkv = torch.cat([blk.attn1.to_q.weight, blk.attn1.to_k.weight, blk.attn1.to_v.weight], 0)
+            w_qkv, s_qkv, c_qkv = packing.fold_layernorm(w_qkv, blk.norm1.weight, blk.norm1.bias)
+            w_q2, s_q2, c_q2 = packing.fold_layernorm(blk.attn2.to_q.weight, blk.norm2.weight, blk.norm2.bias)
+            wg, s_ff1, bg = packing.fold_layernorm(blk.ff.net[0].proj.weight, blk.norm3.weight, blk.norm3.bias, blk.ff.net[0].proj.bias,
+                                                   geglu_tile=tile)
             W[prefix] = dict(
                 gn_g=f32(a.norm.weight), gn_b=f32(a.norm.bias),
                 w_in=packing.pack_linear(a.proj_in.weight.detach()), b_in=f32(a.proj_in.bias),
                 w_out=packing.pack_linear(a.proj_out.weight.detach()), b_out=f32(a.proj_out.bias),
-                ln1_g=f32(blk.norm1.weight), ln1_b=f32(blk.norm1.bias),
-                ln2_g=f32(blk.norm2.weight), ln2_b=f32(blk.norm2.bias),
-                ln3_g=f32(blk.norm3.weight), ln3_b=f32(blk.norm3.bias),
-                w_qkv=packing.pack_linear(torch.cat([blk.attn1.to_q.weight, blk.attn1.to_k.weight, blk.attn1.to_v.weight], 0).detach()),
+                ln_one=torch.ones_like(f32(blk.norm1.weight)), ln_zero=torch.zeros_like(f32(blk.norm1.bias)),
+                w_qkv=w_qkv, s_qkv=s_qkv, c_qkv=c_qkv,
                 w_o1=packing.pack_linear(blk.attn1.to_out[0].weight.detach()), b_o1=f32(blk.attn1.to_out[0].bias),
-                w_q2=packing.pack_linear(blk.attn2.to_q.weight.detach()),
+                w_q2=w_q2, s_q2=s_q2, c_q2=c_q2,
                 w_kv2=packing.pack_linear(torch.cat([blk.attn2.to_k.weight, blk.attn2.to_v.weight], 0).detach()),
                 w_o2=packing.pack_linear(blk.attn2.to_out[0].weight.detach()), b_o2=f32(blk.attn2.to_out[0].bias),
-                w_ff1=wg, b_ff1=bg, ff_tile=tile,
+                w_ff1=wg, s_ff1=s_ff1, b_ff1=bg, ff_tile=tile, ln_eps=1e-5,
                 w_ff2=packing.pack_linear(blk.ff.net[2].weight.detach()), b_ff2=f32(blk.ff.net[2].bias))
 
         W["conv_in"] = dict(w=packing.pack_conv3x3_f32(self.conv_in.weight.detach()), b=f32(self.conv_in.bias))
```

Result: faster. 202.7 (median of 6 runs) (+2.4%).
